# kjedrzejewski/video-cycle_gan-upscaling

Measured on AMD Instinct MI355X. Metric: upscaled frames/s (train step, G+D fwd+bwd) at 256->512, higher is better.
Workload: dtype f32; 1 GPU; C2: make_upscaler_orig((512,512,3),k=3,x2,res=9) + PatchGAN-70, batch 8/GPU, gan2 wiring, Wasserstein + pixel-MSE, faithful 3-call step incl. predict pass; global_batch=8, frame=256x256->512x512, parallelism=dp1, launch=hipGraph replay

## Files before the change

include/vcg.h:

```cpp
#ifndef VCG_H
#define VCG_H

#include <stddef.h>
#include <stdint.h>

#ifdef __cplusplus
extern "C" {
#endif

typedef void* vcg_stream_t;

enum {
    VCG_OK = 0,
    VCG_E_NULL = -1,
    VCG_E_SHAPE = -2,
    VCG_E_UNSUPPORTED = -3,
    VCG_E_WORKSPACE = -4
};

enum { VCG_ACT_NONE = 0, VCG_ACT_LRELU = 1, VCG_ACT_PRELU = 2, VCG_ACT_TANH = 3 };
enum { VCG_NORM_BATCH = 0, VCG_NORM_INSTANCE = 1 };
enum { VCG_LOSS_MSE = 0, VCG_LOSS_MAE = 1 };
enum { VCG_HEAD_NONE = 0, VCG_HEAD_SIGMOID = 1, VCG_HEAD_LOGSIGM = 2, VCG_HEAD_TANH = 3, VCG_HEAD_BILOG = 4 };

typedef struct vcg_conv_desc {
    int32_t n, cin, h, w;
    int32_t cout, oh, ow;
    int32_t kh, kw, stride;
    int32_t pad_top, pad_left;
} vcg_conv_desc;

typedef struct vcg_epilogue {
    const float* bias;
    int32_t act;
    float act_alpha;
    const float* prelu_alpha;
    const float* residual;
} vcg_epilogue;

const char* vcg_version(void);
const char* vcg_error_string(int code);

int vcg_conv2d_fwd(const vcg_conv_desc* d, const float* x, const float* w_hwio, float* y,
                   const vcg_epilogue* ep, vcg_stream_t stream);
int vcg_conv2d_stats_records(const vcg_conv_desc* d, int stats_mode);
int vcg_conv2d_fwd_stats(const vcg_conv_desc* d, const float* x, const float* w_hwio, const float* bias, float* y, float* stats,
                         vcg_stream_t stream);
int vcg_conv2d_dgrad(const vcg_conv_desc* d, const float* dy, const float* w_hwio, const float* w_hwoi,
                     float* dx, const float* residual, vcg_stream_t stream);
int vcg_conv2d_fwd_affine(const vcg_conv_desc* d, const float* x, const float* w_hwio, float* y, const vcg_epilogue* ep, const float* scale,
                          const float* shift, vcg_stream_t stream);
size_t vcg_conv2d_wgrad_workspace_bytes(const vcg_conv_desc* d);
int vcg_conv2d_wgrad(const vcg_conv_desc* d, const float* x, const float* dy, float* dw_hwio, float* dbias,
                     void* ws, size_t ws_bytes, vcg_stream_t stream);

int vcg_conv_transpose2d_fwd(const vcg_conv_desc* d, const float* x, const float* w_hwio_t, float* y,
                             const vcg_epilogue* ep, vcg_stream_t stream);
int vcg_conv_transpose2d_dgrad(const vcg_conv_desc* d, const float* dy, const float* w_hwoi, float* dx,
                               const float* residual, vcg_stream_t stream);
size_t vcg_conv_transpose2d_wgrad_workspace_bytes(const vcg_conv_desc* d);
int vcg_conv_transpose2d_wgrad(const vcg_conv_desc* d, const float* x, const float* dy, float* dw_hwoi,
                               float* dbias, void* ws, size_t ws_bytes, vcg_stream_t stream);

int vcg_kernel_transpose(const float* src, float* dst, int taps, int a, int b, vcg_stream_t stream);

size_t vcg_norm_stats_workspace_bytes(int n, int c, int hw, int mode);
int vcg_norm_stats(const float* x, int n, int c, int hw, int mode, float* mean, float* var,
                   void* ws, size_t ws_bytes, vcg_stream_t stream);
int vcg_norm_finalize(const float* mean, const float* var, const float* gamma, const float* beta, int c,
                      int rows, float eps, float* scale, float* shift, float* invstd,
                      float* moving_mean, float* moving_var, float momentum, int unbiased_count,
                      vcg_stream_t stream);
int vcg_sum_records(const float* part, int nrec, int c, float scale, float* out, vcg_stream_t stream);
int vcg_bn_fold(const float* bias, const float* moving_mean, const float* moving_var, const float* gamma, const float* beta, int c, float eps,
                float* scale, float* shift, vcg_stream_t stream);
int vcg_bn_fold_batch(const float* const* bias, const float* const* moving_mean, const float* const* moving_var, const float* const* gamma,
                      const float* const* beta, int count, int c, float eps, float* scale, float* shift, vcg_stream_t stream);
int vcg_norm_finalize_batch(const float* const* mean, const float* const* var, const float* const* gamma, const float* const* beta, int count,
                            int c, float eps, float* scale, float* shift, vcg_stream_t stream);
int vcg_norm_finalize_partials(const float* part, int nrec, int groups, int c, double count, const float* gamma, const float* beta,
                               float eps, float* mean, float* scale, float* shift, float* invstd, float* moving_mean,
                               float* moving_var, float momentum, int unbiased_count, vcg_stream_t stream);
int vcg_norm_finalize_partials_shifted(const float* part, int nrec, int groups, int c, double count, const float* kshift, const float* gamma,
                                       const float* beta, float eps, float* mean, float* scale, float* shift, float* invstd, float* moving_mean,
                                       float* moving_var, float momentum, int unbiased_count, vcg_stream_t stream);
int vcg_norm_act_fwd(const float* x, int n, int c, int hw, const float* scale, const float* shift,
                     int per_sample, int act, float act_alpha, const float* prelu_alpha,
                     const float* residual, float* y, vcg_stream_t stream);
size_t vcg_norm_act_bwd_workspace_bytes(int n, int c, int hw, int mode);
int vcg_norm_act_bwd(const float* x, const float* dy, int n, int c, int hw, int mode,
                     const float* mean, const float* invstd, const float* gamma, const float* beta,
                     int act, float act_alpha, const float* prelu_alpha, int use_batch_stats,
                     float* dx, float* dgamma, float* dbeta, float* dprelu_alpha,
                     void* ws, size_t ws_bytes, vcg_stream_t stream);

size_t vcg_act_bwd_workspace_bytes(int n, int c, int hw);
int vcg_act_bwd(const float* saved, const float* dy, int n, int c, int hw, int act, float act_alpha,
                const float* prelu_alpha, float* dx, float* dprelu_alpha, float* dsum, void* ws, size_t ws_bytes,
                vcg_stream_t stream);
size_t vcg_channel_sum_workspace_bytes(int n, int c, int hw);
int vcg_channel_sum(const float* x, int n, int c, int hw, float* out, void* ws, size_t ws_bytes,
                    vcg_stream_t stream);

int vcg_dense_fwd(const float* x, const float* w_io, const float* bias, float* y, int batch, int in,
                  int out, vcg_stream_t stream);
int vcg_dense_dgrad(const float* dy, const float* w_io, float* dx, int batch, int in, int out,
                    vcg_stream_t stream);
int vcg_dense_wgrad(const float* x, const float* dy, float* dw_io, float* dbias, int batch, int in,
                    int out, vcg_stream_t stream);

size_t vcg_mean_reduce_workspace_bytes(size_t count);
int vcg_mean_reduce(const float* x, size_t count, float* out, void* ws, size_t ws_bytes, vcg_stream_t stream);
int vcg_pixel_loss(const float* pred, const float* target, size_t count, int kind, float grad_scale,
                   float* out, float* dpred, void* ws, size_t ws_bytes, vcg_stream_t stream);
int vcg_head_act_fwd(const float* z, float* y, size_t count, int kind, vcg_stream_t stream);
int vcg_head_act_bwd(const float* z, const float* dy, float* dz, size_t count, int kind, vcg_stream_t stream);
int vcg_gan_loss(const float* mean_a, const float* mean_b, float mean_scale, int kind, float* loss_out, float* da, size_t na,
                 float ga, float* db, size_t nb, float gb, vcg_stream_t stream);
int vcg_sigmoid_gate_fwd(const float* a, const float* m, float* y, size_t count, vcg_stream_t stream);
int vcg_sigmoid_gate_bwd(const float* a, const float* m, const float* dy, float* da, float* dm, size_t count, vcg_stream_t stream);
int vcg_atanh_scale(const float* x, float* y, size_t count, float scale, vcg_stream_t stream);
int vcg_dilate2d(const float* src, float* dst, size_t planes, int h, int w, int stride, vcg_stream_t stream);
int vcg_resize2d(const float* src, float* dst, size_t planes, int h, int w, int factor, int bilinear, vcg_stream_t stream);
int vcg_crop2d(const float* src, float* dst, size_t planes, int h, int w, int top, int left, int oh, int ow, vcg_stream_t stream);
int vcg_pad2d(const float* src, float* dst, size_t planes, int h, int w, int top, int left, int oh, int ow, vcg_stream_t stream);
int vcg_copy_channels(const float* src, float* dst, int n, int c_src, int c_src_off, int c_dst, int c_dst_off, int c_count, size_t hw,
                      vcg_stream_t stream);
int vcg_dropout_fwd(const float* x, float* y, unsigned char* mask, size_t count, float rate, unsigned long long seed,
                    const unsigned long long* step, vcg_stream_t stream);
int vcg_dropout_bwd(const float* dy, const unsigned char* mask, float* dx, size_t count, float rate, vcg_stream_t stream);
int vcg_counter_inc(unsigned long long* counter, vcg_stream_t stream);
int vcg_fill(float* y, size_t count, float value, vcg_stream_t stream);
int vcg_axpby(const float* x, float* y, size_t count, float a, float b, vcg_stream_t stream);

int vcg_maxpool2x2_fwd(const float* x, float* y, int n, int c, int h, int w, vcg_stream_t stream);
int vcg_maxpool2x2_bwd(const float* x, const float* dy, float* dx, int n, int c, int h, int w, vcg_stream_t stream);

int vcg_adam_keras_multi(float* p, const float* g, float* m, float* v, size_t count, float lr_t,
                         float beta_1, float beta_2, float eps, float grad_scale, vcg_stream_t stream);

int vcg_adam_keras_multi_dev(float* p, const float* g, float* m, float* v, size_t count, float lr,
                             float beta_1, float beta_2, float eps, float grad_scale, int* t_dev, vcg_stream_t stream);

int vcg_frames_u8_to_nchw(const uint8_t* src, float* dst, int n, int h, int w, int c, vcg_stream_t stream);
int vcg_nchw_to_frames_u8(const float* src, uint8_t* dst, int n, int h, int w, int c, vcg_stream_t stream);
int vcg_nhwc_to_nchw(const float* src, float* dst, int n, int h, int w, int c, vcg_stream_t stream);
int vcg_nchw_to_nhwc(const float* src, float* dst, int n, int h, int w, int c, vcg_stream_t stream);


typedef struct vcg_epilogue_bf16 {
    const void* scale;
    const void* shift;
    int32_t act;
    float act_alpha;
    const void* prelu_alpha;
    const void* residual;
    void* stats;
    int32_t stats_mode;
} vcg_epilogue_bf16;
#define VCG_STATS_NONE 0
#define VCG_STATS_BATCH 1
#define VCG_STATS_INSTANCE 2

int vcg_pack_conv_kernel_bf16(const void* w, int32_t taps, int32_t a, int32_t b, int32_t transpose, int32_t flip, void* out,
                              hipStream_t stream);

int vcg_pack_conv3x3_c64_bf16_batch(const void* const* w_host_array, int32_t count, void* out, hipStream_t stream);
int vcg_f32_nchw_to_bf16_nhwc(const void* x, void* y, int32_t n, int32_t c, int32_t h, int32_t w, hipStream_t stream);
int vcg_bf16_nhwc_to_f32_nchw(const void* x, void* y, int32_t n, int32_t c, int32_t h, int32_t w, hipStream_t stream);

int vcg_conv2d_bf16_fwd(const vcg_conv_desc* d, const void* x, const void* w_packed, void* y, const vcg_epilogue_bf16* ep,
                        hipStream_t stream);
int vcg_conv2d_bf16_stats_records(const vcg_conv_desc* d, int32_t stats_mode);

int vcg_conv_transpose2d_bf16_fwd(const vcg_conv_desc* d, const void* x, const void* w_packed, void* y, const vcg_epilogue_bf16* ep,
                                  hipStream_t stream);

#define VCG_FINAL9X9_WFRAG_BYTES ((4 * 9 * 4 * 64 + 4) * 16)
int vcg_pack_final9x9_bf16(const void* w, void* out, hipStream_t stream);
int vcg_conv9x9_to3_bf16_fwd(const vcg_conv_desc* d, const void* x, const void* wfrag, const void* bias, int32_t tanh_act, void* y,
                             hipStream_t stream);
size_t vcg_conv9x9_to3_bf16_wfrag_bytes(int32_t cin);
int vcg_pack_conv9x9_to3_bf16(const void* w, int32_t cin, void* out, hipStream_t stream);
#define VCG_OUT_F32_NCHW 0
#define VCG_OUT_U8_NHWC 1
int vcg_conv9x9_to3_bf16_fwd_window(const vcg_conv_desc* d, const void* x, const void* wfrag, const void* bias, int32_t tanh_act,
                                    int32_t out_kind, void* y, int32_t row0, int32_t rows, int32_t y_row0, int32_t y_h, hipStream_t stream);
size_t vcg_conv9x9_c64to3_bf16_wfrag_bytes(void);
int vcg_pack_conv9x9_c64to3_bf16(const void* w, void* out, hipStream_t stream);
int vcg_conv9x9_c64to3_bf16_fwd(const vcg_conv_desc* d, const void* x, const void* wfrag, const void* bias, int32_t tanh_act, void* y,
                                hipStream_t stream);
int vcg_conv9x9_c64to3_bf16_fwd_window(const vcg_conv_desc* d, const void* x, const void* wfrag, const void* bias, int32_t tanh_act,
                                       int32_t out_kind, void* y, int32_t row0, int32_t rows, int32_t y_row0, int32_t y_h, hipStream_t stream);

#define VCG_FIRST9X9_WFRAG_BYTES (27 * 64 * 2 * 16)
int vcg_pack_first9x9_bf16(const void* w, void* out, hipStream_t stream);
int vcg_pack_conv9x9_3ch_bf16(const void* w, int32_t cout, int32_t dgrad, void* out, hipStream_t stream);
int vcg_conv9x9_to3_bf16_dgrad(const vcg_conv_desc* d, const void* dy, const void* wfrag, const void* y_prev, float lrelu_slope, void* dx,
                               hipStream_t stream);
int vcg_conv9x9_to3_bf16_dgrad_chsum_records(const vcg_conv_desc* d);
int vcg_conv9x9_to3_bf16_dgrad_chsum(const vcg_conv_desc* d, const void* dy, const void* wfrag, const void* y_prev, float lrelu_slope, void* dx,
                                     float* records, hipStream_t stream);
int vcg_conv9x9_from3_bf16_fwd(const vcg_conv_desc* d, const void* x, const void* wfrag, const void* bias, const void* prelu_alpha,
                               void* y, hipStream_t stream);

size_t vcg_conv3ch_bf16_wfrag_bytes(int32_t kh, int32_t kw, int32_t cout);
int vcg_pack_conv3ch_bf16(const void* w, int32_t kh, int32_t kw, int32_t cout, void* out, hipStream_t stream);
int vcg_conv3ch_bf16_fwd(const vcg_conv_desc* d, const void* x, const void* wfrag, const void* bias, float lrelu_slope, void* y, hipStream_t stream);

size_t vcg_conv_in_gate_bf16_wfrag_bytes(int32_t cin, int32_t kh, int32_t kw, int32_t cout);
int vcg_pack_conv_in_gate_bf16(const void* w_hwio, int32_t cin, int32_t kh, int32_t kw, int32_t cout, void* out, hipStream_t stream);
int vcg_conv_in_gate_bf16_fwd(const vcg_conv_desc* d, const void* u, const void* wfrag, const void* bias, const void* m, void* y,
                              hipStream_t stream);

int vcg_input_convt_add_bf16(const vcg_conv_desc* d, const void* x, const void* w_hwoi, const void* bias, void* y, hipStream_t stream);
size_t vcg_conv3ch_bf16_dgrad_workspace_bytes(const vcg_conv_desc* d);
int vcg_conv3ch_bf16_dgrad(const vcg_conv_desc* d, const void* dz, const float* w_hwio, float* dx, void* ws, size_t ws_bytes, vcg_stream_t stream);
size_t vcg_conv3ch_bf16_wgrad_workspace_bytes(const vcg_conv_desc* d);
int vcg_conv3ch_bf16_wgrad(const vcg_conv_desc* d, const float* x, const void* dz, float* dw_hwio, float* dbias, void* ws, size_t ws_bytes,
                           vcg_stream_t stream);
int vcg_conv9x9_from3_bf16_fwd_train(const vcg_conv_desc* d, const void* x, const void* wfrag, const void* bias, const void* prelu_alpha,
                                     void* y, void* z, hipStream_t stream);
int vcg_prelu_bwd_nhwc_bf16_records(int n, int hw);
int vcg_prelu_bwd_nhwc_bf16(const void* d1, const void* d2, const void* z, const float* prelu_alpha, int n, int c, int hw, float* dz_nchw,
                            float* records, hipStream_t stream);
int vcg_prelu_bwd_nhwc_bf16_to_bf16(const void* d1, const void* d2, const void* z, const float* prelu_alpha, int n, int c, int hw, void* dz_nhwc,
                                    float* records, hipStream_t stream);

size_t vcg_norm_stats_bf16_workspace_bytes(int n, int c, int hw, int mode);
int vcg_norm_stats_bf16(const void* x, int n, int c, int hw, int mode, float* mean, float* var, void* ws, size_t ws_bytes,
                        hipStream_t stream);
int vcg_norm_act_fwd_bf16(const void* x, int n, int c, int hw, const float* scale, const float* shift, int per_sample, int act,
                          float alpha, const float* prelu_alpha, const void* residual, void* y, hipStream_t stream);
size_t vcg_norm_act_bwd_bf16_workspace_bytes(int n, int c, int hw, int mode);
int vcg_norm_act_bwd_bf16(const void* x, const void* dy, int n, int c, int hw, int mode, const float* mean, const float* invstd,
                          const float* gamma, const float* beta, int act, float act_alpha, const float* prelu_alpha, int use_batch_stats,
                          void* dx, float* dgamma, float* dbeta, float* dprelu_alpha, void* ws, size_t ws_bytes, hipStream_t stream);

int vcg_conv2d_cout1_nhwc_bf16_fwd(const vcg_conv_desc* d, const void* x, const float* w_hwio, const float* bias, float* y, vcg_stream_t stream);
int vcg_conv2d_cout1_nhwc_bf16_dgrad(const vcg_conv_desc* d, const float* dy, const float* w_hwio, void* dx, vcg_stream_t stream);
size_t vcg_conv2d_cout1_nhwc_bf16_wgrad_workspace_bytes(const vcg_conv_desc* d);
int vcg_conv2d_cout1_nhwc_bf16_wgrad(const vcg_conv_desc* d, const void* x, const float* dy, float* dw_hwio, float* dbias, void* ws, size_t ws_bytes,
                                     vcg_stream_t stream);

size_t vcg_conv2d_bf16_wgrad_workspace_bytes(const vcg_conv_desc* d);
int vcg_conv2d_bf16_wgrad(const vcg_conv_desc* d, const void* x, const void* dy, float* dw_hwio, float* dbias, void* ws, size_t ws_bytes,
                          hipStream_t stream);

size_t vcg_conv9x9_to3_bf16_wgrad_workspace_bytes(const vcg_conv_desc* d);
int vcg_conv9x9_to3_bf16_wgrad(const vcg_conv_desc* d, const void* x, const float* dz, float* dw_hwio, void* ws, size_t ws_bytes, hipStream_t stream);

size_t vcg_conv_frag_bf16_bytes(int taps, int mdim, int kdim);
// ... 28 lines not shown
```

video-cycle_gan-upscaling_amd/csrc/api.hip:

```cpp
#include "vcg_common.hpp"

int vcg_internal_conv(const float* x, const float* w, float* y, int n, int cin, int h, int wd, int cout, int oh,
                      int ow, int kh, int kw, int stride, int pad_top, int pad_left, int flip, const vcg_epilogue* ep,
                      int smallm, int ws_t, int ws_m, int ws_k, hipStream_t st, float* stats = nullptr, const float* scale = nullptr,
                      const float* shift = nullptr);
int vcg_internal_convt(const float* x, const float* w, float* y, int n, int cin, int h, int wd, int cout, int oh,
                       int ow, int k, int cby, int cbx, const vcg_epilogue* ep, hipStream_t st);
size_t vcg_internal_wgrad_ws(int n, int mtot, int ah, int aw, int jctot, int kh, int kw, int S);
int vcg_internal_wgrad(const float* A, const float* B, float* dw, float* db, int n, int mtot, int ah, int aw,
                       int jctot, int bh, int bw, int kh, int kw, int S, int pt, int pl_, int flip, int ts, int sm,
                       int sj, void* ws, size_t ws_bytes, hipStream_t st);

namespace {

int check_desc(const vcg_conv_desc* d) {
    if (d == nullptr) return VCG_E_NULL;
    if (d->n <= 0 || d->cin <= 0 || d->h <= 0 || d->w <= 0 || d->cout <= 0 || d->oh <= 0 || d->ow <= 0)
        return VCG_E_SHAPE;
    if (d->kh <= 0 || d->kw <= 0 || d->stride < 1 || d->stride > 3) return VCG_E_UNSUPPORTED;
    if (d->pad_top < 0 || d->pad_left < 0 || d->pad_top >= d->kh || d->pad_left >= d->kw) return VCG_E_SHAPE;
    return VCG_OK;
}

inline bool use_smallm(int mch, int kh, int kw, int stride) { return stride == 1 && kh == kw && kh >= 3 && mch * kw <= 32; }

}

extern "C" {

const char* vcg_version(void) { return "vcg-hip 0.1 (gfx950, fp32 MFMA 32x32x2)"; }

const char* vcg_error_string(int code) {
    switch (code) {
        case VCG_OK: return "ok";
        case VCG_E_NULL: return "required pointer is NULL";
        case VCG_E_SHAPE: return "inconsistent or unsupported dimensions";
        case VCG_E_UNSUPPORTED: return "kernel size / stride / padding combination not instantiated";
        case VCG_E_WORKSPACE: return "workspace missing or too small";
        default: return code > 0 ? hipGetErrorString((hipError_t)code) : "unknown error";
    }
}

int vcg_conv2d_fwd(const vcg_conv_desc* d, const float* x, const float* w_hwio, float* y, const vcg_epilogue* ep,
                   vcg_stream_t stream) {
    int rc = check_desc(d);
    if (rc) return rc;
    VCG_CHECK_PTR(x); VCG_CHECK_PTR(w_hwio); VCG_CHECK_PTR(y);
    if ((d->oh - 1) * d->stride - d->pad_top >= d->h || (d->ow - 1) * d->stride - d->pad_left >= d->w) return VCG_E_SHAPE;
    const bool sm = use_smallm(d->cout, d->kh, d->kw, d->stride);
    return vcg_internal_conv(x, w_hwio, y, d->n, d->cin, d->h, d->w, d->cout, d->oh, d->ow, d->kh, d->kw, d->stride,
                             d->pad_top, d->pad_left, 0, ep, sm ? 1 : 0, d->cin * d->cout, 1, d->cout,
                             (hipStream_t)stream);
}

static bool conv_stats_tiles(const vcg_conv_desc* d, int* tiles_per_image) {
    const bool k3 = d->kh == 3 && d->kw == 3, k4 = d->kh == 4 && d->kw == 4;
    if (!(k3 || k4) || d->stride > 2 || d->cin <= 3) return false;
    const bool sm = use_smallm(d->cout, d->kh, d->kw, d->stride);
    if (sm) return false;
    const int xt = (k3 && d->stride == 1 && d->ow > 32) ? 2 : 1;
    *tiles_per_image = ceil_div(d->ow, 32 * xt) * ceil_div(d->oh, 8);
    return true;
}

int vcg_conv2d_stats_records(const vcg_conv_desc* d, int stats_mode) {
    int rc = check_desc(d);
    if (rc) return rc;
    int tpi = 0;
    if (!conv_stats_tiles(d, &tpi) || (stats_mode != VCG_STATS_BATCH && stats_mode != VCG_STATS_INSTANCE)) return VCG_E_UNSUPPORTED;
    const long all = (long)tpi * d->n;
    if (all > 0x3fffffffL) return VCG_E_UNSUPPORTED;
    return (int)(stats_mode == VCG_STATS_INSTANCE ? tpi : all);
}

int vcg_conv2d_fwd_stats(const vcg_conv_desc* d, const float* x, const float* w_hwio, const float* bias, float* y, float* stats,
                         vcg_stream_t stream) {
    int rc = check_desc(d);
    if (rc) return rc;
    VCG_CHECK_PTR(x); VCG_CHECK_PTR(w_hwio); VCG_CHECK_PTR(y); VCG_CHECK_PTR(stats);
    if ((d->oh - 1) * d->stride - d->pad_top >= d->h || (d->ow - 1) * d->stride - d->pad_left >= d->w) return VCG_E_SHAPE;
    int tpi = 0;
    if (!conv_stats_tiles(d, &tpi)) return VCG_E_UNSUPPORTED;
    vcg_epilogue ep{};
    ep.bias = bias;
    ep.act = VCG_ACT_NONE;
    return vcg_internal_conv(x, w_hwio, y, d->n, d->cin, d->h, d->w, d->cout, d->oh, d->ow, d->kh, d->kw, d->stride, d->pad_top, d->pad_left, 0,
                             &ep, 0, d->cin * d->cout, 1, d->cout, (hipStream_t)stream, stats);
}

int vcg_conv2d_fwd_affine(const vcg_conv_desc* d, const float* x, const float* w_hwio, float* y, const vcg_epilogue* ep, const float* scale,
                          const float* shift, vcg_stream_t stream) {
    int rc = check_desc(d);
    if (rc) return rc;
    VCG_CHECK_PTR(x); VCG_CHECK_PTR(w_hwio); VCG_CHECK_PTR(y); VCG_CHECK_PTR(scale); VCG_CHECK_PTR(shift);
    if ((d->oh - 1) * d->stride - d->pad_top >= d->h || (d->ow - 1) * d->stride - d->pad_left >= d->w) return VCG_E_SHAPE;
    if (use_smallm(d->cout, d->kh, d->kw, d->stride)) return VCG_E_UNSUPPORTED;
    return vcg_internal_conv(x, w_hwio, y, d->n, d->cin, d->h, d->w, d->cout, d->oh, d->ow, d->kh, d->kw, d->stride, d->pad_top, d->pad_left, 0,
                             ep, 0, d->cin * d->cout, 1, d->cout, (hipStream_t)stream, nullptr, scale, shift);
}

int vcg_conv2d_dgrad(const vcg_conv_desc* d, const float* dy, const float* w_hwio, const float* w_hwoi, float* dx,
                     const float* residual, vcg_stream_t stream) {
    int rc = check_desc(d);
    if (rc) return rc;
    VCG_CHECK_PTR(dy); VCG_CHECK_PTR(dx);
    vcg_epilogue ep{};
    ep.residual = residual;
    hipStream_t st = (hipStream_t)stream;
    if (d->stride == 1) {
        const int pt = d->kh - 1 - d->pad_top, pl = d->kw - 1 - d->pad_left;
        if (use_smallm(d->cin, d->kh, d->kw, 1)) {
            VCG_CHECK_PTR(w_hwio);
            return vcg_internal_conv(dy, w_hwio, dx, d->n, d->cout, d->oh, d->ow, d->cin, d->h, d->w, d->kh, d->kw, 1,
                                     pt, pl, 1, &ep, 1, d->cin * d->cout, d->cout, 1, st);
        }
        VCG_CHECK_PTR(w_hwoi);
        return vcg_internal_conv(dy, w_hwoi, dx, d->n, d->cout, d->oh, d->ow, d->cin, d->h, d->w, d->kh, d->kw, 1, pt,
                                 pl, 1, &ep, 0, 0, 0, 0, st);
    }
    if (d->kh != d->kw || d->stride != 2) return VCG_E_UNSUPPORTED;
    VCG_CHECK_PTR(w_hwoi);
    return vcg_internal_convt(dy, w_hwoi, dx, d->n, d->cout, d->oh, d->ow, d->cin, d->h, d->w, d->kh, d->pad_top,
                              d->pad_left, &ep, st);
}

size_t vcg_conv2d_wgrad_workspace_bytes(const vcg_conv_desc* d) {
    if (check_desc(d)) return 0;
    size_t a;
    if (d->stride == 1 && d->cout <= 3)
        a = vcg_internal_wgrad_ws(d->n, d->cin, d->h, d->w, d->cout, d->kh, d->kw, 1);
    else
        a = vcg_internal_wgrad_ws(d->n, d->cout, d->oh, d->ow, d->cin, d->kh, d->kw, d->stride);
    const size_t b = vcg_channel_sum_workspace_bytes(d->n, d->cout, d->oh * d->ow);
    return a > b ? a : b;
}

int vcg_conv2d_wgrad(const vcg_conv_desc* d, const float* x, const float* dy, float* dw_hwio, float* dbias, void* ws,
                     size_t ws_bytes, vcg_stream_t stream) {
    int rc = check_desc(d);
    if (rc) return rc;
    VCG_CHECK_PTR(x); VCG_CHECK_PTR(dy); VCG_CHECK_PTR(dw_hwio);
    hipStream_t st = (hipStream_t)stream;
    const int cc = d->cin * d->cout;
    if (d->stride == 1 && d->cout <= 3) {
        rc = vcg_internal_wgrad(x, dy, dw_hwio, nullptr, d->n, d->cin, d->h, d->w, d->cout, d->oh, d->ow, d->kh, d->kw,
                                1, d->kh - 1 - d->pad_top, d->kw - 1 - d->pad_left, 1, cc, d->cout, 1, ws, ws_bytes, st);
    } else {
        rc = vcg_internal_wgrad(dy, x, dw_hwio, dbias, d->n, d->cout, d->oh, d->ow, d->cin, d->h, d->w, d->kh, d->kw,
                                d->stride, d->pad_top, d->pad_left, 0, cc, 1, d->cout, ws, ws_bytes, st);
        dbias = nullptr;
    }
    if (rc) return rc;
    if (dbias) {
        if (ws_bytes < vcg_channel_sum_workspace_bytes(d->n, d->cout, d->oh * d->ow)) return VCG_E_WORKSPACE;
        rc = vcg_channel_sum(dy, d->n, d->cout, d->oh * d->ow, dbias, ws, ws_bytes, stream);
    }
    return rc;
}

int vcg_conv_transpose2d_fwd(const vcg_conv_desc* d, const float* x, const float* w_hwio_t, float* y,
                             const vcg_epilogue* ep, vcg_stream_t stream) {
    int rc = check_desc(d);
    if (rc) return rc;
    VCG_CHECK_PTR(x); VCG_CHECK_PTR(w_hwio_t); VCG_CHECK_PTR(y);
    if (d->stride != 2 || d->kh != d->kw) return VCG_E_UNSUPPORTED;
    if (d->oh > 2 * d->h || d->ow > 2 * d->w) return VCG_E_SHAPE;
    return vcg_internal_convt(x, w_hwio_t, y, d->n, d->cin, d->h, d->w, d->cout, d->oh, d->ow, d->kh, d->pad_top,
                              d->pad_left, ep, (hipStream_t)stream);
}

int vcg_conv_transpose2d_dgrad(const vcg_conv_desc* d, const float* dy, const float* w_hwoi, float* dx,
                               const float* residual, vcg_stream_t stream) {
    int rc = check_desc(d);
    if (rc) return rc;
    VCG_CHECK_PTR(dy); VCG_CHECK_PTR(w_hwoi); VCG_CHECK_PTR(dx);
    if (d->stride != 2) return VCG_E_UNSUPPORTED;
    vcg_epilogue ep{};
    ep.residual = residual;
    return vcg_internal_conv(dy, w_hwoi, dx, d->n, d->cout, d->oh, d->ow, d->cin, d->h, d->w, d->kh, d->kw, 2,
                             d->pad_top, d->pad_left, 0, &ep, 0, 0, 0, 0, (hipStream_t)stream);
}

size_t vcg_conv_transpose2d_wgrad_workspace_bytes(const vcg_conv_desc* d) {
    if (check_desc(d)) return 0;
    size_t a = vcg_internal_wgrad_ws(d->n, d->cin, d->h, d->w, d->cout, d->kh, d->kw, 2);
    size_t b = vcg_channel_sum_workspace_bytes(d->n, d->cout, d->oh * d->ow);
    return a > b ? a : b;
}

int vcg_conv_transpose2d_wgrad(const vcg_conv_desc* d, const float* x, const float* dy, float* dw_hwoi, float* dbias,
                               void* ws, size_t ws_bytes, vcg_stream_t stream) {
    int rc = check_desc(d);
    if (rc) return rc;
    VCG_CHECK_PTR(x); VCG_CHECK_PTR(dy); VCG_CHECK_PTR(dw_hwoi);
    if (d->stride != 2) return VCG_E_UNSUPPORTED;
    rc = vcg_internal_wgrad(x, dy, dw_hwoi, nullptr, d->n, d->cin, d->h, d->w, d->cout, d->oh, d->ow, d->kh, d->kw, 2,
                            d->pad_top, d->pad_left, 0, d->cin * d->cout, 1, d->cin, ws, ws_bytes, (hipStream_t)stream);
    if (rc) return rc;
    if (dbias) {
        if (ws_bytes < vcg_channel_sum_workspace_bytes(d->n, d->cout, d->oh * d->ow)) return VCG_E_WORKSPACE;
        rc = vcg_channel_sum(dy, d->n, d->cout, d->oh * d->ow, dbias, ws, ws_bytes, stream);
    }
    return rc;
}

}
```

video-cycle_gan-upscaling_amd/csrc/conv_fwd.hip:

```cpp
#include "vcg_common.hpp"
#include <type_traits>

namespace {

struct ConvParams {
    const float* x;
    const float* w;
    float* y;
    const float* bias;
    const float* prelu;
    const float* residual;
    int n, cin, h, w_, cout, oh, ow, pad_top, pad_left;
    int tiles_x, tiles_y, co_blocks;
    int act;
    float alpha;
    int flip;
    int ws_t, ws_m, ws_k;
    float* stats;
    const float* scale;
    const float* shift;
};

template <int KH, int KW, int S, int CK, int XT>
struct ConvCfg {
    static constexpr int ROWS = 8;
    static constexpr int IH = (ROWS - 1) * S + KH;
    static constexpr int IW = (32 * XT - 1) * S + KW;
    static constexpr int PLANE = IH * IW;
    static constexpr int T = KH * KW;
    static constexpr int IN_ELEMS = CK * PLANE;
    static constexpr int W_ELEMS = CK * T * 64;
    static constexpr int IN_PT = (IN_ELEMS + 255) / 256;
    static constexpr int W_PT = (W_ELEMS + 255) / 256;
    static constexpr size_t LDS_BYTES = (size_t)(IN_ELEMS + W_ELEMS) * sizeof(float);
};

template <int XT, bool AFFINE = false>
__device__ __forceinline__ void conv_epilogue(const ConvParams& p, f32x16 (&acc)[2][2][XT], int n, int co0, int oy0, int ox0,
                                              int wv, int lane) {
    const int half = lane >> 5, l31 = lane & 31;
    const unsigned plane = (unsigned)(p.oh * p.ow), plane4 = 4u * plane, ow4 = 4u * (unsigned)p.ow;
    const int nch = p.cout - co0 < 64 ? p.cout - co0 : 64;
    const size_t blk = ((size_t)n * p.cout + co0) * plane;
    const size_t blk_bytes = (size_t)nch * plane * sizeof(float);
    const vcg_rsrc ry = make_rsrc(p.y + blk, blk_bytes);
    const vcg_rsrc rr = make_rsrc(p.residual ? p.residual + blk : nullptr, p.residual ? blk_bytes : 0);
    const bool is_prelu = p.act == VCG_ACT_PRELU;
    const vcg_rsrc rbias = make_rsrc(p.bias, p.bias ? (size_t)p.cout * sizeof(float) : 0);
    const vcg_rsrc rslope = make_rsrc(is_prelu ? p.prelu : nullptr, is_prelu ? (size_t)p.cout * sizeof(float) : 0);
    const float slope_u = (p.act == VCG_ACT_LRELU) ? p.alpha : 1.f;
    const unsigned chan4 = 4u * (unsigned)(co0 + 4 * half);
    const vcg_rsrc rscale = make_rsrc(AFFINE ? p.scale : nullptr, AFFINE ? (size_t)p.cout * sizeof(float) : 0);
    const vcg_rsrc rshift = make_rsrc(AFFINE ? p.shift : nullptr, AFFINE ? (size_t)p.cout * sizeof(float) : 0);

    const int oy = oy0 + wv * 2, ox = ox0 + l31;
    const unsigned base = (unsigned)(4 * half) * plane4 + (unsigned)oy * ow4 + 4u * (unsigned)ox;
    unsigned vo[2][XT];
#pragma unroll
    for (int rt = 0; rt < 2; ++rt)
#pragma unroll
        for (int xt = 0; xt < XT; ++xt)
            vo[rt][xt] = (oy + rt < p.oh && ox + xt * 32 < p.ow) ? base + (unsigned)rt * ow4 + 128u * xt : VCG_OOB;

    constexpr int RG = 8 / XT, NG = 32 / RG;
    auto emit = [&](auto res_tag, auto prelu_tag) {
        constexpr bool RES = decltype(res_tag)::value;
        constexpr bool PRELU_FMA = decltype(prelu_tag)::value;
        float rs[2][RG][2][XT];
        auto row_of = [](int g, int j) { const int q = g * RG + j, r = q & 15; return (q >> 4) * 32 + (r & 3) + 8 * (r >> 2); };
        auto load_res = [&](int g) {
#pragma unroll
            for (int j = 0; j < RG; ++j) {
                const unsigned srow = (unsigned)row_of(g, j) * plane4;
#pragma unroll
                for (int rt = 0; rt < 2; ++rt)
#pragma unroll
                    for (int xt = 0; xt < XT; ++xt) rs[g & 1][j][rt][xt] = buf_load(rr, __builtin_elementwise_add_sat(vo[rt][xt], srow));
            }
        };
        if (RES) load_res(0);
#pragma unroll
        for (int g = 0; g < NG; ++g) {
            float bv[RG], al[RG], sc[RG], sh[RG];
#pragma unroll
            for (int j = 0; j < RG; ++j) {
                bv[j] = buf_load(rbias, chan4 + 4u * (unsigned)row_of(g, j));
                const float pa = buf_load(rslope, chan4 + 4u * (unsigned)row_of(g, j));
                al[j] = is_prelu ? pa : slope_u;
                if (AFFINE) {
                    sc[j] = buf_load(rscale, chan4 + 4u * (unsigned)row_of(g, j));
                    sh[j] = buf_load(rshift, chan4 + 4u * (unsigned)row_of(g, j));
                }
            }
            if (RES && g + 1 < NG) load_res(g + 1);
#pragma unroll
            for (int j = 0; j < RG; ++j) {
                const int q = g * RG + j;
                const unsigned srow = (unsigned)row_of(g, j) * plane4;
#pragma unroll
                for (int rt = 0; rt < 2; ++rt) {
#pragma unroll
                    for (int xt = 0; xt < XT; ++xt) {
                        float v = acc[q >> 4][rt][xt][q & 15] + bv[j];
                        if (AFFINE) v = __builtin_fmaf(sc[j], v, sh[j]);
                        if (PRELU_FMA) v = __builtin_fmaf(al[j], fminf(v, 0.f), fmaxf(v, 0.f));
                        else v = v >= 0.f ? v : v * al[j];
                        if (RES) v += rs[g & 1][j][rt][xt];
                        buf_store(ry, __builtin_elementwise_add_sat(vo[rt][xt], srow), v);
                    }
                }
            }
        }
    };
    if constexpr (AFFINE) {
        if (is_prelu) {
            if (p.residual) emit(std::true_type{}, std::true_type{}); else emit(std::false_type{}, std::true_type{});
        } else {
            if (p.residual) emit(std::true_type{}, std::false_type{}); else emit(std::false_type{}, std::false_type{});
        }
    } else {
        if (p.residual) emit(std::true_type{}, std::false_type{}); else emit(std::false_type{}, std::false_type{});
    }
}

template <int XT>
__device__ __forceinline__ void conv_stats_epilogue(const ConvParams& p, f32x16 (&acc)[2][2][XT], float* smem, int rec, int co0, int oy0, int ox0,
                                                    int wv, int lane, int tid) {
    const int half = lane >> 5, l31 = lane & 31;
    float sv[32], sq[32];
#pragma unroll
    for (int mt = 0; mt < 2; ++mt)
#pragma unroll
        for (int r = 0; r < 16; ++r) {
            float a = 0.f, b = 0.f;
#pragma unroll
            for (int rt = 0; rt < 2; ++rt)
#pragma unroll
                for (int xt = 0; xt < XT; ++xt) {
                    const bool ok = oy0 + wv * 2 + rt < p.oh && ox0 + l31 + xt * 32 < p.ow;
                    const float v = ok ? acc[mt][rt][xt][r] : 0.f;
                    a += v;
                    b = fmaf(v, v, b);
                }
            sv[mt * 16 + r] = a;
            sq[mt * 16 + r] = b;
        }
    const float ts = half_wave_reduce_scatter32(sv, l31), tq = half_wave_reduce_scatter32(sq, l31);
    const int ch = (l31 >> 4) * 32 + (l31 & 3) + 8 * ((l31 & 15) >> 2) + 4 * half;
    __syncthreads();
    smem[(0 * 4 + wv) * 64 + ch] = ts;
    smem[(1 * 4 + wv) * 64 + ch] = tq;
    __syncthreads();
    if (tid < 128) {
        const int st = tid >> 6, c = tid & 63;
        const float t = (smem[(st * 4 + 0) * 64 + c] + smem[(st * 4 + 1) * 64 + c]) + (smem[(st * 4 + 2) * 64 + c] + smem[(st * 4 + 3) * 64 + c]);
        if (co0 + c < p.cout) p.stats[((size_t)rec * 2 + st) * p.cout + co0 + c] = t;
    }
}

template <int KH, int KW, int S, int CK, int XT, bool STATS = false, bool AFFINE = false>
__global__ __launch_bounds__(256, (KH >= 9 ? 1 : 2)) void conv_fwd_kernel(const ConvParams p) {
    using C = ConvCfg<KH, KW, S, CK, XT>;
    extern __shared__ __attribute__((aligned(16))) float smem[];
    float* s_in = smem;
    float* s_w = smem + C::IN_ELEMS;

    const int tid = threadIdx.x, lane = tid & 63, wv = tid >> 6;
    const int half = lane >> 5, l31 = lane & 31;
    int b = blockIdx.x;
    const int cb = b % p.co_blocks; b /= p.co_blocks;
    const int tx = b % p.tiles_x;   b /= p.tiles_x;
    const int ty = b % p.tiles_y;   b /= p.tiles_y;
    const int n = b;
    const int ox0 = tx * 32 * XT, oy0 = ty * C::ROWS, co0 = cb * 64;
    const int gy0 = oy0 * S - p.pad_top, gx0 = ox0 * S - p.pad_left;
    const float* xn = p.x + (size_t)n * p.cin * p.h * p.w_;

    float rin[C::IN_PT], rw[C::W_PT];

    const int hw = p.h * p.w_;
    const int wvu = __builtin_amdgcn_readfirstlane(wv);
    const unsigned wcol = 4u * (unsigned)(co0 + lane < p.cout ? co0 + lane : p.cout - 1);
    const size_t wbytes = (size_t)C::T * p.cin * p.cout * sizeof(float);

    auto in_rsrc = [&](int ci0) { return make_rsrc(xn + (size_t)ci0 * hw, (size_t)(p.cin - ci0) * hw * sizeof(float)); };
    auto load_w = [&](int ci0) {
        const vcg_rsrc rwt = make_rsrc(p.w + (size_t)ci0 * p.cout, wbytes - (size_t)ci0 * p.cout * sizeof(float));
#pragma unroll
        for (int i = 0; i < C::W_PT; ++i) {
            const int q = wvu + 4 * i;
            const int t = q % C::T, ci = q / C::T;
            const int tap = p.flip ? (C::T - 1 - t) : t;
            rw[i] = buf_load(rwt, 4u * (unsigned)((tap * p.cin + ci) * p.cout) + wcol);
        }
    };
    load_w(0);
    __builtin_amdgcn_sched_barrier(0);

    unsigned in_off[C::IN_PT];
    {
        constexpr int Q1 = 256 / C::PLANE, R1 = 256 % C::PLANE, QR = R1 / C::IW, RC = R1 % C::IW;
        const vcg_rsrc rx = in_rsrc(0);
        const unsigned w4 = 4u * (unsigned)p.w_, hw4 = 4u * (unsigned)hw;
        const unsigned step = (unsigned)Q1 * hw4 + (unsigned)QR * w4 + 4u * RC;
        const unsigned col_wrap = w4 - 4u * C::IW, row_wrap = hw4 - (unsigned)C::IH * w4;
        int ci = tid / C::PLANE, r = (tid % C::PLANE) / C::IW, c = (tid % C::PLANE) % C::IW;
        unsigned off = (unsigned)ci * hw4 + (unsigned)(gy0 + r) * w4 + 4u * (unsigned)(gx0 + c);
#pragma unroll
        for (int i = 0; i < C::IN_PT; ++i) {
            const bool in_tile = (i + 1) * 256 <= C::IN_ELEMS || ci < CK;
            const bool ok = in_tile && (unsigned)(gy0 + r) < (unsigned)p.h && (unsigned)(gx0 + c) < (unsigned)p.w_;
            in_off[i] = ok ? off : VCG_OOB;
            rin[i] = buf_load(rx, in_off[i]);
            __builtin_amdgcn_sched_barrier(0);
            c += RC;
            const bool cw = c >= C::IW;
            c -= cw ? C::IW : 0;
            r += QR + (cw ? 1 : 0);
            const bool rwr = r >= C::IH;
            r -= rwr ? C::IH : 0;
            ci += Q1 + (rwr ? 1 : 0);
            off += step + (cw ? col_wrap : 0u) + (rwr ? row_wrap : 0u);
        }
    }
    auto load_chunk = [&](int ci0) {
        const vcg_rsrc rx = in_rsrc(ci0);
#pragma unroll
        for (int i = 0; i < C::IN_PT; ++i) rin[i] = buf_load(rx, in_off[i]);
        load_w(ci0);
    };
    auto store_chunk = [&]() {
#pragma unroll
        for (int i = 0; i < C::IN_PT; ++i) {
            const int e = tid + i * 256;
            if (e < C::IN_ELEMS) s_in[e] = rin[i];
        }
#pragma unroll
        for (int i = 0; i < C::W_PT; ++i) {
            const int e = tid + i * 256;
            if (e < C::W_ELEMS) s_w[e] = rw[i];
        }
    };

    f32x16 acc[2][2][XT];
#pragma unroll
    for (int i = 0; i < 2; ++i)
#pragma unroll
        for (int j = 0; j < 2; ++j)
#pragma unroll
            for (int x = 0; x < XT; ++x)
#pragma unroll
                for (int r = 0; r < 16; ++r) acc[i][j][x][r] = 0.f;

    const float* bbase = s_in + half * C::PLANE + (wv * 2 * S) * C::IW + l31 * S;
    const float* abase = s_w + half * C::T * 64 + l31;

    const int nchunks = (p.cin + CK - 1) / CK;
    for (int c = 0; c < nchunks; ++c) {
        __syncthreads();
        store_chunk();
        __syncthreads();
        if (c + 1 < nchunks) load_chunk((c + 1) * CK);
        constexpr int NTAP = (CK / 2) * C::T;
        auto rd = [&](int q, float (&a)[2], float (&b)[2][XT]) {
            const int cp = q / C::T, t = q % C::T, ky = t / KW, kx = t % KW;
            a[0] = abase[(cp * 2 * C::T + t) * 64];
            a[1] = abase[(cp * 2 * C::T + t) * 64 + 32];
#pragma unroll
            for (int xt = 0; xt < XT; ++xt) {
                b[0][xt] = bbase[cp * 2 * C::PLANE + ky * C::IW + kx + xt * 32 * S];
                b[1][xt] = bbase[cp * 2 * C::PLANE + (S + ky) * C::IW + kx + xt * 32 * S];
            }
        };
        float a_[2][2], b_[2][2][XT];
        rd(0, a_[0], b_[0]);
#pragma unroll
        for (int q = 0; q < NTAP; ++q) {
            const int cur = q & 1, nxt = cur ^ 1;
            if (q + 1 < NTAP) rd(q + 1, a_[nxt], b_[nxt]);
#pragma unroll
            for (int xt = 0; xt < XT; ++xt) {
                acc[0][0][xt] = mfma32(a_[cur][0], b_[cur][0][xt], acc[0][0][xt]);
                acc[0][1][xt] = mfma32(a_[cur][0], b_[cur][1][xt], acc[0][1][xt]);
                acc[1][0][xt] = mfma32(a_[cur][1], b_[cur][0][xt], acc[1][0][xt]);
                acc[1][1][xt] = mfma32(a_[cur][1], b_[cur][1][xt], acc[1][1][xt]);
            }
            if (q + 1 < NTAP) __builtin_amdgcn_sched_group_barrier(0x100, 1 + 2 * XT, 0);
            __builtin_amdgcn_sched_group_barrier(0x008, 4 * XT, 0);
        }
    }

    conv_epilogue<XT, AFFINE>(p, acc, n, co0, oy0, ox0, wv, lane);
    if (STATS) conv_stats_epilogue<XT>(p, acc, smem, (n * p.tiles_y + ty) * p.tiles_x + tx, co0, oy0, ox0, wv, lane, tid);
}

template <int KH, int KW, int S>
struct C3Cfg {
    static constexpr int ROWS = 8;
    static constexpr int IH = (ROWS - 1) * S + KH;
    static constexpr int IW = 31 * S + KW;
    static constexpr int PLANE = IH * IW;
    static constexpr int T = KH * KW;
    static constexpr int KT = 3 * T;
    static constexpr int NP = (KT + 1) / 2;
    static constexpr int IN_ELEMS = 3 * PLANE;
    static constexpr int W_ROWS = 2 * NP;
    static constexpr int W_ELEMS = W_ROWS * 64;
    static constexpr int IN_PT = (IN_ELEMS + 255) / 256;
    static constexpr int W_PT = W_ELEMS / 256;
    static constexpr int IN_BUF = IN_ELEMS + 4;
    static constexpr size_t LDS_BYTES = (size_t)(2 * IN_BUF + W_ELEMS) * sizeof(float);
    static_assert(IW < 256 && W_ELEMS % 256 == 0, "packed (row, column) of a halo element; whole weight rows per wave");
    static constexpr int off(int k) { return (k / T) * PLANE + ((k % T) / KW) * IW + (k % T) % KW; }
    static constexpr int D_ROW = IW - (KW - 1);
    static constexpr int D_CH = PLANE - (KH - 1) * IW - (KW - 1);
};

template <int KH, int KW, int S>
__global__ __launch_bounds__(256, 2) void conv_c3_kernel(const ConvParams p) {
    using C = C3Cfg<KH, KW, S>;
    extern __shared__ __attribute__((aligned(16))) float smem[];
    float* s_in = smem;
    float* s_w = smem + 2 * C::IN_BUF;

    const int tid = threadIdx.x, lane = tid & 63, wv = tid >> 6;
    const int half = lane >> 5, l31 = lane & 31;
    const int nblk = p.co_blocks, step = (int)gridDim.x / nblk;
    const int cb = (int)blockIdx.x % nblk, co0 = cb * 64;
    int t = (int)blockIdx.x / nblk;
    const int tiles = p.n * p.tiles_y * p.tiles_x;
    if (t >= tiles) return;
    int tx = t % p.tiles_x, ty = (t / p.tiles_x) % p.tiles_y, n = t / (p.tiles_x * p.tiles_y);
    const int dtx = step % p.tiles_x, dty = (step / p.tiles_x) % p.tiles_y, dn = step / (p.tiles_x * p.tiles_y);

    constexpr bool KEEP = C::IN_PT <= 8;
    const int hw = p.h * p.w_;
    const unsigned w4 = 4u * (unsigned)p.w_, hw4 = 4u * (unsigned)hw;
    const size_t img_bytes = (size_t)p.cin * hw * sizeof(float);
    auto decode = [&](int tid_, int i, unsigned& rel_, unsigned& rc_) {
        const int e = tid_ + i * 256;
        const int ci = e / C::PLANE, rem = e % C::PLANE;
        const int r = rem / C::IW, c = rem % C::IW;
        rel_ = (unsigned)ci * hw4 + (unsigned)r * w4 + 4u * (unsigned)c;
        rc_ = (unsigned)(r << 8 | c);
    };
    unsigned rel[KEEP ? C::IN_PT : 1], rc[KEEP ? C::IN_PT : 1];
    if constexpr (KEEP) {
#pragma unroll
        for (int i = 0; i < C::IN_PT; ++i) {
            decode(tid, i, rel[i], rc[i]);
            asm volatile("" : "+v"(rc[i]));
        }
    }
    const bool last_live = tid + (C::IN_PT - 1) * 256 < C::IN_ELEMS;
    float rin[C::IN_PT];
    auto load_tile = [&](int n_, int ty_, int tx_) {
        const int gy0 = ty_ * C::ROWS * S - p.pad_top, gx0 = tx_ * 32 * S - p.pad_left;
        const vcg_rsrc rx = make_rsrc(p.x + (size_t)n_ * p.cin * hw, img_bytes);
        const unsigned tb = (unsigned)gy0 * w4 + 4u * (unsigned)gx0;
        int tid_t = tid;
        if constexpr (!KEEP) asm volatile("" : "+v"(tid_t));
#pragma unroll
        for (int i = 0; i < C::IN_PT; ++i) {
            unsigned rl, q;
            if constexpr (KEEP) { rl = rel[i]; q = rc[i]; } else decode(tid_t, i, rl, q);
            bool ok = (unsigned)(gy0 + (int)(q >> 8)) < (unsigned)p.h && (unsigned)(gx0 + (int)(q & 255u)) < (unsigned)p.w_;
            if (i == C::IN_PT - 1) ok = ok && last_live;
            rin[i] = buf_load(rx, ok ? tb + rl : VCG_OOB);
        }
    };
    auto store_tile = [&](float* buf) {
#pragma unroll
        for (int i = 0; i < C::IN_PT; ++i) {
            const int e = tid + i * 256;
            if (e < C::IN_ELEMS) buf[e] = rin[i];
        }
    };
    load_tile(n, ty, tx);

    {
        const vcg_rsrc rwt = make_rsrc(p.w, (size_t)C::T * p.cin * p.cout * sizeof(float));
        const int wvu = __builtin_amdgcn_readfirstlane(wv);
        const unsigned col = co0 + lane < p.cout ? 4u * (unsigned)(co0 + lane) : VCG_OOB;
        float rw[C::W_PT];
#pragma unroll
        for (int i = 0; i < C::W_PT; ++i) {
            const int k = wvu + 4 * i;
            const int ci = k / C::T, tt = k % C::T;
            const int tap = p.flip ? (C::T - 1 - tt) : tt;
            const unsigned row = (k < C::KT && ci < p.cin) ? 4u * (unsigned)((tap * p.cin + ci) * p.cout) : VCG_OOB;
            rw[i] = buf_load(rwt, __builtin_elementwise_add_sat(col, row));
        }
        if (tid < 8) s_in[(tid >> 2) * C::IN_BUF + C::IN_ELEMS + (tid & 3)] = 0.f;
#pragma unroll
        for (int i = 0; i < C::W_PT; ++i) s_w[tid + i * 256] = rw[i];
    }
    store_tile(s_in);
    lds_barrier();

    const float* abase = s_w + half * 64 + l31;
    const float* b0p = s_in + (wv * 2 * S) * C::IW + l31 * S;
    int cur = 0;
    for (;;) {
        const bool more = step < tiles - t;
        const int n0 = n, oy0 = ty * C::ROWS, ox0 = tx * 32;
        if (more) {
            t += step;
            tx += dtx;
            const int cx = tx >= p.tiles_x ? 1 : 0;
            tx -= cx ? p.tiles_x : 0;
            ty += dty + cx;
            const int cy = ty >= p.tiles_y ? 1 : 0;
            ty -= cy ? p.tiles_y : 0;
            n += dn + cy;
            load_tile(n, ty, tx);
        }

        f32x16 acc[2][2][1];
#pragma unroll
        for (int i = 0; i < 2; ++i)
#pragma unroll
            for (int j = 0; j < 2; ++j)
#pragma unroll
                for (int r = 0; r < 16; ++r) acc[i][j][0][r] = 0.f;

        const float* b0 = b0p + cur * C::IN_BUF;
        const float* bb1 = b0 + half * 1;
        const float* bb2 = b0 + half * C::D_ROW;
        const float* bb3 = b0 + half * C::D_CH;
        auto rd = [&](int pr, float (&f)[4]) {
            const int k0 = 2 * pr, k1 = 2 * pr + 1;
            const int o0 = C::off(k0);
            const int d = (k1 < C::KT) ? (C::off(k1) - o0) : 1;
            const float* bb = (d == 1) ? bb1 : (d == C::D_ROW ? bb2 : bb3);
            f[0] = abase[k0 * 64];
            f[1] = abase[k0 * 64 + 32];
            f[2] = bb[o0];
            f[3] = bb[o0 + S * C::IW];
        };
        float f_[2][4];
        rd(0, f_[0]);
#pragma unroll
        for (int pr = 0; pr < C::NP; ++pr) {
            const float(&f)[4] = f_[pr & 1];
            if (pr + 1 < C::NP) rd(pr + 1, f_[(pr & 1) ^ 1]);
            acc[0][0][0] = mfma32(f[0], f[2], acc[0][0][0]);
            acc[0][1][0] = mfma32(f[0], f[3], acc[0][1][0]);
            acc[1][0][0] = mfma32(f[1], f[2], acc[1][0][0]);
            acc[1][1][0] = mfma32(f[1], f[3], acc[1][1][0]);
            if (pr + 1 < C::NP) __builtin_amdgcn_sched_group_barrier(0x100, 4, 0);
            __builtin_amdgcn_sched_group_barrier(0x008, 4, 0);
        }
        if (more) {
            store_tile(s_in + (cur ^ 1) * C::IN_BUF);
            lds_barrier();
        }
        conv_epilogue<1>(p, acc, n0, co0, oy0, ox0, wv, lane);
        if (!more) break;
        cur ^= 1;
    }
}

template <int KH, int KW, int CK>
struct SmallCfg {
    static constexpr int ROWS = 8;
    static constexpr int XW = 64;
    static constexpr int OUTW = XW - (KW - 1);
    static constexpr int IH = ROWS + KH - 1;
    static constexpr int PLANE = IH * XW;
    static constexpr int IN_ELEMS = CK * PLANE;
    static constexpr int W_ELEMS = CK * KH * 32;
    static constexpr int IN_PT = (IN_ELEMS + 255) / 256;
    static constexpr int W_PT = (W_ELEMS + 255) / 256;
    static constexpr int PST = XW + 1;
    static constexpr int SCRATCH = 4 * 32 * PST;
    static constexpr int LDS_ELEMS = (IN_ELEMS + W_ELEMS) > SCRATCH ? (IN_ELEMS + W_ELEMS) : SCRATCH;
    static constexpr size_t LDS_BYTES = (size_t)LDS_ELEMS * sizeof(float);
};

template <int KH, int KW, int CK>
__global__ __launch_bounds__(256) void conv_smallm_kernel(const ConvParams p) {
    using C = SmallCfg<KH, KW, CK>;
    extern __shared__ __attribute__((aligned(16))) float smem[];
    float* s_in = smem;
    float* s_w = smem + C::IN_ELEMS;

    const int tid = threadIdx.x, lane = tid & 63, wv = tid >> 6;
    const int half = lane >> 5, l31 = lane & 31;
    int b = blockIdx.x;
    const int tx = b % p.tiles_x; b /= p.tiles_x;
    const int ty = b % p.tiles_y; b /= p.tiles_y;
    const int n = b;
    const int ox0 = tx * C::OUTW, oy0 = ty * C::ROWS;
    const int gy0 = oy0 - p.pad_top, gx0 = ox0 - p.pad_left;
    const float* xn = p.x + (size_t)n * p.cin * p.h * p.w_;
    const int mrows = p.cout * KW;

    float rin[C::IN_PT], rw[C::W_PT];
    const int wvu = __builtin_amdgcn_readfirstlane(tid >> 6);
    const int gx = gx0 + lane;
    const bool col_ok = gx >= 0 && gx < p.w_;
    const int gxc = min(max(gx, 0), p.w_ - 1);
    const int hw = p.h * p.w_;
    const vcg_rsrc rx = make_rsrc(xn, (size_t)p.cin * hw * sizeof(float));
    const vcg_rsrc rwt = make_rsrc(p.w, (size_t)KH * KW * p.cin * p.cout * sizeof(float));
    auto load_chunk = [&](int ci0) {
#pragma unroll
        for (int i = 0; i < C::IN_PT; ++i) {
            const int q = wvu + 4 * i;
            const int r = q % C::IH, ci = q / C::IH;
            const int gy = gy0 + r, ch = ci0 + ci;
            const bool ok = col_ok && ch < p.cin && gy >= 0 && gy < p.h;
            rin[i] = buf_load(rx, ok ? 4u * (unsigned)(ch * hw + gy * p.w_ + gxc) : VCG_OOB);
        }
#pragma unroll
        for (int i = 0; i < C::W_PT; ++i) {
            const int e = tid + i * 256;
            const int mi = e & 31, q = e >> 5;
            const int ky = q % KH, ci = q / KH;
            const int ch = ci0 + ci;
            const bool ok = e < C::W_ELEMS && ch < p.cin && mi < mrows;
            const int mch = mi / KW, kx = mi % KW;
            int tap = ky * KW + kx;
            if (p.flip) tap = KH * KW - 1 - tap;
            rw[i] = buf_load(rwt, ok ? 4u * (unsigned)(tap * p.ws_t + mch * p.ws_m + ch * p.ws_k) : VCG_OOB);
        }
    };
    auto store_chunk = [&]() {
#pragma unroll
        for (int i = 0; i < C::IN_PT; ++i) {
            const int e = tid + i * 256;
            if (e < C::IN_ELEMS) s_in[e] = rin[i];
        }
#pragma unroll
        for (int i = 0; i < C::W_PT; ++i) {
            const int e = tid + i * 256;
            if (e < C::W_ELEMS) s_w[e] = rw[i];
        }
    };

    f32x16 acc[2][2];
#pragma unroll
    for (int i = 0; i < 2; ++i)
#pragma unroll
        for (int j = 0; j < 2; ++j)
#pragma unroll
            for (int r = 0; r < 16; ++r) acc[i][j][r] = 0.f;

    const float* bbase = s_in + half * C::PLANE + (wv * 2) * C::XW + l31;
    const float* abase = s_w + half * KH * 32 + l31;

    const int nchunks = (p.cin + CK - 1) / CK;
    load_chunk(0);
    for (int c = 0; c < nchunks; ++c) {
        __syncthreads();
        store_chunk();
        __syncthreads();
        if (c + 1 < nchunks) load_chunk((c + 1) * CK);
#pragma unroll
        for (int cp = 0; cp < CK / 2; ++cp) {
#pragma unroll
            for (int ky = 0; ky < KH; ++ky) {
                const float a = abase[(cp * 2 * KH + ky) * 32];
                const float b00 = bbase[cp * 2 * C::PLANE + ky * C::XW];
                const float b01 = bbase[cp * 2 * C::PLANE + ky * C::XW + 32];
                const float b10 = bbase[cp * 2 * C::PLANE + (ky + 1) * C::XW];
                const float b11 = bbase[cp * 2 * C::PLANE + (ky + 1) * C::XW + 32];
                acc[0][0] = mfma32(a, b00, acc[0][0]);
                acc[0][1] = mfma32(a, b01, acc[0][1]);
                acc[1][0] = mfma32(a, b10, acc[1][0]);
                acc[1][1] = mfma32(a, b11, acc[1][1]);
            }
        }
    }

    float* s_p = smem + wv * 32 * C::PST;
#pragma unroll
    for (int rt = 0; rt < 2; ++rt) {
        __syncthreads();
#pragma unroll
        for (int xt = 0; xt < 2; ++xt)
#pragma unroll
            for (int r = 0; r < 16; ++r) s_p[mfma_row(r, lane) * C::PST + xt * 32 + l31] = acc[rt][xt][r];
        __syncthreads();
        const int oy = oy0 + wv * 2 + rt;
        const int ox = ox0 + lane;
        if (lane < C::OUTW && oy < p.oh && ox < p.ow) {
            for (int mch = 0; mch < p.cout; ++mch) {
                float v = 0.f;
#pragma unroll
                for (int kx = 0; kx < KW; ++kx) v += s_p[(mch * KW + kx) * C::PST + lane + kx];
                const float bv = p.bias ? p.bias[mch] : 0.f;
                const float al = (p.act == VCG_ACT_PRELU) ? p.prelu[mch] : p.alpha;
                const size_t idx = (((size_t)n * p.cout + mch) * p.oh + oy) * p.ow + ox;
                v = apply_act(v + bv, p.act, al);
                if (p.residual) v += p.residual[idx];
                p.y[idx] = v;
            }
        }
    }
}

template <int K>
__global__ __launch_bounds__(256) void conv_cout1_kernel(const ConvParams p) {
    __shared__ float red[4][64];
    const int tid = threadIdx.x, xl = tid & 63;
    const int cg = __builtin_amdgcn_readfirstlane(tid >> 6);
    int b = blockIdx.x;
    const int seg = b % p.tiles_x; b /= p.tiles_x;
    const int oy = b % p.oh;
    const int n = b / p.oh;
    const int ox = seg * 64 + xl, gx0 = ox - p.pad_left, gy0 = oy - p.pad_top;
    const int hw = p.h * p.w_;
    const vcg_rsrc rx = make_rsrc(p.x + (size_t)n * p.cin * hw, (size_t)p.cin * hw * sizeof(float));
    unsigned coff[K];
#pragma unroll
    for (int kx = 0; kx < K; ++kx) coff[kx] = (unsigned)(gx0 + kx) < (unsigned)p.w_ ? 4u * (unsigned)(gx0 + kx) : VCG_OOB;
    float acc = 0.f;
#pragma unroll 1
    for (int c = cg; c < p.cin; c += 4) {
        float wr[K * K];
#pragma unroll
        for (int t = 0; t < K * K; ++t) wr[t] = p.w[(p.flip ? K * K - 1 - t : t) * p.ws_t + c * p.ws_k];
#pragma unroll
        for (int ky = 0; ky < K; ++ky) {
            const int gy = gy0 + ky;
            const bool rok = (unsigned)gy < (unsigned)p.h;
            const unsigned rbase = 4u * (unsigned)(c * hw + gy * p.w_);
#pragma unroll
            for (int kx = 0; kx < K; ++kx) acc += buf_load(rx, rok && coff[kx] != VCG_OOB ? rbase + coff[kx] : VCG_OOB) * wr[ky * K + kx];
        }
    }
    red[cg][xl] = acc;
    __syncthreads();
    if (cg == 0 && ox < p.ow) {
        float v = ((red[0][xl] + red[1][xl]) + (red[2][xl] + red[3][xl])) + (p.bias ? p.bias[0] : 0.f);
        if (p.act == VCG_ACT_LRELU) v = v >= 0.f ? v : v * p.alpha;
        else if (p.act == VCG_ACT_TANH) v = tanhf(v);
        const size_t o = ((size_t)n * p.oh + oy) * p.ow + ox;
        if (p.residual) v += p.residual[o];
        p.y[o] = v;
    }
}

template <int K>
int launch_cout1(ConvParams p, hipStream_t st) {
    p.tiles_x = ceil_div(p.ow, 64);
    const long grid = (long)p.tiles_x * p.oh * p.n;
    if (grid <= 0 || grid > 0x7fffffffL) return VCG_E_SHAPE;
    hipLaunchKernelGGL(conv_cout1_kernel<K>, dim3((unsigned)grid), dim3(256), 0, st, p);
    VCG_LAUNCH_CHECK();
    return VCG_OK;
}

template <typename Kern>
int launch_with_lds(Kern kern, int grid, size_t lds, const ConvParams& p, hipStream_t st) {
    if (int e = vcg_allow_dyn_lds(reinterpret_cast<const void*>(kern), lds)) return e;
    hipLaunchKernelGGL(kern, dim3(grid), dim3(256), lds, st, p);
    VCG_LAUNCH_CHECK();
    return VCG_OK;
}

bool conv_block_fits(int oh, int ow, int ck, int h, int w) {
    const unsigned long long lim = 0xFFFFFFE0ull;
    return 64ull * oh * ow * sizeof(float) < lim && (unsigned long long)ck * h * w * sizeof(float) < lim;
}

template <int KH, int KW, int S, int CK, int XT>
int launch_conv(ConvParams p, hipStream_t st) {
    using C = ConvCfg<KH, KW, S, CK, XT>;
    if (!conv_block_fits(p.oh, p.ow, CK, p.h, p.w_)) return VCG_E_UNSUPPORTED;
    p.tiles_x = ceil_div(p.ow, 32 * XT);
    p.tiles_y = ceil_div(p.oh, C::ROWS);
    p.co_blocks = ceil_div(p.cout, 64);
    const long grid = (long)p.tiles_x * p.tiles_y * p.co_blocks * p.n;
    if (grid <= 0 || grid > 0x7fffffffL) return VCG_E_SHAPE;
    if (p.stats && p.scale) return VCG_E_UNSUPPORTED;
    if (p.stats) {
        if constexpr ((KH == 3 && KW == 3 && S <= 2) || (KH == 4 && KW == 4 && S <= 2))
            return launch_with_lds(conv_fwd_kernel<KH, KW, S, CK, XT, true>, (int)grid, C::LDS_BYTES, p, st);
        else
            return VCG_E_UNSUPPORTED;
    }
    if (p.scale) {
        if constexpr (S == 1 && ((KH == 3 && KW == 3) || (KH == 5 && KW == 5)))
            return launch_with_lds(conv_fwd_kernel<KH, KW, S, CK, XT, false, true>, (int)grid, C::LDS_BYTES, p, st);
        else
            return VCG_E_UNSUPPORTED;
    }
    return launch_with_lds(conv_fwd_kernel<KH, KW, S, CK, XT>, (int)grid, C::LDS_BYTES, p, st);
}

int device_cu_count() {
    static const int cus = [] {
        int dev = 0, v = 0;
        if (hipGetDevice(&dev) != hipSuccess || hipDeviceGetAttribute(&v, hipDeviceAttributeMultiprocessorCount, dev) != hipSuccess) return 0;
        return v;
    }();
    return cus;
}

template <int KH, int KW, int S>
int launch_c3(ConvParams p, hipStream_t st) {
    using C = C3Cfg<KH, KW, S>;
    if (!conv_block_fits(p.oh, p.ow, 3, p.h, p.w_)) return VCG_E_UNSUPPORTED;
    p.tiles_x = ceil_div(p.ow, 32);
    p.tiles_y = ceil_div(p.oh, C::ROWS);
    p.co_blocks = ceil_div(p.cout, 64);
    const long tiles = (long)p.tiles_x * p.tiles_y * p.co_blocks * p.n;
    if (tiles <= 0 || tiles > 0x7fffffffL) return VCG_E_SHAPE;
    const int cus = device_cu_count();
    if (cus <= 0) return VCG_E_UNSUPPORTED;
    long grid = tiles < 2L * cus ? tiles : 2L * cus;
    grid -= grid % p.co_blocks;
    if (grid < p.co_blocks) grid = p.co_blocks;
    return launch_with_lds(conv_c3_kernel<KH, KW, S>, (int)grid, C::LDS_BYTES, p, st);
}

template <int KH, int KW, int CK>
int launch_smallm(ConvParams p, hipStream_t st) {
    using C = SmallCfg<KH, KW, CK>;
    p.tiles_x = ceil_div(p.ow, C::OUTW);
    p.tiles_y = ceil_div(p.oh, C::ROWS);
    p.co_blocks = 1;
    const long grid = (long)p.tiles_x * p.tiles_y * p.n;
    if (grid <= 0 || grid > 0x7fffffffL) return VCG_E_SHAPE;
    return launch_with_lds(conv_smallm_kernel<KH, KW, CK>, (int)grid, C::LDS_BYTES, p, st);
}

}

int vcg_internal_conv9_rowchain(const float* x, const float* w, float* y, int n, int cin, int h, int wd, int cout, const float* bias, int act,
                                int ws_t, int ws_m, int ws_k, hipStream_t st);

int vcg_internal_conv(const float* x, const float* w, float* y, int n, int cin, int h, int wd, int cout,
                      int oh, int ow, int kh, int kw, int stride, int pad_top, int pad_left, int flip,
                      const vcg_epilogue* ep, int smallm, int ws_t, int ws_m, int ws_k, hipStream_t st, float* stats, const float* scale, const float* shift) {
    ConvParams p{};
    p.x = x; p.w = w; p.y = y; p.stats = stats;
    if (stats && (smallm || cin <= 3)) return VCG_E_UNSUPPORTED;
    if (scale && (smallm || stats || cin <= 3)) return VCG_E_UNSUPPORTED;
    if (scale && shift == nullptr) return VCG_E_NULL;
    p.scale = scale; p.shift = scale ? shift : nullptr;
    p.bias = ep ? ep->bias : nullptr;
    p.prelu = ep ? ep->prelu_alpha : nullptr;
    p.residual = ep ? ep->residual : nullptr;
    p.act = ep ? ep->act : VCG_ACT_NONE;
    p.alpha = ep ? ep->act_alpha : 0.f;
    if (p.act == VCG_ACT_PRELU && p.prelu == nullptr) return VCG_E_NULL;
    p.n = n; p.cin = cin; p.h = h; p.w_ = wd; p.cout = cout; p.oh = oh; p.ow = ow;
    p.pad_top = pad_top; p.pad_left = pad_left; p.flip = flip;
    p.ws_t = ws_t; p.ws_m = ws_m; p.ws_k = ws_k;
    if (n <= 0 || cin <= 0 || cout <= 0 || oh <= 0 || ow <= 0) return VCG_E_SHAPE;
    if (smallm) {
        if (stride != 1 || cout * kw > 32) return VCG_E_UNSUPPORTED;
        if (kh == 9 && kw == 9 && !flip && pad_top == 4 && pad_left == 4 && oh == h && ow == wd && !p.prelu && !p.residual) {
            const int rc = vcg_internal_conv9_rowchain(x, w, y, n, cin, h, wd, cout, p.bias, p.act, ws_t, ws_m, ws_k, st);
            if (rc != VCG_E_UNSUPPORTED) return rc;
        }
        if (cout == 1 && cin >= 64 && kh == kw && ws_m == 1 && !p.prelu && (size_t)cin * h * wd * 4 <= 0xFFFFFFE0u) {
            if (kh == 3) return launch_cout1<3>(p, st);
            if (kh == 4) return launch_cout1<4>(p, st);
            if (kh == 5) return launch_cout1<5>(p, st);
        }
        if (kh == 9 && kw == 9) return launch_smallm<9, 9, 8>(p, st);
        if (kh == 4 && kw == 4) return launch_smallm<4, 4, 8>(p, st);
        if (kh == 3 && kw == 3) return launch_smallm<3, 3, 8>(p, st);
        if (kh == 5 && kw == 5) return launch_smallm<5, 5, 8>(p, st);
        return VCG_E_UNSUPPORTED;
    }
    if (p.act == VCG_ACT_TANH) return VCG_E_UNSUPPORTED;
    if (cin <= 3) {
        if (kh == 9 && kw == 9 && stride == 1) return launch_c3<9, 9, 1>(p, st);
        if (kh == 3 && kw == 3 && stride == 1) return launch_c3<3, 3, 1>(p, st);
        if (kh == 4 && kw == 4 && stride == 2) return launch_c3<4, 4, 2>(p, st);
        if (kh == 5 && kw == 5 && stride == 1) return launch_c3<5, 5, 1>(p, st);
    }
    const bool wide = ow > 32;
    if (kh == 3 && kw == 3 && stride == 1) return wide ? launch_conv<3, 3, 1, 8, 2>(p, st) : launch_conv<3, 3, 1, 8, 1>(p, st);
    if (kh == 5 && kw == 5 && stride == 1) return launch_conv<5, 5, 1, 8, 1>(p, st);
    if (scale) return VCG_E_UNSUPPORTED;
    if (kh == 3 && kw == 3 && stride == 2) return launch_conv<3, 3, 2, 8, 1>(p, st);
    if (kh == 4 && kw == 4 && stride == 1) return launch_conv<4, 4, 1, 8, 1>(p, st);
    if (kh == 4 && kw == 4 && stride == 2) return launch_conv<4, 4, 2, 4, 1>(p, st);
    if (kh == 5 && kw == 5 && stride == 2) return launch_conv<5, 5, 2, 4, 1>(p, st);
    if (kh == 5 && kw == 5 && stride == 3) return launch_conv<5, 5, 3, 4, 1>(p, st);
    if (kh == 9 && kw == 9 && stride == 1) return launch_conv<9, 9, 1, 4, 1>(p, st);
    if (stride == 1) {
        if (kh == 1 && kw == 1) return launch_conv<1, 1, 1, 8, 1>(p, st);
        if (kh == 1 && kw == 3) return launch_conv<1, 3, 1, 8, 1>(p, st);
        if (kh == 3 && kw == 1) return launch_conv<3, 1, 1, 8, 1>(p, st);
        if (kh == 1 && kw == 5) return launch_conv<1, 5, 1, 8, 1>(p, st);
        if (kh == 5 && kw == 1) return launch_conv<5, 1, 1, 8, 1>(p, st);
        if (kh == 1 && kw == 7) return launch_conv<1, 7, 1, 8, 1>(p, st);
        if (kh == 7 && kw == 1) return launch_conv<7, 1, 1, 8, 1>(p, st);
    }
    return VCG_E_UNSUPPORTED;
}
```

video-cycle_gan-upscaling_amd/csrc/conv_transpose.hip:

```cpp
#include "vcg_common.hpp"
#include <type_traits>

namespace {

struct ConvTParams {
    const float* x;
    const float* w;
    float* y;
    const float* bias;
    const float* prelu;
    const float* residual;
    int n, cin, h, w_, cout, oh, ow;
    int tiles_x, tiles_y, co_blocks;
    int act;
    float alpha;
};

constexpr int phase_of(int k, int cb) { return (((k - cb) % 2) + 2) % 2; }
constexpr int d_of(int k, int cb) { return (k - cb - phase_of(k, cb)) / 2; }
constexpr int dmin_of(int K, int cb) { int m = 1000; for (int k = 0; k < K; ++k) m = d_of(k, cb) < m ? d_of(k, cb) : m; return m; }
constexpr int dmax_of(int K, int cb) { int m = -1000; for (int k = 0; k < K; ++k) m = d_of(k, cb) > m ? d_of(k, cb) : m; return m; }

template <int K, int CBY, int CBX, int CK, int MT>
struct ConvTCfg {
    static constexpr int QROWS = 4;
    static constexpr int DMINY = dmin_of(K, CBY), DMAXY = dmax_of(K, CBY);
    static constexpr int DMINX = dmin_of(K, CBX), DMAXX = dmax_of(K, CBX);
    static constexpr int NDY = DMAXY - DMINY + 1, NDX = DMAXX - DMINX + 1;
    static constexpr int NR = QROWS + DMAXY - DMINY;
    static constexpr int NC = 32 + DMAXX - DMINX;
    static constexpr int PLANE = NR * NC;
    static constexpr int T = K * K;
    static constexpr int IN_ELEMS = CK * PLANE;
    static constexpr int MB = 32 * MT;
    static constexpr int W_ELEMS = CK * T * MB;
    static constexpr int IN_PT = (IN_ELEMS + 255) / 256;
    static constexpr int W_PT = (W_ELEMS + 255) / 256;
    static constexpr size_t LDS_BYTES = (size_t)(IN_ELEMS + W_ELEMS) * sizeof(float);
};

template <int K, int CBY, int CBX, int CK, int MT>
__global__ __launch_bounds__(256, (MT == 1 ? 2 : 1)) void convt_kernel(const ConvTParams p) {
    using C = ConvTCfg<K, CBY, CBX, CK, MT>;
    extern __shared__ __attribute__((aligned(16))) float smem[];
    float* s_in = smem;
    float* s_w = smem + C::IN_ELEMS;

    const int tid = threadIdx.x, lane = tid & 63, wv = tid >> 6;
    const int half = lane >> 5, l31 = lane & 31;
    int b = blockIdx.x;
    const int cb = b % p.co_blocks; b /= p.co_blocks;
    const int tx = b % p.tiles_x;   b /= p.tiles_x;
    const int ty = b % p.tiles_y;   b /= p.tiles_y;
    const int n = b;
    const int qx0 = tx * 32, qy0 = ty * C::QROWS, co0 = cb * C::MB;
    const int gy0 = qy0 - C::DMAXY, gx0 = qx0 - C::DMAXX;
    const float* xn = p.x + (size_t)n * p.cin * p.h * p.w_;

    float rin[C::IN_PT], rw[C::W_PT];
    unsigned in_off[C::IN_PT];
#pragma unroll
    for (int i = 0; i < C::IN_PT; ++i) {
        const int e = tid + i * 256;
        unsigned off = VCG_OOB;
        if (e < C::IN_ELEMS) {
            const int ci = e / C::PLANE, rem = e % C::PLANE;
            const int r = rem / C::NC, c = rem % C::NC;
            const int gy = gy0 + r, gx = gx0 + c;
            if (gy >= 0 && gy < p.h && gx >= 0 && gx < p.w_) off = 4u * (unsigned)((ci * p.h + gy) * p.w_ + gx);
        }
        in_off[i] = off;
    }
    const int hw = p.h * p.w_;
    unsigned w_off[C::W_PT];
#pragma unroll
    for (int i = 0; i < C::W_PT; ++i) {
        const int e = tid + i * 256;
        const int m = e % C::MB, q = e / C::MB;
        const int t = q % C::T, ci = q / C::T;
        const int col = co0 + m < p.cout ? co0 + m : p.cout - 1;
        w_off[i] = e < C::W_ELEMS ? 4u * (unsigned)((t * p.cin + ci) * p.cout + col) : VCG_OOB;
    }
    const size_t wbytes = (size_t)C::T * p.cin * p.cout * sizeof(float);
    auto load_chunk = [&](int ci0) {
        const vcg_rsrc rx = make_rsrc(xn + (size_t)ci0 * hw, (size_t)(p.cin - ci0) * hw * sizeof(float));
#pragma unroll
        for (int i = 0; i < C::IN_PT; ++i) rin[i] = buf_load(rx, in_off[i]);
        const vcg_rsrc rwt = make_rsrc(p.w + (size_t)ci0 * p.cout, wbytes - (size_t)ci0 * p.cout * sizeof(float));
#pragma unroll
        for (int i = 0; i < C::W_PT; ++i) rw[i] = buf_load(rwt, w_off[i]);
    };
    auto store_chunk = [&]() {
#pragma unroll
        for (int i = 0; i < C::IN_PT; ++i) {
            const int e = tid + i * 256;
            if (e < C::IN_ELEMS) s_in[e] = rin[i];
        }
#pragma unroll
        for (int i = 0; i < C::W_PT; ++i) {
            const int e = tid + i * 256;
            if (e < C::W_ELEMS) s_w[e] = rw[i];
        }
    };

    f32x16 acc[2][2][MT];
#pragma unroll
    for (int a = 0; a < 2; ++a)
#pragma unroll
        for (int c = 0; c < 2; ++c)
#pragma unroll
            for (int m = 0; m < MT; ++m)
#pragma unroll
                for (int r = 0; r < 16; ++r) acc[a][c][m][r] = 0.f;

    const float* bbase = s_in + half * C::PLANE + wv * C::NC + l31;
    const float* abase = s_w + half * C::T * C::MB + l31;

    const int nchunks = (p.cin + CK - 1) / CK;
    load_chunk(0);
    for (int c = 0; c < nchunks; ++c) {
        __syncthreads();
        store_chunk();
        __syncthreads();
        if (c + 1 < nchunks) load_chunk((c + 1) * CK);
#pragma unroll
        for (int cp = 0; cp < CK / 2; ++cp) {
            float bv[C::NDY][C::NDX];
#pragma unroll
            for (int iy = 0; iy < C::NDY; ++iy)
#pragma unroll
                for (int ix = 0; ix < C::NDX; ++ix)
                    bv[iy][ix] = bbase[cp * 2 * C::PLANE + (C::DMAXY - (C::DMINY + iy)) * C::NC +
                                       (C::DMAXX - (C::DMINX + ix))];
            float av[C::T][MT];
#pragma unroll
            for (int t = 0; t < C::T; ++t)
#pragma unroll
                for (int mt = 0; mt < MT; ++mt) av[t][mt] = abase[(cp * 2 * C::T + t) * C::MB + mt * 32];
#pragma unroll
            for (int ky = 0; ky < K; ++ky) {
#pragma unroll
                for (int kx = 0; kx < K; ++kx) {
                    const int t = ky * K + kx;
                    const int py = phase_of(ky, CBY), px = phase_of(kx, CBX);
                    const int iy = d_of(ky, CBY) - C::DMINY, ix = d_of(kx, CBX) - C::DMINX;
#pragma unroll
                    for (int mt = 0; mt < MT; ++mt) acc[py][px][mt] = mfma32(av[t][mt], bv[iy][ix], acc[py][px][mt]);
                }
            }
        }
    }

    const int qy = qy0 + wv, qx = qx0 + l31;
    const bool vec_ok = (p.ow % 2) == 0;
    const bool full = vec_ok && (co0 + C::MB <= p.cout) && (2 * (qy0 + C::QROWS) <= p.oh) && (2 * (qx0 + 32) <= p.ow);
    const int plane = p.oh * p.ow;
    const size_t img = (size_t)n * p.cout * plane;
    float* yimg = p.y + img;
    const float* rimg = p.residual ? p.residual + img : nullptr;
    const int ob = (co0 + 4 * half) * plane + (2 * qy) * p.ow + 2 * qx;
    const float* bp = p.bias ? p.bias : vcg_zero_word;
    const int bmask = p.bias ? ~0 : 0;
    const bool is_prelu = p.act == VCG_ACT_PRELU;
    const float* ap = is_prelu ? p.prelu : vcg_zero_word;
    const int amask = is_prelu ? ~0 : 0;
    const float slope_u = (p.act == VCG_ACT_LRELU) ? p.alpha : 1.f;
    auto emit = [&](auto guard_tag, auto res_tag) {
        constexpr bool GUARD = decltype(guard_tag)::value, RES = decltype(res_tag)::value;
#pragma unroll
        for (int mt = 0; mt < MT; ++mt) {
#pragma unroll
            for (int r = 0; r < 16; ++r) {
                const int row = mt * 32 + mfma_row(r, lane);
                const int co = co0 + row;
                const bool co_ok = !GUARD || co < p.cout;
                const int cs = co_ok ? co : co0;
                const float bvv = bp[cs & bmask];
                const float pa = ap[cs & amask];
                const float al = is_prelu ? pa : slope_u;
#pragma unroll
                for (int py = 0; py < 2; ++py) {
                    const int o = ob + (row - 4 * half) * plane + py * p.ow;
                    float v0 = acc[py][0][mt][r] + bvv, v1 = acc[py][1][mt][r] + bvv;
                    v0 = v0 >= 0.f ? v0 : v0 * al;
                    v1 = v1 >= 0.f ? v1 : v1 * al;
                    if (!GUARD) {
                        if (RES) { const float2 rr = *reinterpret_cast<const float2*>(rimg + o); v0 += rr.x; v1 += rr.y; }
                        *reinterpret_cast<float2*>(yimg + o) = make_float2(v0, v1);
                    } else {
                        const int oy = 2 * qy + py, ox = 2 * qx;
                        if (co_ok && oy < p.oh && ox < p.ow) {
                            if (vec_ok) {
                                if (RES) { const float2 rr = *reinterpret_cast<const float2*>(rimg + o); v0 += rr.x; v1 += rr.y; }
                                *reinterpret_cast<float2*>(yimg + o) = make_float2(v0, v1);
                            } else {
                                if (RES) v0 += rimg[o];
                                yimg[o] = v0;
                                if (ox + 1 < p.ow) {
                                    if (RES) v1 += rimg[o + 1];
                                    yimg[o + 1] = v1;
                                }
                            }
                        }
                    }
                }
            }
        }
    };
    using T_ = std::true_type;
    using F_ = std::false_type;
    if (full) {
        if (p.residual) emit(F_{}, T_{}); else emit(F_{}, F_{});
    } else {
        if (p.residual) emit(T_{}, T_{}); else emit(T_{}, F_{});
    }
}

template <int K, int CBY, int CBX, int CK, int MT>
int launch_convt(ConvTParams p, hipStream_t st) {
    using C = ConvTCfg<K, CBY, CBX, CK, MT>;
    p.tiles_x = ceil_div(ceil_div(p.ow, 2), 32);
    p.tiles_y = ceil_div(ceil_div(p.oh, 2), C::QROWS);
    p.co_blocks = ceil_div(p.cout, C::MB);
    const long grid = (long)p.tiles_x * p.tiles_y * p.co_blocks * p.n;
    if (grid <= 0 || grid > 0x7fffffffL) return VCG_E_SHAPE;
    auto kern = convt_kernel<K, CBY, CBX, CK, MT>;
    if (int e = vcg_allow_dyn_lds(reinterpret_cast<const void*>(kern), C::LDS_BYTES)) return e;
    hipLaunchKernelGGL(kern, dim3((int)grid), dim3(256), C::LDS_BYTES, st, p);
    VCG_LAUNCH_CHECK();
    return VCG_OK;
}

}

int vcg_internal_convt(const float* x, const float* w, float* y, int n, int cin, int h, int wd, int cout,
                       int oh, int ow, int k, int cby, int cbx, const vcg_epilogue* ep, hipStream_t st) {
    ConvTParams p{};
    p.x = x; p.w = w; p.y = y;
    p.bias = ep ? ep->bias : nullptr;
    p.prelu = ep ? ep->prelu_alpha : nullptr;
    p.residual = ep ? ep->residual : nullptr;
    p.act = ep ? ep->act : VCG_ACT_NONE;
    p.alpha = ep ? ep->act_alpha : 0.f;
    if (p.act == VCG_ACT_PRELU && p.prelu == nullptr) return VCG_E_NULL;
    if (p.act == VCG_ACT_TANH) return VCG_E_UNSUPPORTED;
    p.n = n; p.cin = cin; p.h = h; p.w_ = wd; p.cout = cout; p.oh = oh; p.ow = ow;
    if (n <= 0 || cin <= 0 || cout <= 0 || oh <= 0 || ow <= 0) return VCG_E_SHAPE;
#define VCG_CT(K_, A_, B_, CK_, MT_) if (k == K_ && cby == A_ && cbx == B_) return launch_convt<K_, A_, B_, CK_, MT_>(p, st)
    VCG_CT(3, 0, 0, 16, 1); VCG_CT(3, 0, 1, 16, 1); VCG_CT(3, 1, 0, 16, 1); VCG_CT(3, 1, 1, 16, 1);
    VCG_CT(4, 1, 1, 16, 1);
    VCG_CT(5, 1, 1, 8, 2); VCG_CT(5, 1, 2, 8, 2); VCG_CT(5, 2, 1, 8, 2); VCG_CT(5, 2, 2, 8, 2);
#undef VCG_CT
    return VCG_E_UNSUPPORTED;
}
```

video-cycle_gan-upscaling_amd/csrc/elementwise.hip:

```cpp
#include "vcg_common.hpp"

namespace {

constexpr int kSumSplitMax = 64;

inline int pick_split_cs(int c, size_t per_channel) {
    int s = 1;
    while (s < kSumSplitMax && (size_t)c * s < 1024 && per_channel / (s * 2) >= 2048) s *= 2;
    return s;
}

__device__ __forceinline__ float act_bwd_one(float s, float d, int act, float al, float& dal) {
    float g;
    if (act == VCG_ACT_TANH) g = 1.f - s * s;
    else if (act == VCG_ACT_LRELU) g = s > 0.f ? 1.f : al;
    else if (act == VCG_ACT_PRELU) { g = s > 0.f ? 1.f : al; dal += d * fminf(s, 0.f); }
    else g = 1.f;
    return d * g;
}

template <bool VEC>
__global__ __launch_bounds__(256) void act_bwd_kernel(const float* saved, const float* dy, int n, int c, int hw,
                                                      int act, float act_alpha, const float* prelu, float* dx,
                                                      float* part_alpha, float* part_sum ) {
    __shared__ float red[8];
    for (int plane = blockIdx.y; plane < n * c; plane += gridDim.y) {
    const int ch = plane % c;
    const float al = (act == VCG_ACT_PRELU) ? prelu[ch] : act_alpha;
    const size_t base = (size_t)plane * hw;
    float v[2] = {0.f, 0.f};
    if (VEC) {
        for (int i = (blockIdx.x * 256 + threadIdx.x) * 4; i < hw; i += gridDim.x * 1024) {
            const float4 s = *reinterpret_cast<const float4*>(saved + base + i);
            const float4 d = *reinterpret_cast<const float4*>(dy + base + i);
            float4 o;
            o.x = act_bwd_one(s.x, d.x, act, al, v[0]);
            o.y = act_bwd_one(s.y, d.y, act, al, v[0]);
            o.z = act_bwd_one(s.z, d.z, act, al, v[0]);
            o.w = act_bwd_one(s.w, d.w, act, al, v[0]);
            v[1] += (o.x + o.y) + (o.z + o.w);
            *reinterpret_cast<float4*>(dx + base + i) = o;
        }
    } else {
        for (int i = blockIdx.x * 256 + threadIdx.x; i < hw; i += gridDim.x * 256) {
            const float o = act_bwd_one(saved[base + i], dy[base + i], act, al, v[0]);
            v[1] += o;
            dx[base + i] = o;
        }
    }
    if (part_alpha || part_sum) {
        block_sum<2>(v, red);
        if (threadIdx.x == 0) {
            if (part_alpha) part_alpha[(size_t)plane * gridDim.x + blockIdx.x] = v[0];
            if (part_sum) part_sum[(size_t)plane * gridDim.x + blockIdx.x] = v[1];
        }
    }
    }
}

template <int AHEAD>
__device__ __forceinline__ void plane_chain(const float* part, int c, int ch, int per, int total, int& j, int& nn, int& k, float& s) {
    for (; j + AHEAD <= total; j += AHEAD) {
        float v[AHEAD];
#pragma unroll
        for (int u = 0; u < AHEAD; ++u) {
            v[u] = part[((size_t)nn * c + ch) * per + k];
            if (++k == per) { k = 0; ++nn; }
        }
#pragma unroll
        for (int u = 0; u < AHEAD; ++u) s += v[u];
    }
}

__global__ void plane_partial_final_kernel(const float* part, int n, int c, int per, float* out) {
    const int ch = blockIdx.x * blockDim.x + threadIdx.x;
    if (ch >= c) return;
    const int total = n * per;
    float s = 0.f;
    int nn = 0, k = 0, j = 0;
    plane_chain<32>(part, c, ch, per, total, j, nn, k, s);
    plane_chain<8>(part, c, ch, per, total, j, nn, k, s);
    plane_chain<1>(part, c, ch, per, total, j, nn, k, s);
    out[ch] = s;
}

__global__ __launch_bounds__(256) void channel_sum_partial_kernel(const float* x, int n, int c, int hw, int split,
                                                                  float* part ) {
    __shared__ float red[4];
    const int ch = blockIdx.x / split, s = blockIdx.x % split;
    const size_t M = (size_t)n * hw;
    const size_t per = (M + split - 1) / split;
    const size_t beg = (size_t)s * per, end = beg + per < M ? beg + per : M;
    float v[1] = {0.f};
    if (beg < end) {
        const size_t hws = (size_t)hw;
        const size_t n0 = beg / hws, n1 = (end - 1) / hws;
        for (size_t nn = n0; nn <= n1; ++nn) {
            const size_t lo = (beg > nn * hws ? beg : nn * hws) - nn * hws;
            const size_t hi = (end < (nn + 1) * hws ? end : (nn + 1) * hws) - nn * hws;
            const float* xp = x + (nn * c + ch) * hws;
            for (size_t r = lo + threadIdx.x; r < hi; r += 256) v[0] += xp[r];
        }
    }
    block_sum<1>(v, red);
    if (threadIdx.x == 0) part[(size_t)ch * split + s] = v[0];
}

__global__ void channel_sum_final_kernel(const float* part, int c, int split, float* out) {
    const int ch = blockIdx.x * blockDim.x + threadIdx.x;
    if (ch >= c) return;
    float s = 0.f;
    for (int k = 0; k < split; ++k) s += part[(size_t)ch * split + k];
    out[ch] = s;
}

constexpr int kRedBlocks = 1024;

__global__ __launch_bounds__(256) void sum_partial_kernel(const float* x, size_t count, float* part) {
    __shared__ float red[4];
    float v[1] = {0.f};
    for (size_t i = (size_t)blockIdx.x * 256 + threadIdx.x; i < count; i += (size_t)gridDim.x * 256) v[0] += x[i];
    block_sum<1>(v, red);
    if (threadIdx.x == 0) part[blockIdx.x] = v[0];
}

__global__ __launch_bounds__(256) void sum_final_kernel(const float* part, int nparts, float scale, float* out) {
    __shared__ float red[4];
    float v[1] = {0.f};
    for (int i = threadIdx.x; i < nparts; i += 256) v[0] += part[i];
    block_sum<1>(v, red);
    if (threadIdx.x == 0) out[0] = v[0] * scale;
}

__global__ __launch_bounds__(256) void pixel_loss_kernel(const float* pred, const float* target, size_t count, int kind,
                                                         float gscale, float* part, float* dpred) {
    __shared__ float red[4];
    float v[1] = {0.f};
    for (size_t i = (size_t)blockIdx.x * 256 + threadIdx.x; i < count; i += (size_t)gridDim.x * 256) {
        const float d = pred[i] - target[i];
        if (kind == VCG_LOSS_MSE) {
            v[0] += d * d;
            if (dpred) dpred[i] = 2.f * d * gscale;
        } else {
            v[0] += fabsf(d);
            if (dpred) dpred[i] = (d > 0.f ? 1.f : (d < 0.f ? -1.f : 0.f)) * gscale;
        }
    }
    block_sum<1>(v, red);
    if (threadIdx.x == 0) part[blockIdx.x] = v[0];
}

__global__ void fill_kernel(float* y, size_t count, float value) {
    const size_t i = (size_t)blockIdx.x * 256 + threadIdx.x;
    if (i < count) y[i] = value;
}

__global__ void axpby_kernel(const float* x, float* y, size_t count, float a, float b) {
    const size_t i = (size_t)blockIdx.x * 256 + threadIdx.x;
    if (i < count) y[i] = a * x[i] + (b == 0.f ? 0.f : b * y[i]);
}

__global__ __launch_bounds__(256) void adam_kernel(float* p, const float* g, float* m, float* v, size_t count,
                                                   float lr_t, float b1, float b2, float eps, float gscale) {
    const size_t i = (size_t)blockIdx.x * 256 + threadIdx.x;
    if (i >= count) return;
    const float gi = g[i] * gscale;
    const float mi = b1 * m[i] + (1.f - b1) * gi;
    const float vi = b2 * v[i] + (1.f - b2) * gi * gi;
    m[i] = mi;
    v[i] = vi;
    p[i] = p[i] - lr_t * mi / (sqrtf(vi) + eps);
}

__global__ void adam_lr_kernel(int* t_dev, float lr, float b1, float b2) {
    if (threadIdx.x != 0 || blockIdx.x != 0) return;
    const double t = (double)(t_dev[0] + 1);
    const double lr_t = (double)lr * sqrt(1.0 - pow((double)b2, t)) / (1.0 - pow((double)b1, t));
    ((float*)t_dev)[1] = (float)lr_t;
    t_dev[0] += 1;
}

__global__ __launch_bounds__(256) void adam_dev_kernel(float* p, const float* g, float* m, float* v, size_t count, float b1,
                                                       float b2, float eps, float gscale, const int* t_dev) {
    const size_t i = (size_t)blockIdx.x * 256 + threadIdx.x;
    if (i >= count) return;
// ... 201 lines not shown
                                  int oh, int ow) {
    const size_t total = planes * oh * ow;
    const size_t i = (size_t)blockIdx.x * 256 + threadIdx.x;
    if (i >= total) return;
    const int x = (int)(i % ow), y = (int)((i / ow) % oh);
    const size_t pl = i / ((size_t)ow * oh);
    if (PAD) {
        const int sy = y - top, sx = x - left;
        dst[i] = ((unsigned)sy < (unsigned)h && (unsigned)sx < (unsigned)w) ? src[(pl * h + sy) * w + sx] : 0.f;
    } else {
        dst[i] = src[(pl * h + y + top) * w + x + left];
    }
}

__global__ void copy_channels_kernel(const float* __restrict__ src, float* __restrict__ dst, int c_src, int c_src_off, int c_dst, int c_dst_off,
                                     int c_count, size_t hw, size_t total) {
    const size_t i = (size_t)blockIdx.x * 256 + threadIdx.x;
    if (i >= total) return;
    const size_t p = i % hw, c = (i / hw) % c_count, n = i / (hw * c_count);
    dst[(n * c_dst + c_dst_off + c) * hw + p] = src[(n * c_src + c_src_off + c) * hw + p];
}

__device__ __forceinline__ float hash_uniform(unsigned long long seed, unsigned long long step, unsigned long long idx) {
    unsigned long long z = seed + 0x9E3779B97F4A7C15ull * (step + 1) + 0xD1B54A32D192ED03ull * idx;
    z = (z ^ (z >> 30)) * 0xBF58476D1CE4E5B9ull;
    z = (z ^ (z >> 27)) * 0x94D049BB133111EBull;
    z ^= z >> 31;
    return (float)(unsigned)(z >> 40) * (1.0f / 16777216.0f);
}

__global__ void dropout_fwd_kernel(const float* __restrict__ x, float* __restrict__ y, unsigned char* __restrict__ mask, size_t count, float rate,
                                   unsigned long long seed, const unsigned long long* __restrict__ step) {
    const size_t i = (size_t)blockIdx.x * 256 + threadIdx.x;
    if (i >= count) return;
    const bool keep = hash_uniform(seed, step ? *step : 0ull, i) >= rate;
    mask[i] = keep ? 1 : 0;
    y[i] = keep ? x[i] / (1.0f - rate) : 0.f;
}

__global__ void dropout_bwd_kernel(const float* __restrict__ dy, const unsigned char* __restrict__ mask, float* __restrict__ dx, size_t count, float rate) {
    const size_t i = (size_t)blockIdx.x * 256 + threadIdx.x;
    if (i >= count) return;
    dx[i] = mask[i] ? dy[i] / (1.0f - rate) : 0.f;
}

__global__ void counter_inc_kernel(unsigned long long* c) { *c += 1; }

inline unsigned blocks_for(size_t count) { return (unsigned)((count + 255) / 256); }

}

extern "C" {

size_t vcg_act_bwd_workspace_bytes(int n, int c, int hw) { return (size_t)2 * n * c * 64 * sizeof(float); }

int vcg_act_bwd(const float* saved, const float* dy, int n, int c, int hw, int act, float act_alpha,
                const float* prelu_alpha, float* dx, float* dprelu_alpha, float* dsum, void* ws, size_t ws_bytes,
                vcg_stream_t stream) {
    VCG_CHECK_PTR(saved); VCG_CHECK_PTR(dy); VCG_CHECK_PTR(dx);
    if (n <= 0 || c <= 0 || hw <= 0 || (long)n * c > 0x7fffffffL) return VCG_E_SHAPE;
    if (act == VCG_ACT_PRELU && prelu_alpha == nullptr) return VCG_E_NULL;
    hipStream_t st = (hipStream_t)stream;
    const unsigned gy = (unsigned)((long)n * c > 65535 ? 65535 : n * c);
    int gx = ceil_div(hw, 256 * 4);
    if (gx > 64) gx = 64;
    if (gx < 1) gx = 1;
    float* part_alpha = nullptr;
    float* part_sum = nullptr;
    if (dprelu_alpha || dsum) {
        if (ws == nullptr || ws_bytes < vcg_act_bwd_workspace_bytes(n, c, hw)) return VCG_E_WORKSPACE;
        if (dprelu_alpha) part_alpha = (float*)ws;
        if (dsum) part_sum = (float*)ws + (size_t)n * c * 64;
    }
    if (hw % 4 == 0) {
        hipLaunchKernelGGL(act_bwd_kernel<true>, dim3(gx, gy), dim3(256), 0, st, saved, dy, n, c, hw, act,
                           act_alpha, prelu_alpha, dx, part_alpha, part_sum);
    } else {
        hipLaunchKernelGGL(act_bwd_kernel<false>, dim3(gx, gy), dim3(256), 0, st, saved, dy, n, c, hw, act,
                           act_alpha, prelu_alpha, dx, part_alpha, part_sum);
    }
    VCG_LAUNCH_CHECK();
    if (dprelu_alpha) {
        hipLaunchKernelGGL(plane_partial_final_kernel, dim3(ceil_div(c, 256)), dim3(256), 0, st, (const float*)part_alpha,
                           n, c, gx, dprelu_alpha);
        VCG_LAUNCH_CHECK();
    }
    if (dsum) {
        hipLaunchKernelGGL(plane_partial_final_kernel, dim3(ceil_div(c, 256)), dim3(256), 0, st, (const float*)part_sum, n,
                           c, gx, dsum);
        VCG_LAUNCH_CHECK();
    }
    return VCG_OK;
}

size_t vcg_channel_sum_workspace_bytes(int n, int c, int hw) { return (size_t)c * kSumSplitMax * sizeof(float); }

int vcg_channel_sum(const float* x, int n, int c, int hw, float* out, void* ws, size_t ws_bytes,
                    vcg_stream_t stream) {
    VCG_CHECK_PTR(x); VCG_CHECK_PTR(out); VCG_CHECK_PTR(ws);
    if (n <= 0 || c <= 0 || hw <= 0) return VCG_E_SHAPE;
    if (ws_bytes < vcg_channel_sum_workspace_bytes(n, c, hw)) return VCG_E_WORKSPACE;
    hipStream_t st = (hipStream_t)stream;
    const int split = pick_split_cs(c, (size_t)n * hw);
    hipLaunchKernelGGL(channel_sum_partial_kernel, dim3(c * split), dim3(256), 0, st, x, n, c, hw, split, (float*)ws);
    VCG_LAUNCH_CHECK();
    hipLaunchKernelGGL(channel_sum_final_kernel, dim3(ceil_div(c, 256)), dim3(256), 0, st, (const float*)ws, c, split,
                       out);
    VCG_LAUNCH_CHECK();
    return VCG_OK;
}

size_t vcg_mean_reduce_workspace_bytes(size_t count) { return kRedBlocks * sizeof(float); }

int vcg_mean_reduce(const float* x, size_t count, float* out, void* ws, size_t ws_bytes, vcg_stream_t stream) {
    VCG_CHECK_PTR(x); VCG_CHECK_PTR(out); VCG_CHECK_PTR(ws);
    if (count == 0) return VCG_E_SHAPE;
    if (ws_bytes < kRedBlocks * sizeof(float)) return VCG_E_WORKSPACE;
    hipStream_t st = (hipStream_t)stream;
    unsigned nb = blocks_for(count);
    if (nb > kRedBlocks) nb = kRedBlocks;
    hipLaunchKernelGGL(sum_partial_kernel, dim3(nb), dim3(256), 0, st, x, count, (float*)ws);
    VCG_LAUNCH_CHECK();
    hipLaunchKernelGGL(sum_final_kernel, dim3(1), dim3(256), 0, st, (const float*)ws, (int)nb, 1.f / (float)count, out);
    VCG_LAUNCH_CHECK();
    return VCG_OK;
}

int vcg_pixel_loss(const float* pred, const float* target, size_t count, int kind, float grad_scale, float* out,
                   float* dpred, void* ws, size_t ws_bytes, vcg_stream_t stream) {
    VCG_CHECK_PTR(pred); VCG_CHECK_PTR(target); VCG_CHECK_PTR(out); VCG_CHECK_PTR(ws);
    if (count == 0) return VCG_E_SHAPE;
    if (kind != VCG_LOSS_MSE && kind != VCG_LOSS_MAE) return VCG_E_UNSUPPORTED;
    if (ws_bytes < kRedBlocks * sizeof(float)) return VCG_E_WORKSPACE;
    hipStream_t st = (hipStream_t)stream;
    unsigned nb = blocks_for(count);
    if (nb > kRedBlocks) nb = kRedBlocks;
    hipLaunchKernelGGL(pixel_loss_kernel, dim3(nb), dim3(256), 0, st, pred, target, count, kind,
                       grad_scale / (float)count, (float*)ws, dpred);
    VCG_LAUNCH_CHECK();
    hipLaunchKernelGGL(sum_final_kernel, dim3(1), dim3(256), 0, st, (const float*)ws, (int)nb, 1.f / (float)count, out);
    VCG_LAUNCH_CHECK();
    return VCG_OK;
}

int vcg_head_act_fwd(const float* z, float* y, size_t count, int kind, vcg_stream_t stream) {
    VCG_CHECK_PTR(z); VCG_CHECK_PTR(y);
    if (kind < VCG_HEAD_NONE || kind > VCG_HEAD_BILOG) return VCG_E_UNSUPPORTED;
    if (count == 0) return VCG_OK;
    hipLaunchKernelGGL(head_act_fwd_kernel, dim3(blocks_for(count)), dim3(256), 0, (hipStream_t)stream, z, y, count, kind);
    VCG_LAUNCH_CHECK();
    return VCG_OK;
}

int vcg_head_act_bwd(const float* z, const float* dy, float* dz, size_t count, int kind, vcg_stream_t stream) {
    VCG_CHECK_PTR(z); VCG_CHECK_PTR(dy); VCG_CHECK_PTR(dz);
    if (kind < VCG_HEAD_NONE || kind > VCG_HEAD_BILOG) return VCG_E_UNSUPPORTED;
    if (count == 0) return VCG_OK;
    hipLaunchKernelGGL(head_act_bwd_kernel, dim3(blocks_for(count)), dim3(256), 0, (hipStream_t)stream, z, dy, dz, count, kind);
    VCG_LAUNCH_CHECK();
    return VCG_OK;
}

int vcg_gan_loss(const float* mean_a, const float* mean_b, float mean_scale, int kind, float* loss_out, float* da, size_t na,
                 float ga, float* db, size_t nb, float gb, vcg_stream_t stream) {
    VCG_CHECK_PTR(mean_a);
    if (kind < VCG_HEAD_NONE || kind > VCG_HEAD_BILOG) return VCG_E_UNSUPPORTED;
    if ((na && da == nullptr) || (nb && db == nullptr)) return VCG_E_NULL;
    const size_t most = na > nb ? na : nb;
    unsigned nbk = blocks_for(most ? most : 1);
    if (nbk > 1024) nbk = 1024;
    hipLaunchKernelGGL(gan_loss_kernel, dim3(nbk), dim3(256), 0, (hipStream_t)stream, mean_a, mean_b, mean_scale, kind, loss_out,
                       da, na, ga, db, nb, gb);
    VCG_LAUNCH_CHECK();
    return VCG_OK;
}

int vcg_sigmoid_gate_fwd(const float* a, const float* m, float* y, size_t count, vcg_stream_t stream) {
    VCG_CHECK_PTR(a); VCG_CHECK_PTR(m); VCG_CHECK_PTR(y);
    if (count == 0) return VCG_OK;
    hipLaunchKernelGGL(sigmoid_gate_fwd_kernel, dim3(blocks_for(count)), dim3(256), 0, (hipStream_t)stream, a, m, y, count);
    VCG_LAUNCH_CHECK();
    return VCG_OK;
}

int vcg_sigmoid_gate_bwd(const float* a, const float* m, const float* dy, float* da, float* dm, size_t count, vcg_stream_t stream) {
    VCG_CHECK_PTR(a); VCG_CHECK_PTR(m); VCG_CHECK_PTR(dy); VCG_CHECK_PTR(da); VCG_CHECK_PTR(dm);
    if (count == 0) return VCG_OK;
    hipLaunchKernelGGL(sigmoid_gate_bwd_kernel, dim3(blocks_for(count)), dim3(256), 0, (hipStream_t)stream, a, m, dy, da, dm, count);
    VCG_LAUNCH_CHECK();
    return VCG_OK;
}

int vcg_atanh_scale(const float* x, float* y, size_t count, float scale, vcg_stream_t stream) {
    VCG_CHECK_PTR(x); VCG_CHECK_PTR(y);
    if (count == 0) return VCG_OK;
    hipLaunchKernelGGL(atanh_scale_kernel, dim3(blocks_for(count)), dim3(256), 0, (hipStream_t)stream, x, y, count, scale);
    VCG_LAUNCH_CHECK();
    return VCG_OK;
}

int vcg_dilate2d(const float* src, float* dst, size_t planes, int h, int w, int stride, vcg_stream_t stream) {
    VCG_CHECK_PTR(src); VCG_CHECK_PTR(dst);
    if (planes == 0 || h <= 0 || w <= 0 || stride < 1) return VCG_E_SHAPE;
    const size_t total = planes * ((size_t)(h - 1) * stride + 1) * ((size_t)(w - 1) * stride + 1);
    hipLaunchKernelGGL(dilate2d_kernel, dim3(blocks_for(total)), dim3(256), 0, (hipStream_t)stream, src, dst, planes, h, w, stride);
    VCG_LAUNCH_CHECK();
    return VCG_OK;
}

int vcg_resize2d(const float* src, float* dst, size_t planes, int h, int w, int factor, int bilinear, vcg_stream_t stream) {
    VCG_CHECK_PTR(src); VCG_CHECK_PTR(dst);
    if (planes == 0 || h <= 0 || w <= 0 || factor < 1) return VCG_E_SHAPE;
    const size_t total = planes * (size_t)h * factor * w * factor;
    hipLaunchKernelGGL(resize2d_kernel, dim3(blocks_for(total)), dim3(256), 0, (hipStream_t)stream, src, dst, planes, h, w, factor, bilinear);
    VCG_LAUNCH_CHECK();
    return VCG_OK;
}

int vcg_crop2d(const float* src, float* dst, size_t planes, int h, int w, int top, int left, int oh, int ow, vcg_stream_t stream) {
    VCG_CHECK_PTR(src); VCG_CHECK_PTR(dst);
    if (planes == 0 || h <= 0 || w <= 0 || oh <= 0 || ow <= 0 || top < 0 || left < 0 || top + oh > h || left + ow > w) return VCG_E_SHAPE;
    hipLaunchKernelGGL(crop_pad2d_kernel<false>, dim3(blocks_for(planes * oh * ow)), dim3(256), 0, (hipStream_t)stream, src, dst, planes, h, w, top,
                       left, oh, ow);
    VCG_LAUNCH_CHECK();
    return VCG_OK;
}

int vcg_pad2d(const float* src, float* dst, size_t planes, int h, int w, int top, int left, int oh, int ow, vcg_stream_t stream) {
    VCG_CHECK_PTR(src); VCG_CHECK_PTR(dst);
    if (planes == 0 || h <= 0 || w <= 0 || oh <= 0 || ow <= 0 || top < 0 || left < 0 || top + h > oh || left + w > ow) return VCG_E_SHAPE;
    hipLaunchKernelGGL(crop_pad2d_kernel<true>, dim3(blocks_for(planes * oh * ow)), dim3(256), 0, (hipStream_t)stream, src, dst, planes, h, w, top,
                       left, oh, ow);
    VCG_LAUNCH_CHECK();
    return VCG_OK;
}

int vcg_copy_channels(const float* src, float* dst, int n, int c_src, int c_src_off, int c_dst, int c_dst_off, int c_count, size_t hw,
                      vcg_stream_t stream) {
    VCG_CHECK_PTR(src); VCG_CHECK_PTR(dst);
    if (n <= 0 || c_count <= 0 || hw == 0 || c_src_off < 0 || c_dst_off < 0 || c_src_off + c_count > c_src || c_dst_off + c_count > c_dst)
        return VCG_E_SHAPE;
    const size_t total = (size_t)n * c_count * hw;
    hipLaunchKernelGGL(copy_channels_kernel, dim3(blocks_for(total)), dim3(256), 0, (hipStream_t)stream, src, dst, c_src, c_src_off, c_dst, c_dst_off,
                       c_count, hw, total);
    VCG_LAUNCH_CHECK();
    return VCG_OK;
}

int vcg_dropout_fwd(const float* x, float* y, unsigned char* mask, size_t count, float rate, unsigned long long seed,
                    const unsigned long long* step, vcg_stream_t stream) {
    VCG_CHECK_PTR(x); VCG_CHECK_PTR(y); VCG_CHECK_PTR(mask);
    if (!(rate >= 0.f && rate < 1.f)) return VCG_E_SHAPE;
    if (count == 0) return VCG_OK;
    hipLaunchKernelGGL(dropout_fwd_kernel, dim3(blocks_for(count)), dim3(256), 0, (hipStream_t)stream, x, y, mask, count, rate, seed, step);
    VCG_LAUNCH_CHECK();
    return VCG_OK;
}

int vcg_dropout_bwd(const float* dy, const unsigned char* mask, float* dx, size_t count, float rate, vcg_stream_t stream) {
    VCG_CHECK_PTR(dy); VCG_CHECK_PTR(mask); VCG_CHECK_PTR(dx);
    if (!(rate >= 0.f && rate < 1.f)) return VCG_E_SHAPE;
    if (count == 0) return VCG_OK;
    hipLaunchKernelGGL(dropout_bwd_kernel, dim3(blocks_for(count)), dim3(256), 0, (hipStream_t)stream, dy, mask, dx, count, rate);
    VCG_LAUNCH_CHECK();
    return VCG_OK;
}

int vcg_counter_inc(unsigned long long* counter, vcg_stream_t stream) {
    VCG_CHECK_PTR(counter);
    hipLaunchKernelGGL(counter_inc_kernel, dim3(1), dim3(1), 0, (hipStream_t)stream, counter);
    VCG_LAUNCH_CHECK();
    return VCG_OK;
}

int vcg_fill(float* y, size_t count, float value, vcg_stream_t stream) {
    VCG_CHECK_PTR(y);
    if (count == 0) return VCG_OK;
    hipLaunchKernelGGL(fill_kernel, dim3(blocks_for(count)), dim3(256), 0, (hipStream_t)stream, y, count, value);
    VCG_LAUNCH_CHECK();
    return VCG_OK;
}

int vcg_axpby(const float* x, float* y, size_t count, float a, float b, vcg_stream_t stream) {
    VCG_CHECK_PTR(x); VCG_CHECK_PTR(y);
    if (count == 0) return VCG_OK;
    hipLaunchKernelGGL(axpby_kernel, dim3(blocks_for(count)), dim3(256), 0, (hipStream_t)stream, x, y, count, a, b);
    VCG_LAUNCH_CHECK();
    return VCG_OK;
}

int vcg_adam_keras_multi(float* p, const float* g, float* m, float* v, size_t count, float lr_t, float beta_1,
                         float beta_2, float eps, float grad_scale, vcg_stream_t stream) {
    VCG_CHECK_PTR(p); VCG_CHECK_PTR(g); VCG_CHECK_PTR(m); VCG_CHECK_PTR(v);
    if (count == 0) return VCG_OK;
    hipLaunchKernelGGL(adam_kernel, dim3(blocks_for(count)), dim3(256), 0, (hipStream_t)stream, p, g, m, v, count, lr_t,
                       beta_1, beta_2, eps, grad_scale);
    VCG_LAUNCH_CHECK();
    return VCG_OK;
}

int vcg_adam_keras_multi_dev(float* p, const float* g, float* m, float* v, size_t count, float lr, float beta_1,
                             float beta_2, float eps, float grad_scale, int* t_dev, vcg_stream_t stream) {
    VCG_CHECK_PTR(p); VCG_CHECK_PTR(g); VCG_CHECK_PTR(m); VCG_CHECK_PTR(v); VCG_CHECK_PTR(t_dev);
    hipStream_t st = (hipStream_t)stream;
    hipLaunchKernelGGL(adam_lr_kernel, dim3(1), dim3(64), 0, st, (int*)t_dev, lr, beta_1, beta_2);
    VCG_LAUNCH_CHECK();
// ... 73 lines not shown
```

video-cycle_gan-upscaling_amd/upscaler/_engine.py:

```python
import ctypes
import math
from collections import OrderedDict

import numpy as np
import torch

from . import _lib as L

BN_EPS = 1e-3
BN_MOMENTUM = 0.99
IN_EPS = 1e-5


def same_pads(size, k, s):
    out = -(-size // s)
    total = max((out - 1) * s + k - size, 0)
    return out, total // 2, total - total // 2


class Runtime:

    _inst = None

    def __init__(self):
# ... 120 lines not shown
def glorot_uniform(rng, shape, fan_in, fan_out):
    limit = math.sqrt(6.0 / (fan_in + fan_out))
    return rng.uniform(-limit, limit, size=shape).astype(np.float32)


class Layer:
    def __init__(self, name):
        self.name = name
        self.rt = None
        self.ps = None
        self.caches = []

    def bind(self, rt, ps):
        self.rt, self.ps = rt, ps

    def init_weights(self, rng):
        return {}

    def refresh(self):
        for c in self.caches:
            c.stale = True


class PackedOperand:

    def __init__(self, build, *layers):
        self.build, self.bufs, self.stale = build, None, True
        for l in layers:
            l.caches.append(self)

    def get(self):
        if self.stale:
            bufs = self.build(self.bufs)
            self.bufs = bufs if self.bufs is None else self.bufs
            self.stale = False
        return self.bufs


def act_bwd_bias(layer, y, dy, d, param_grads, which):
    rt = layer.rt
    hw = d.oh * d.ow
    dz = rt.empty(*dy.shape)
    db = layer.ps.grad(layer.name + "/bias", which).data_ptr() if param_grads else None
    ws, wsn = rt.workspace(rt.lib.vcg_act_bwd_workspace_bytes(d.n, layer.cout, hw))
    L.check(rt.lib.vcg_act_bwd(y.data_ptr(), dy.data_ptr(), d.n, layer.cout, hw, layer.act, float(layer.alpha),
                               None, dz.data_ptr(), None, db, ws, wsn, rt.stream), "vcg_act_bwd[%s]" % layer.name)
    return dz


def kernel_transpose(rt, w, taps, a, b, out=None):
    out = rt.empty(taps, b, a) if out is None else out
    L.check(rt.lib.vcg_kernel_transpose(w.data_ptr(), out.data_ptr(), taps, a, b, rt.stream), "vcg_kernel_transpose")
    return out


class Conv2D(Layer):

    def __init__(self, name, cin, cout, k, stride=1, padding="same", act=L.ACT_NONE, alpha=0.0):
        super().__init__(name)
        self.kh, self.kw = (int(k[0]), int(k[1])) if isinstance(k, (tuple, list)) else (int(k), int(k))
        self.cin, self.cout, self.k, self.stride, self.padding = cin, cout, self.kh, stride, padding
        self.act, self.alpha = act, alpha
        self._wt = PackedOperand(lambda out: kernel_transpose(self.rt, self.ps[self.name + "/kernel"], self.kh * self.kw, self.cin, self.cout, out), self)

    def declare(self, ps):
        ps.declare(self.name + "/kernel", (self.kh, self.kw, self.cin, self.cout))
        ps.declare(self.name + "/bias", (self.cout,))

    def init_weights(self, rng):
        t = self.kh * self.kw
        return {self.name + "/kernel": glorot_uniform(rng, (self.kh, self.kw, self.cin, self.cout), t * self.cin, t * self.cout),
                self.name + "/bias": np.zeros((self.cout,), np.float32)}

    def out_hw(self, h, w):
        kh, kw, s = self.kh, self.kw, self.stride
        if self.padding == "same":
            oh, pt, _ = same_pads(h, kh, s)
            ow, pl, _ = same_pads(w, kw, s)
        elif self.padding == "valid":
            oh, ow, pt, pl = (h - kh) // s + 1, (w - kw) // s + 1, 0, 0
        else:
            p = int(self.padding)
            oh, ow, pt, pl = (h + 2 * p - kh) // s + 1, (w + 2 * p - kw) // s + 1, p, p
        return oh, ow, pt, pl

    def desc(self, n, h, w):
        oh, ow, pt, pl = self.out_hw(h, w)
        return L.ConvDesc(n, self.cin, h, w, self.cout, oh, ow, self.kh, self.kw, self.stride, pt, pl)

    def forward(self, x, residual=None, tag=None):
        rt = self.rt
        n, _, h, w = x.shape
        d = self.desc(n, h, w)
        y = rt.empty(n, self.cout, d.oh, d.ow)
        ep = L.Epilogue(_ptr(self.ps[self.name + "/bias"]), self.act, float(self.alpha), None, _ptr(residual))
        with Timed(rt, tag):
            L.check(rt.lib.vcg_conv2d_fwd(ctypes.byref(d), x.data_ptr(), self.ps[self.name + "/kernel"].data_ptr(),
                                          y.data_ptr(), ctypes.byref(ep), rt.stream), "vcg_conv2d_fwd[%s]" % self.name)
        return y, (x, y if self.act != L.ACT_NONE else None, d)

    def forward_prelu(self, x, alpha, training=False, tag=None):
        if training or self.act != L.ACT_NONE:
            raise NotImplementedError("Conv2D.forward_prelu: the predict pass of a layer without an activation of its own")
        rt = self.rt
        n, _, h, w = x.shape
        d = self.desc(n, h, w)
        y = rt.empty(n, self.cout, d.oh, d.ow)
        ep = L.Epilogue(_ptr(self.ps[self.name + "/bias"]), L.ACT_PRELU, 0.0, alpha.data_ptr(), None)
        with Timed(rt, tag):
            L.check(rt.lib.vcg_conv2d_fwd(ctypes.byref(d), x.data_ptr(), self.ps[self.name + "/kernel"].data_ptr(),
                                          y.data_ptr(), ctypes.byref(ep), rt.stream), "vcg_conv2d_fwd[%s]" % self.name)
        return y

    def forward_folded(self, x, norm, residual=None, folded=None, tag=None):
        rt, ps = self.rt, self.ps
        if self.act != L.ACT_NONE or norm.norm != "batch":
            raise NotImplementedError("Conv2D.forward_folded: a convolution without activation in front of a BatchNormalization")
        n, _, h, w = x.shape
        d = self.desc(n, h, w)
        if folded is not None:
            scale, shift = folded
        else:
            scale, shift = finalize_batch(rt, [norm])[id(norm)]
        y = rt.empty(n, self.cout, d.oh, d.ow)
        ep = L.Epilogue(_ptr(ps[self.name + "/bias"]), norm.act, float(norm.alpha), norm._alpha_ptr(), _ptr(residual))
        with Timed(rt, tag):
            rc = rt.lib.vcg_conv2d_fwd_affine(ctypes.byref(d), x.data_ptr(), ps[self.name + "/kernel"].data_ptr(), y.data_ptr(), ctypes.byref(ep),
                                              scale.data_ptr(), shift.data_ptr(), rt.stream)
        if rc != L.E_UNSUPPORTED:
            L.check(rc, "vcg_conv2d_fwd_affine[%s]" % self.name)
            return y
        z, _ = self.forward(x, tag=tag)
        L.check(rt.lib.vcg_norm_act_fwd(z.data_ptr(), n, self.cout, d.oh * d.ow, scale.data_ptr(), shift.data_ptr(), 0, norm.act, float(norm.alpha),
                                        norm._alpha_ptr(), _ptr(residual), y.data_ptr(), rt.stream), "vcg_norm_act_fwd[%s]" % norm.name)
        return y

    def forward_stats(self, x, instance, tag=None):
        rt = self.rt
        n, _, h, w = x.shape
        d = self.desc(n, h, w)
        nrec = rt.lib.vcg_conv2d_stats_records(ctypes.byref(d), L.STATS_INSTANCE if instance else L.STATS_BATCH)
        if nrec <= 0 or self.act != L.ACT_NONE:
            y, ctx = self.forward(x, tag=tag)
            return y, ctx, None
        y = rt.empty(n, self.cout, d.oh, d.ow)
        total = nrec * (n if instance else 1)
        rec = rt.empty(total * 2 * self.cout)
        bias = self.ps[self.name + "/bias"]
        with Timed(rt, tag):
            L.check(rt.lib.vcg_conv2d_fwd_stats(ctypes.byref(d), x.data_ptr(), self.ps[self.name + "/kernel"].data_ptr(), bias.data_ptr(),
                                                y.data_ptr(), rec.data_ptr(), rt.stream), "vcg_conv2d_fwd_stats[%s]" % self.name)
        return y, (x, None, d), (rec, nrec, bias)

    def backward(self, ctx, dy, need_dx=True, param_grads=True, which=0, dx_residual=None, tag=None):
        rt = self.rt
        x, y, d = ctx
        n = d.n
        db_done = self.act != L.ACT_NONE
        if db_done:
            dy = act_bwd_bias(self, y, dy, d, param_grads, which)
        if param_grads:
            self._wgrad_fp32(d, x, dy, which, not db_done, tag)
        dx = None
        if need_dx:
            dx = rt.empty(n, self.cin, d.h, d.w)
            dd, dyd = d, dy
            if self.stride > 2:
                s = self.stride
                dyd = rt.empty(n, self.cout, (d.oh - 1) * s + 1, (d.ow - 1) * s + 1)
                L.check(rt.lib.vcg_dilate2d(dy.data_ptr(), dyd.data_ptr(), n * self.cout, d.oh, d.ow, s, rt.stream), "vcg_dilate2d")
                dd = L.ConvDesc(n, self.cin, d.h, d.w, self.cout, dyd.shape[2], dyd.shape[3], self.kh, self.kw, 1, d.pad_top, d.pad_left)
            with Timed(rt, tag and tag + "_dgrad"):
                L.check(rt.lib.vcg_conv2d_dgrad(ctypes.byref(dd), dyd.data_ptr(), self.ps[self.name + "/kernel"].data_ptr(),
                                                self._wt.get().data_ptr(), dx.data_ptr(), _ptr(dx_residual), rt.stream),
                        "vcg_conv2d_dgrad[%s]" % self.name)
        return dx

    def _wgrad_fp32(self, d, x, dy, which, with_bias, tag):
        rt = self.rt
        ws, wsn = rt.workspace(rt.lib.vcg_conv2d_wgrad_workspace_bytes(ctypes.byref(d)))
        with Timed(rt, tag and tag + "_wgrad"):
            L.check(rt.lib.vcg_conv2d_wgrad(ctypes.byref(d), x.data_ptr(), dy.data_ptr(), self.ps.grad(self.name + "/kernel", which).data_ptr(),
                                            self.ps.grad(self.name + "/bias", which).data_ptr() if with_bias else None, ws, wsn, rt.stream),
                    "vcg_conv2d_wgrad[%s]" % self.name)


class ConvT2D(Layer):

    def __init__(self, name, cin, cout, k, act=L.ACT_NONE, alpha=0.0):
        super().__init__(name)
        self.cin, self.cout, self.k, self.act, self.alpha = cin, cout, k, act, alpha
        self._wt = PackedOperand(lambda out: kernel_transpose(self.rt, self.ps[self.name + "/kernel"], k * k, cout, cin, out), self)

    def declare(self, ps):
        ps.declare(self.name + "/kernel", (self.k, self.k, self.cout, self.cin))
        ps.declare(self.name + "/bias", (self.cout,))

    def init_weights(self, rng):
        k = self.k
        return {self.name + "/kernel": glorot_uniform(rng, (k, k, self.cout, self.cin), k * k * self.cout, k * k * self.cin),
                self.name + "/bias": np.zeros((self.cout,), np.float32)}

    def desc(self, n, h, w):
        crop = max(self.k - 2, 0) // 2
        return L.ConvDesc(n, self.cin, h, w, self.cout, 2 * h, 2 * w, self.k, self.k, 2, crop, crop)

    def forward(self, x, tag=None):
        rt = self.rt
        n, _, h, w = x.shape
        d = self.desc(n, h, w)
        y = rt.empty(n, self.cout, d.oh, d.ow)
        ep = L.Epilogue(_ptr(self.ps[self.name + "/bias"]), self.act, float(self.alpha), None, None)
        with Timed(rt, tag):
            L.check(rt.lib.vcg_conv_transpose2d_fwd(ctypes.byref(d), x.data_ptr(), self._wt.get().data_ptr(), y.data_ptr(),
                                                    ctypes.byref(ep), rt.stream), "vcg_conv_transpose2d_fwd[%s]" % self.name)
        return y, (x, y if self.act != L.ACT_NONE else None, d)

    def backward(self, ctx, dy, need_dx=True, param_grads=True, which=0, tag=None):
        rt = self.rt
        x, y, d = ctx
        db_done = self.act != L.ACT_NONE
        if db_done:
            dy = act_bwd_bias(self, y, dy, d, param_grads, which)
        if param_grads:
            need = rt.lib.vcg_conv_transpose2d_wgrad_workspace_bytes(ctypes.byref(d))
            ws, wsn = rt.workspace(need)
            with Timed(rt, tag and tag + "_wgrad"):
                L.check(rt.lib.vcg_conv_transpose2d_wgrad(ctypes.byref(d), x.data_ptr(), dy.data_ptr(),
                                                          self.ps.grad(self.name + "/kernel", which).data_ptr(),
                                                          None if db_done else self.ps.grad(self.name + "/bias", which).data_ptr(),
                                                          ws, wsn, rt.stream), "vcg_conv_transpose2d_wgrad[%s]" % self.name)
        dx = None
        if need_dx:
            dx = rt.empty(d.n, self.cin, d.h, d.w)
            with Timed(rt, tag and tag + "_dgrad"):
                L.check(rt.lib.vcg_conv_transpose2d_dgrad(ctypes.byref(d), dy.data_ptr(),
                                                          self.ps[self.name + "/kernel"].data_ptr(), dx.data_ptr(), None,
                                                          rt.stream), "vcg_conv_transpose2d_dgrad[%s]" % self.name)
        return dx


class ConvTDilated(ConvT2D):

    def __init__(self, name, cin, cout, k, stride):
        super().__init__(name, cin, cout, k, L.ACT_NONE, 0.0)
        if k < stride:
            raise NotImplementedError("Conv2DTranspose with kernel_size < strides")
        self.stride = stride
        self._ones = None

    def _descs(self, n, h, w):
        s, k = self.stride, self.k
        hd, wd = (h - 1) * s + 1, (w - 1) * s + 1
        crop = (k - s) // 2
        return hd, wd, L.ConvDesc(n, self.cout, h * s, w * s, self.cin, hd, wd, k, k, 1, crop, crop)

    def forward(self, x, tag=None):
        rt = self.rt
        n, _, h, w = x.shape
        hd, wd, d = self._descs(n, h, w)
        xd = rt.empty(n, self.cin, hd, wd)
        L.check(rt.lib.vcg_dilate2d(x.data_ptr(), xd.data_ptr(), n * self.cin, h, w, self.stride, rt.stream), "vcg_dilate2d")
        z = rt.empty(n, self.cout, d.h, d.w)
        L.check(rt.lib.vcg_conv2d_dgrad(ctypes.byref(d), xd.data_ptr(), self.ps[self.name + "/kernel"].data_ptr(), self._wt.get().data_ptr(), z.data_ptr(),
                                        None, rt.stream), "vcg_conv2d_dgrad[%s]" % self.name)
        if self._ones is None:
            self._ones = filled_like(rt, self.ps[self.name + "/bias"], 1.0)
        y = rt.empty(*z.shape)
        L.check(rt.lib.vcg_norm_act_fwd(z.data_ptr(), n, self.cout, d.h * d.w, self._ones.data_ptr(), self.ps[self.name + "/bias"].data_ptr(), 0,
                                        L.ACT_NONE, 0.0, None, None, y.data_ptr(), rt.stream), "vcg_norm_act_fwd[%s]" % self.name)
        return y, (xd, d)

    def backward(self, ctx, dy, need_dx=True, param_grads=True, which=0, tag=None):
        rt = self.rt
        xd, d = ctx
        if need_dx:
            raise NotImplementedError("Conv2DTranspose(strides=%d): the input gradient is not built (the reference applies it to the network input)"
                                      % self.stride)
        if param_grads:
            ws, wsn = rt.workspace(max(rt.lib.vcg_conv2d_wgrad_workspace_bytes(ctypes.byref(d)),
                                       rt.lib.vcg_channel_sum_workspace_bytes(d.n, self.cout, d.h * d.w)))
            L.check(rt.lib.vcg_conv2d_wgrad(ctypes.byref(d), dy.data_ptr(), xd.data_ptr(), self.ps.grad(self.name + "/kernel", which).data_ptr(), None,
                                            ws, wsn, rt.stream), "vcg_conv2d_wgrad[%s]" % self.name)
            L.check(rt.lib.vcg_channel_sum(dy.data_ptr(), d.n, self.cout, d.h * d.w, self.ps.grad(self.name + "/bias", which).data_ptr(), ws, wsn,
                                           rt.stream), "vcg_channel_sum[%s]" % self.name)
        return None


def finalize_batch(rt, norms):
    out = {}
    by_c = {}
    for nm in norms:
        by_c.setdefault(nm.c, []).append(nm)
    for c, group in by_c.items():
        for at in range(0, len(group), 48):
            part = group[at:at + 48]
            n = len(part)
            buf = rt.empty(2, n, c)
            col = lambda key: (ctypes.c_void_p * n)(*[nm.ps[nm.name + key].data_ptr() for nm in part])
            L.check(rt.lib.vcg_norm_finalize_batch(col("/moving_mean"), col("/moving_variance"), col("/gamma"), col("/beta"), n, c, BN_EPS,
                                                   buf[0].data_ptr(), buf[1].data_ptr(), rt.stream), "vcg_norm_finalize_batch")
            for i, nm in enumerate(part):
                out[id(nm)] = (buf[0, i], buf[1, i])
    return out


class NormAct(Layer):

    def __init__(self, name, c, norm="batch", act=L.ACT_NONE, alpha=0.0, prelu_name=None):
        super().__init__(name)
        self.c, self.norm, self.act, self.alpha, self.prelu_name = c, norm, act, alpha, prelu_name

    def declare(self, ps):
        if self.norm == "batch":
            ps.declare(self.name + "/gamma", (self.c,))
            ps.declare(self.name + "/beta", (self.c,))
            ps.declare(self.name + "/moving_mean", (self.c,), trainable=False)
            ps.declare(self.name + "/moving_variance", (self.c,), trainable=False)
        if self.act == L.ACT_PRELU:
            ps.declare(self.prelu_name + "/alpha", (self.c,))

    def init_weights(self, rng):
        w = {}
        if self.norm == "batch":
            w[self.name + "/gamma"] = np.ones((self.c,), np.float32)
            w[self.name + "/beta"] = np.zeros((self.c,), np.float32)
            w[self.name + "/moving_mean"] = np.zeros((self.c,), np.float32)
            w[self.name + "/moving_variance"] = np.ones((self.c,), np.float32)
        if self.act == L.ACT_PRELU:
            w[self.prelu_name + "/alpha"] = np.zeros((self.c,), np.float32)
        return w

    def _alpha_ptr(self):
        return self.ps[self.prelu_name + "/alpha"].data_ptr() if self.act == L.ACT_PRELU else None

    def needs_stats(self, training):
        return self.norm is not None and bool(training or self.norm == "instance")

    STATS, ACT_FWD, ACT_BWD = "vcg_norm_stats", "vcg_norm_act_fwd", "vcg_norm_act_bwd"

    def _dims(self, x):
        if x.dim() == 4:
            n, c, h, w = x.shape
            return n, c, h * w
        n, c = x.shape
        return n, c, 1

    def _like(self, x):
        return self.rt.empty(*x.shape)

    def _finalize_partials(self, stats, rows, c, count, gamma, beta, eps, mean, scale, shift, invstd, mm, mv, unbiased_n):
        buf, nrec, kshift = stats
        L.check(self.rt.lib.vcg_norm_finalize_partials_shifted(buf.data_ptr(), nrec, rows, c, count, kshift.data_ptr(), gamma, beta, eps,
                                                               mean.data_ptr(), scale.data_ptr(), shift.data_ptr(), invstd.data_ptr(), mm, mv,
                                                               BN_MOMENTUM, unbiased_n, self.rt.stream),
                "vcg_norm_finalize_partials_shifted[%s]" % self.name)

    def forward(self, x, training, residual=None, update_moving=True, stats=None):
        rt, ps = self.rt, self.ps
        lib = rt.lib
        n, c, hw = self._dims(x)
        y = self._like(x)
        saved = None
        act_fwd = getattr(lib, self.ACT_FWD)
        if self.norm is None:
            L.check(act_fwd(x.data_ptr(), n, c, hw, None, None, 0, self.act, float(self.alpha),
                            self._alpha_ptr(), _ptr(residual), y.data_ptr(), rt.stream), self.ACT_FWD)
            return y, (x, None, None, (n, c, hw))
        inst = self.norm == "instance"
        rows = n if inst else 1
        mode = L.NORM_INSTANCE if inst else L.NORM_BATCH
        scale, shift, invstd = rt.empty(rows * c), rt.empty(rows * c), rt.empty(rows * c)
        gamma = None if inst else ps[self.name + "/gamma"].data_ptr()
        beta = None if inst else ps[self.name + "/beta"].data_ptr()
        eps = IN_EPS if inst else BN_EPS
# ... 829 lines not shown
```

video-cycle_gan-upscaling_amd/upscaler/_lib.py:

```python
import ctypes
import os
from ctypes import POINTER, c_char_p, c_float, c_int, c_int32, c_size_t, c_void_p

_PKG_DIR = os.path.dirname(os.path.dirname(os.path.abspath(__file__)))
LIB_PATH = os.path.join(_PKG_DIR, "libvcg_hip.so")

ACT_NONE, ACT_LRELU, ACT_PRELU, ACT_TANH = 0, 1, 2, 3
NORM_BATCH, NORM_INSTANCE = 0, 1
LOSS_MSE, LOSS_MAE = 0, 1
HEAD_NONE, HEAD_SIGMOID, HEAD_LOGSIGM, HEAD_TANH, HEAD_BILOG = 0, 1, 2, 3, 4
HEAD_KINDS = {None: 0, "none": 0, "sigmoid": 1, "log-sigm": 2, "tanh": 3, "bi-log": 4}


class ConvDesc(ctypes.Structure):
    _fields_ = [(k, c_int32) for k in ("n", "cin", "h", "w", "cout", "oh", "ow", "kh", "kw", "stride",
                                       "pad_top", "pad_left")]


class Epilogue(ctypes.Structure):
    _fields_ = [("bias", c_void_p), ("act", c_int32), ("act_alpha", c_float), ("prelu_alpha", c_void_p),
                ("residual", c_void_p)]


FINAL9X9_WFRAG_BYTES = (4 * 9 * 4 * 64 + 4) * 16
FIRST9X9_WFRAG_BYTES = 27 * 64 * 2 * 16


class EpilogueBf16(ctypes.Structure):
    _fields_ = [("scale", c_void_p), ("shift", c_void_p), ("act", c_int32), ("act_alpha", c_float),
                ("prelu_alpha", c_void_p), ("residual", c_void_p), ("stats", c_void_p), ("stats_mode", c_int32)]


STATS_NONE, STATS_BATCH, STATS_INSTANCE = 0, 1, 2
E_UNSUPPORTED = -3
OUT_F32_NCHW, OUT_U8_NHWC = 0, 1

_P = c_void_p
_D = POINTER(ConvDesc)
_E = POINTER(Epilogue)
_EB = POINTER(EpilogueBf16)
SIGNATURES = {
    "vcg_version": (c_char_p, []),
    "vcg_error_string": (c_char_p, [c_int]),
    "vcg_conv2d_fwd": (c_int, [_D, _P, _P, _P, _E, _P]),
    "vcg_conv2d_dgrad": (c_int, [_D, _P, _P, _P, _P, _P, _P]),
    "vcg_conv2d_fwd_affine": (c_int, [_D, _P, _P, _P, _E, _P, _P, _P]),
    "vcg_norm_finalize_batch": (c_int, [_P, _P, _P, _P, c_int, c_int, c_float, _P, _P, _P]),
    "vcg_conv2d_wgrad_workspace_bytes": (c_size_t, [_D]),
    "vcg_conv2d_wgrad": (c_int, [_D, _P, _P, _P, _P, _P, c_size_t, _P]),
    "vcg_conv_transpose2d_fwd": (c_int, [_D, _P, _P, _P, _E, _P]),
    "vcg_conv_transpose2d_dgrad": (c_int, [_D, _P, _P, _P, _P, _P]),
    "vcg_conv_transpose2d_wgrad_workspace_bytes": (c_size_t, [_D]),
    "vcg_conv_transpose2d_wgrad": (c_int, [_D, _P, _P, _P, _P, _P, c_size_t, _P]),
    "vcg_kernel_transpose": (c_int, [_P, _P, c_int, c_int, c_int, _P]),
    "vcg_norm_stats_workspace_bytes": (c_size_t, [c_int, c_int, c_int, c_int]),
    "vcg_norm_stats": (c_int, [_P, c_int, c_int, c_int, c_int, _P, _P, _P, c_size_t, _P]),
    "vcg_norm_finalize": (c_int, [_P, _P, _P, _P, c_int, c_int, c_float, _P, _P, _P, _P, _P, c_float, c_int, _P]),
    "vcg_sum_records": (c_int, [_P, c_int, c_int, c_float, _P, _P]),
    "vcg_bn_fold": (c_int, [_P, _P, _P, _P, _P, c_int, c_float, _P, _P, _P]),
    "vcg_norm_finalize_partials": (c_int, [_P, c_int, c_int, c_int, ctypes.c_double, _P, _P, c_float, _P, _P, _P, _P, _P, _P, c_float, c_int, _P]),
    "vcg_norm_finalize_partials_shifted": (c_int, [_P, c_int, c_int, c_int, ctypes.c_double, _P, _P, _P, c_float, _P, _P, _P, _P, _P, _P, c_float, c_int, _P]),
    "vcg_conv2d_stats_records": (c_int, [_D, c_int]),
    "vcg_conv2d_fwd_stats": (c_int, [_D, _P, _P, _P, _P, _P, _P]),
    "vcg_norm_act_fwd": (c_int, [_P, c_int, c_int, c_int, _P, _P, c_int, c_int, c_float, _P, _P, _P, _P]),
    "vcg_norm_act_bwd_workspace_bytes": (c_size_t, [c_int, c_int, c_int, c_int]),
    "vcg_norm_act_bwd": (c_int, [_P, _P, c_int, c_int, c_int, c_int, _P, _P, _P, _P, c_int, c_float, _P, c_int,
                                 _P, _P, _P, _P, _P, c_size_t, _P]),
    "vcg_act_bwd_workspace_bytes": (c_size_t, [c_int, c_int, c_int]),
    "vcg_act_bwd": (c_int, [_P, _P, c_int, c_int, c_int, c_int, c_float, _P, _P, _P, _P, _P, c_size_t, _P]),
    "vcg_channel_sum_workspace_bytes": (c_size_t, [c_int, c_int, c_int]),
    "vcg_channel_sum": (c_int, [_P, c_int, c_int, c_int, _P, _P, c_size_t, _P]),
    "vcg_dense_fwd": (c_int, [_P, _P, _P, _P, c_int, c_int, c_int, _P]),
    "vcg_dense_dgrad": (c_int, [_P, _P, _P, c_int, c_int, c_int, _P]),
    "vcg_dense_wgrad": (c_int, [_P, _P, _P, _P, c_int, c_int, c_int, _P]),
    "vcg_mean_reduce_workspace_bytes": (c_size_t, [c_size_t]),
    "vcg_mean_reduce": (c_int, [_P, c_size_t, _P, _P, c_size_t, _P]),
    "vcg_pixel_loss": (c_int, [_P, _P, c_size_t, c_int, c_float, _P, _P, _P, c_size_t, _P]),
    "vcg_dilate2d": (c_int, [_P, _P, c_size_t, c_int, c_int, c_int, _P]),
    "vcg_resize2d": (c_int, [_P, _P, c_size_t, c_int, c_int, c_int, c_int, _P]),
    "vcg_crop2d": (c_int, [_P, _P, c_size_t, c_int, c_int, c_int, c_int, c_int, c_int, _P]),
    "vcg_pad2d": (c_int, [_P, _P, c_size_t, c_int, c_int, c_int, c_int, c_int, c_int, _P]),
    "vcg_copy_channels": (c_int, [_P, _P, c_int, c_int, c_int, c_int, c_int, c_int, c_size_t, _P]),
    "vcg_dropout_fwd": (c_int, [_P, _P, _P, c_size_t, c_float, ctypes.c_uint64, _P, _P]),
    "vcg_dropout_bwd": (c_int, [_P, _P, _P, c_size_t, c_float, _P]),
    "vcg_counter_inc": (c_int, [_P, _P]),
    "vcg_fill": (c_int, [_P, c_size_t, c_float, _P]),
    "vcg_axpby": (c_int, [_P, _P, c_size_t, c_float, c_float, _P]),
    "vcg_adam_keras_multi": (c_int, [_P, _P, _P, _P, c_size_t, c_float, c_float, c_float, c_float, c_float, _P]),
    "vcg_adam_keras_multi_dev": (c_int, [_P, _P, _P, _P, c_size_t, c_float, c_float, c_float, c_float, c_float, _P, _P]),
    "vcg_sigmoid_gate_fwd": (c_int, [_P, _P, _P, c_size_t, _P]),
    "vcg_sigmoid_gate_bwd": (c_int, [_P, _P, _P, _P, _P, c_size_t, _P]),
    "vcg_atanh_scale": (c_int, [_P, _P, c_size_t, c_float, _P]),
    "vcg_head_act_fwd": (c_int, [_P, _P, c_size_t, c_int, _P]),
    "vcg_head_act_bwd": (c_int, [_P, _P, _P, c_size_t, c_int, _P]),
    "vcg_gan_loss": (c_int, [_P, _P, c_float, c_int, _P, _P, c_size_t, c_float, _P, c_size_t, c_float, _P]),
    "vcg_frames_u8_to_nchw": (c_int, [_P, _P, c_int, c_int, c_int, c_int, _P]),
    "vcg_nchw_to_frames_u8": (c_int, [_P, _P, c_int, c_int, c_int, c_int, _P]),
    "vcg_nhwc_to_nchw": (c_int, [_P, _P, c_int, c_int, c_int, c_int, _P]),
    "vcg_nchw_to_nhwc": (c_int, [_P, _P, c_int, c_int, c_int, c_int, _P]),
    "vcg_maxpool2x2_fwd": (c_int, [_P, _P, c_int, c_int, c_int, c_int, _P]),
    "vcg_maxpool2x2_bwd": (c_int, [_P, _P, _P, c_int, c_int, c_int, c_int, _P]),
    "vcg_pack_conv_kernel_bf16": (c_int, [_P, c_int, c_int, c_int, c_int, c_int, _P, _P]),
    "vcg_f32_nchw_to_bf16_nhwc": (c_int, [_P, _P, c_int, c_int, c_int, c_int, _P]),
    "vcg_bf16_nhwc_to_f32_nchw": (c_int, [_P, _P, c_int, c_int, c_int, c_int, _P]),
    "vcg_conv2d_bf16_fwd": (c_int, [_D, _P, _P, _P, _EB, _P]),
    "vcg_conv2d_bf16_stats_records": (c_int, [_D, c_int32]),
    "vcg_conv_transpose2d_bf16_fwd": (c_int, [_D, _P, _P, _P, _EB, _P]),
    "vcg_norm_stats_bf16_workspace_bytes": (c_size_t, [c_int, c_int, c_int, c_int]),
    "vcg_norm_stats_bf16": (c_int, [_P, c_int, c_int, c_int, c_int, _P, _P, _P, c_size_t, _P]),
    "vcg_norm_act_fwd_bf16": (c_int, [_P, c_int, c_int, c_int, _P, _P, c_int, c_int, c_float, _P, _P, _P, _P]),
    "vcg_norm_act_bwd_bf16_workspace_bytes": (c_size_t, [c_int, c_int, c_int, c_int]),
    "vcg_norm_act_bwd_bf16": (c_int, [_P, _P, c_int, c_int, c_int, c_int, _P, _P, _P, _P, c_int, c_float, _P, c_int, _P, _P, _P, _P, _P,
                                      c_size_t, _P]),
    "vcg_pack_conv3x3_c64_bf16_batch": (c_int, [_P, c_int, _P, _P]),
    "vcg_bn_fold_batch": (c_int, [_P, _P, _P, _P, _P, c_int, c_int, c_float, _P, _P, _P]),
    "vcg_conv3ch_bf16_wfrag_bytes": (c_size_t, [c_int, c_int, c_int]),
    "vcg_pack_conv3ch_bf16": (c_int, [_P, c_int, c_int, c_int, _P, _P]),
    "vcg_conv3ch_bf16_fwd": (c_int, [_D, _P, _P, _P, c_float, _P, _P]),
    "vcg_conv3ch_bf16_dgrad_workspace_bytes": (c_size_t, [_D]),
    "vcg_conv3ch_bf16_dgrad": (c_int, [_D, _P, _P, _P, _P, c_size_t, _P]),
    "vcg_conv3ch_bf16_wgrad_workspace_bytes": (c_size_t, [_D]),
    "vcg_conv3ch_bf16_wgrad": (c_int, [_D, _P, _P, _P, _P, _P, c_size_t, _P]),
    "vcg_conv9x9_from3_bf16_fwd_train": (c_int, [_D, _P, _P, _P, _P, _P, _P, _P]),
    "vcg_prelu_bwd_nhwc_bf16_records": (c_int, [c_int, c_int]),
    "vcg_prelu_bwd_nhwc_bf16": (c_int, [_P, _P, _P, _P, c_int, c_int, c_int, _P, _P, _P]),
    "vcg_prelu_bwd_nhwc_bf16_to_bf16": (c_int, [_P, _P, _P, _P, c_int, c_int, c_int, _P, _P, _P]),
    "vcg_conv2d_cout1_nhwc_bf16_fwd": (c_int, [_D, _P, _P, _P, _P, _P]),
    "vcg_conv2d_cout1_nhwc_bf16_dgrad": (c_int, [_D, _P, _P, _P, _P]),
    "vcg_conv2d_cout1_nhwc_bf16_wgrad_workspace_bytes": (c_size_t, [_D]),
    "vcg_conv2d_cout1_nhwc_bf16_wgrad": (c_int, [_D, _P, _P, _P, _P, _P, c_size_t, _P]),
    "vcg_conv2d_bf16_wgrad_workspace_bytes": (c_size_t, [_D]),
    "vcg_conv2d_bf16_wgrad": (c_int, [_D, _P, _P, _P, _P, _P, c_size_t, _P]),
    "vcg_conv9x9_to3_bf16_wgrad_workspace_bytes": (c_size_t, [_D]),
    "vcg_conv9x9_to3_bf16_wgrad": (c_int, [_D, _P, _P, _P, _P, c_size_t, _P]),
    "vcg_pack_first9x9_bf16": (c_int, [_P, _P, _P]),
    "vcg_pack_conv9x9_3ch_bf16": (c_int, [_P, c_int, c_int, _P, _P]),
    "vcg_conv9x9_to3_bf16_dgrad": (c_int, [_D, _P, _P, _P, c_float, _P, _P]),
    "vcg_conv9x9_to3_bf16_dgrad_chsum_records": (c_int, [_D]),
    "vcg_conv9x9_to3_bf16_dgrad_chsum": (c_int, [_D, _P, _P, _P, c_float, _P, _P, _P]),
    "vcg_conv9x9_from3_bf16_fwd": (c_int, [_D, _P, _P, _P, _P, _P, _P]),
    "vcg_pack_final9x9_bf16": (c_int, [_P, _P, _P]),
    "vcg_conv9x9_to3_bf16_fwd": (c_int, [_D, _P, _P, _P, c_int, _P, _P]),
    "vcg_conv9x9_to3_bf16_fwd_window": (c_int, [_D, _P, _P, _P, c_int, c_int, _P, c_int, c_int, c_int, c_int, _P]),
    "vcg_conv9x9_to3_bf16_wfrag_bytes": (c_size_t, [c_int]),
    "vcg_pack_conv9x9_to3_bf16": (c_int, [_P, c_int, _P, _P]),
    "vcg_conv9x9_c64to3_bf16_wfrag_bytes": (c_size_t, []),
    "vcg_pack_conv9x9_c64to3_bf16": (c_int, [_P, _P, _P]),
    "vcg_conv9x9_c64to3_bf16_fwd": (c_int, [_D, _P, _P, _P, c_int, _P, _P]),
    "vcg_conv9x9_c64to3_bf16_fwd_window": (c_int, [_D, _P, _P, _P, c_int, c_int, _P, c_int, c_int, c_int, c_int, _P]),
    "vcg_conv_in_gate_bf16_wfrag_bytes": (c_size_t, [c_int, c_int, c_int, c_int]),
    "vcg_pack_conv_in_gate_bf16": (c_int, [_P, c_int, c_int, c_int, c_int, _P, _P]),
    "vcg_conv_in_gate_bf16_fwd": (c_int, [_D, _P, _P, _P, _P, _P, _P]),
    "vcg_input_convt_add_bf16": (c_int, [_D, _P, _P, _P, _P, _P]),
    "vcg_conv_frag_bf16_bytes": (c_size_t, [c_int, c_int, c_int]),
    "vcg_pack_conv_frag_bf16": (c_int, [_P, c_int, c_int, c_int, c_int, _P, _P]),
    "vcg_pack_conv_frag_bf16_pair": (c_int, [_P, c_int, c_int, c_int, _P, _P, _P]),
    "vcg_conv2d_nhwc_bf16_fwd": (c_int, [_D, _P, _P, _P, c_int, c_float, _P, _P]),
    "vcg_conv2d_nhwc_bf16_stats_records": (c_int, [_D, c_int]),
    "vcg_conv2d_nhwc_bf16_fwd_stats": (c_int, [_D, _P, _P, _P, _P, _P, _P]),
    "vcg_conv_transpose2d_nhwc_bf16_fwd": (c_int, [_D, _P, _P, _P, c_int, c_float, _P, _P]),
    "vcg_conv2d_nhwc_bf16_dgrad": (c_int, [_D, _P, _P, _P, c_float, _P, _P]),
    "vcg_conv2d_nhwc_bf16_dgrad_add": (c_int, [_D, _P, _P, _P, _P, _P]),
    "vcg_conv2d_nhwc_bf16_wgrad_workspace_bytes": (c_size_t, [_D]),
    "vcg_conv2d_nhwc_bf16_wgrad": (c_int, [_D, _P, _P, _P, _P, _P, c_size_t, _P]),
    "vcg_conv_transpose2d_nhwc_bf16_wgrad_workspace_bytes": (c_size_t, [_D]),
    "vcg_conv_transpose2d_nhwc_bf16_wgrad": (c_int, [_D, _P, _P, _P, _P, c_size_t, _P]),
    "vcg_lrelu_bwd_bf16": (c_int, [_P, _P, c_float, _P, c_size_t, _P]),
    "vcg_bf16_to_f32": (c_int, [_P, _P, c_size_t, _P]),
    "vcg_f32_to_bf16": (c_int, [_P, _P, c_size_t, _P]),
}

_lib = None


def bind(lib):
    for name, (res, args) in SIGNATURES.items():
        fn = getattr(lib, name)
        fn.restype = res
        fn.argtypes = args
    return lib


def load():
    global _lib
    if _lib is not None:
        return _lib
    if not os.path.exists(LIB_PATH):
        raise RuntimeError(
            "libvcg_hip.so not found at %s: build it with `python %s` (hipcc, gfx950). "
            "There is no CPU fallback for the hot path." % (LIB_PATH, os.path.join(_PKG_DIR, "build.py")))
    try:
        lib = ctypes.CDLL(LIB_PATH)
    except OSError as e:
        raise RuntimeError("cannot load %s: %s" % (LIB_PATH, e))
    _lib = bind(lib)
    return lib


class VcgError(RuntimeError):
    pass


def check(rc, what):
    if rc != 0:
        msg = load().vcg_error_string(int(rc)).decode()
        if rc < 0:
            raise ValueError("%s: %s (code %d)" % (what, msg, rc))
        raise VcgError("%s: HIP error %d: %s" % (what, rc, msg))


def require_gpu():
    import torch
    if not torch.cuda.is_available():
        raise RuntimeError("no HIP device visible: the hot path runs only on an MI355X (gfx950) GPU; "
                           "there is no CPU fallback")
    return torch.device("cuda", torch.cuda.current_device())
```

video-cycle_gan-upscaling_amd/upscaler/model.py:

```python
import math
from abc import ABCMeta, abstractmethod
from collections import OrderedDict

import numpy as np
import torch

from . import _engine as E
from . import _lib as L


class Adam:

    def __init__(self, lr=0.001, beta_1=0.9, beta_2=0.999, epsilon=1e-7, decay=0.0, amsgrad=False):
        if decay != 0.0 or amsgrad:
            raise NotImplementedError("Adam(decay/amsgrad) is outside the hot path")
        self.lr, self.beta_1, self.beta_2, self.epsilon = lr, beta_1, beta_2, epsilon
        self.iterations = 0

    def lr_t(self):
        t = self.iterations + 1
        lr, b1, b2 = (float(np.float32(v)) for v in (self.lr, self.beta_1, self.beta_2))
        return lr * math.sqrt(1.0 - b2 ** t) / (1.0 - b1 ** t)


# ... 211 lines not shown
    @property
    def output_shape(self):
        return (None,) + tuple(self._out_shape(self._in_shape))

    def count_params(self):
        return self.ps.count_params()

    def get_weights_dict(self):
        return self.ps.get_weights()

    def set_weights_dict(self, weights):
        missing = self.ps.set_weights(weights)
        if missing:
            raise KeyError("missing weights: %s" % missing[:5])
        self.refresh()

    from_reference_weights = set_weights_dict

    def refresh(self):
        for l in self.layers:
            l.refresh()

    def save(self, path):
        from safetensors.numpy import save_file
        save_file({k: v for k, v in self.ps.get_weights().items()}, path,
                  metadata={"format": "vcg-amd", "name": str(self.name), "input_shape": repr(self._in_shape)})

    def load_weights(self, path):
        from safetensors.numpy import load_file
        self.set_weights_dict(load_file(path))

    def predict(self, x, batch_size=32):
        rt = self.rt
        is_torch = isinstance(x, torch.Tensor)
        n = x.shape[0]
        outs = []
        for i in range(0, n, batch_size):
            xb = E.to_device_nchw(rt, x[i:i + batch_size])
            y, _ = self.forward(xb, training=False)
            outs.append(self._export(y))
        out = outs[0] if len(outs) == 1 else torch.cat(outs, 0)
        return out if is_torch else out.cpu().numpy()

    def _export(self, y):
        return E.to_nhwc(self.rt, y) if y.dim() == 4 else y

    def __call__(self, x):
        return self.predict(x)


class VGG19Features(Model):

    def __init__(self, image_shape, weights="random", seed=19):
        super().__init__("vgg19_block5_conv4", image_shape, seed)
        self.trainable = False
        self.stages = []
        cin = image_shape[2]
        for b, nconv, f in VGG19_BLOCKS:
            convs = []
            for i in range(nconv):
                convs.append(self._add(E.Conv2D("block%d_conv%d" % (b, i + 1), cin, f, 3, act=L.ACT_LRELU, alpha=0.0)))
                cin = f
            self.stages.append((convs, b < 5))
        self._finish()
        if isinstance(weights, str) and weights == "random":
            rng = np.random.RandomState(seed)
            w, cin = {}, image_shape[2]
            for b, nconv, f in VGG19_BLOCKS:
                for i in range(nconv):
                    lim = np.sqrt(6.0 / (9 * cin))
                    w["block%d_conv%d/kernel" % (b, i + 1)] = rng.uniform(-lim, lim, (3, 3, cin, f)).astype(np.float32)
                    w["block%d_conv%d/bias" % (b, i + 1)] = rng.uniform(-0.05, 0.05, (f,)).astype(np.float32)
                    cin = f
            self.set_weights_dict(w)
        elif isinstance(weights, dict):
            self.set_weights_dict({k: np.asarray(v, np.float32) for k, v in weights.items()})
        else:
            path = str(weights)
            if path.endswith(".npz"):
                self.set_weights_dict({k: v.astype(np.float32) for k, v in np.load(path).items()})
            else:
                self.load_weights(path)

    def _out_shape(self, s):
        return (s[0] // 16, s[1] // 16, 512)

    def forward(self, x, training=False):
        tape = []
        h = x
        for convs, pool in self.stages:
            for c in convs:
                h, a = c.forward(h, tag="vgg_conv")
                tape.append(a)
            if pool:
                tape.append(h)
                h = E.maxpool2x2(self.rt, h)
        return h, tape

    def backward_data(self, tape, dy):
        tape = list(tape)
        d = dy
        for convs, pool in reversed(self.stages):
            if pool:
                d = E.maxpool2x2_bwd(self.rt, tape.pop(), d)
            for c in reversed(convs):
                d = c.backward(tape.pop(), d, True, False, 0, tag="vgg_conv")
        return d


class UpscalerOrig(Model):

    def __init__(self, output_image_shape, kernel_size, filters, upscale_factor, res_block_num, norm, seed, trunk_dtype="fp32"):
        f = upscale_factor
        super().__init__("upscaler_orig", (output_image_shape[0] // f, output_image_shape[1] // f, output_image_shape[2]), seed)
        if trunk_dtype not in ("fp32", "bf16", "bf16+tail"):
            raise ValueError(trunk_dtype)
        self.tail_bf16 = trunk_dtype == "bf16+tail"
        if self.tail_bf16:
            trunk_dtype = "bf16"
            if upscale_factor < 2 or upscale_factor & (upscale_factor - 1):
                raise NotImplementedError("the bf16 tail is instantiated for power-of-two upscale_factor >= 2")
        if trunk_dtype == "bf16" and (kernel_size not in (3, 5) or filters != 64):
            raise NotImplementedError("the bf16 trunk is instantiated for kernel_size 3 or 5, filters=64")
        self.trunk_dtype = trunk_dtype
        bf = trunk_dtype == "bf16"
        trunk_conv = E.Conv3x3Bf16 if kernel_size == 3 else E.Conv5x5Bf16
        conv = (lambda n, ci, co, kk: trunk_conv(n, ci, co)) if bf else (lambda n, ci, co, kk: E.Conv2D(n, ci, co, kk))
        normact = E.NormActBf16 if bf else E.NormAct
        self.upscale_times = int(math.log(f, 2))
        self.factor = 2 ** self.upscale_times
        k = kernel_size
        nrm = {"batch": "batch", "instance": "instance"}[norm]
        self.init_bf16 = bool(self.tail_bf16 and output_image_shape[2] == 3)
        self.c_init = self._add((E.InitialConv9x9Bf16 if self.init_bf16 else E.Conv2D)("initial/conv", output_image_shape[2], filters, 9))
        self.a_init = self._add(E.NormAct("initial/prelu_op", filters, None, L.ACT_PRELU, prelu_name="initial/prelu"))
        self.blocks = []
        for i in range(res_block_num):
            n = "res_block/%d" % i
            self.blocks.append((
                self._add(conv(n + "/conv_pre", filters, filters, k)),
                self._add(normact(n + "/batch_norm_pre", filters, nrm, L.ACT_PRELU, prelu_name=n + "/prelu")),
                self._add(conv(n + "/conv_post", filters, filters, k)),
                self._add(normact(n + "/batch_norm_post", filters, nrm)),
            ))
        self.c_pre = self._add(conv("prefinal/conv2d", filters, 64, k))
        self.n_pre = self._add(normact("prefinal/batch_norm", 64, nrm))
        self.ups = []
        cin = 64
        upc = (E.ConvT3x3Bf16 if k == 3 and self.upscale_times == 1 else E.ConvTBf16) if self.tail_bf16 else E.ConvT2D
        for i in range(self.upscale_times):
            self.ups.append(self._add(upc("upscaling/%d/block/conv_transp" % i, cin, 256, k, L.ACT_LRELU, 0.2)))
            cin = 256
        self.c_fin = self._add(E.FinalConv9x9Bf16("final/conv", cin, 3, 9) if self.tail_bf16 else E.Conv2D("final/conv", cin, 3, 9, act=L.ACT_TANH))
        self._finish()
        if bf and k == 3 and len(self.blocks) * 2 + 1 <= 48:
            E.PackGroup3x3([c for b in self.blocks for c in (b[0], b[2])] + [self.c_pre])

    def _out_shape(self, s):
        return (s[0] * self.factor, s[1] * self.factor, 3)

    def to_inference_bf16(self):
        from ._infer import Bf16Generator
        return Bf16Generator(self)

    def forward(self, x, training):
        tape = []
        if self.init_bf16:
            h, c = self.c_init.forward_prelu(x, self.ps[self.a_init.prelu_name + "/alpha"], training); tape.extend((c, None))
        else:
            if training or self.trunk_dtype == "bf16":
                h, c = self.c_init.forward(x); tape.append(c)
                h, c = self.a_init.forward(h, training); tape.append(c)
            else:
                h = self.c_init.forward_prelu(x, self.ps[self.a_init.prelu_name + "/alpha"]); tape.extend((None, None))
            if self.trunk_dtype == "bf16":
                h = E.to_bf16_nhwc(self.rt, h)
        skip = h
        bf = self.trunk_dtype == "bf16"
        folds = {}
        if bf and not training and self.n_pre.norm == "batch" and len(self.blocks) * 2 + 1 <= 48:
            folds = E.fold_batch(self.rt, [p for b in self.blocks for p in ((b[0], b[1]), (b[2], b[3]))] + [(self.c_pre, self.n_pre)])
        fold32 = not bf and not training and self.n_pre.norm == "batch"
        if fold32:
            f32 = E.finalize_batch(self.rt, [nm for b in self.blocks for nm in (b[1], b[3])] + [self.n_pre])
            folds = {id(cv): f32[id(nm)] for cv, nm in [p for b in self.blocks for p in ((b[0], b[1]), (b[2], b[3]))] + [(self.c_pre, self.n_pre)]}

        def conv_norm(cv, nm, h, residual=None):
            if bf and not training and nm.norm == "batch":
                tape.extend((None, None))
                return cv.forward_folded(h, nm, residual=residual, tag="trunk_conv", folded=folds.get(id(cv)))
            if fold32:
                tape.extend((None, None))
                return cv.forward_folded(h, nm, residual=residual, folded=folds.get(id(cv)), tag="trunk_conv")
            if nm.needs_stats(training):
                h, a, st = cv.forward_stats(h, nm.norm == "instance", tag="trunk_conv"); tape.append(a)
                h, a = nm.forward(h, training, residual=residual, stats=st); tape.append(a)
            else:
                h, a = cv.forward(h, tag="trunk_conv"); tape.append(a)
                h, a = nm.forward(h, training, residual=residual); tape.append(a)
            return h

        for (c1, n1, c2, n2) in self.blocks:
            gen = h
            h = conv_norm(c1, n1, h)
            h = conv_norm(c2, n2, h, residual=gen)
        h = conv_norm(self.c_pre, self.n_pre, h, residual=skip)
        if self.trunk_dtype == "bf16" and not self.tail_bf16:
            h = E.from_bf16_nhwc(self.rt, h)
        for u in self.ups:
            h, a = u.forward(h, tag="convt"); tape.append(a)
        h, a = self.c_fin.forward(h, tag="final_conv"); tape.append(a)
        return h, tape

    def backward(self, tape, dy, which=0):
        rt = self.rt
        tape = list(tape)
        if self.tail_bf16:
            d, sums = self.c_fin.backward(tape.pop(), dy, True, True, which, tag="final_conv", input_lrelu_slope=self.ups[-1].alpha,
                                          want_channel_sums=True)
            for i in range(len(self.ups) - 1, -1, -1):
                kw = {"input_lrelu_slope": self.ups[i - 1].alpha} if i else {}
                d = self.ups[i].backward(tape.pop(), d, True, True, which, tag="convt", dz_channel_sums=sums, **kw)
                sums = None
        else:
            d = self.c_fin.backward(tape.pop(), dy, True, True, which, tag="final_conv")
            for u in reversed(self.ups):
                d = u.backward(tape.pop(), d, True, True, which, tag="convt")
        if self.init_bf16:
            dskip = d
        elif self.tail_bf16:
            dskip = E.from_bf16_nhwc(rt, d)
        else:
            dskip = d
            if self.trunk_dtype == "bf16":
                d = E.to_bf16_nhwc(rt, d)
        d = self.n_pre.backward(tape.pop(), d, True, which)
        d = self.c_pre.backward(tape.pop(), d, True, True, which, tag="trunk_conv")
        for (c1, n1, c2, n2) in reversed(self.blocks):
            dres = d
            d = n2.backward(tape.pop(), d, True, which)
            d = c2.backward(tape.pop(), d, True, True, which, tag="trunk_conv")
            d = n1.backward(tape.pop(), d, True, which)
            d = c1.backward(tape.pop(), d, True, True, which, dx_residual=dres, tag="trunk_conv")
        if self.init_bf16:
            tape.pop()
            self.c_init.backward_prelu(tape.pop(), d, dskip, self.ps[self.a_init.prelu_name + "/alpha"],
                                       self.ps.grad(self.a_init.prelu_name + "/alpha", which), which)
            return None
        if self.trunk_dtype == "bf16":
            d = E.from_bf16_nhwc(rt, d)
        E.axpby(rt, dskip, d, 1.0, 1.0)
        d = self.a_init.backward(tape.pop(), d, True, which)
        self.c_init.backward(tape.pop(), d, False, True, which)
        return None


class DiscriminatorStack(Model):

    def __init__(self, input_shape, filters, activation, seed, name, dtype="fp32", kernel=3, strides=None, padding="same", dense1=1024):
        super().__init__(name, input_shape, seed)
        if dtype not in ("fp32", "bf16"):
            raise ValueError(dtype)
        strides = strides or (1,) + (2,) * (len(filters) - 1)
        self.dtype = dtype
        self.activation = activation
        self.head = L.HEAD_KINDS.get(activation, L.HEAD_NONE)
        self.convs = []
        cin = input_shape[2]
        h, w = input_shape[0], input_shape[1]
        for i, f in enumerate(filters):
            n = "discriminator/block_%d" % (i + 1)
            s = strides[i]
            first_bf = dtype == "bf16" and i == 0 and cin == 3 and f % 64 == 0 and (kernel, s) == (3, 1)
            bf = dtype == "bf16" and (i > 0 or first_bf)
            conv = E.FirstConvBf16 if first_bf else E.Conv2DBf16 if bf else E.Conv2D
            norm = E.NormActBf16 if bf else E.NormAct
            cv = self._add(conv(n + "/Conv2d", cin, f, kernel, s, padding))
            self.convs.append((cv, self._add(norm(n + "/BatchNorm", f, "batch", L.ACT_LRELU, 0.1))))
            h, w, _, _ = cv.out_hw(h, w)
            if h < 1 or w < 1:
                raise ValueError("input %s is too small for %s" % (tuple(input_shape), name))
            cin = f
        self.first_bf16 = isinstance(self.convs[0][0], E.FirstConvBf16)
        self.flat = (h, w, cin)
        self.d1 = self._add(E.Dense("discriminator/final/Dense_1", h * w * cin, dense1))
        self.b1 = self._add(E.NormAct("discriminator/final/BatchNorm_1", dense1, "batch", L.ACT_LRELU, 0.1))
        self.d2 = self._add(E.Dense("discriminator/final/Dense_2", dense1, 32))
        self.b2 = self._add(E.NormAct("discriminator/final/BatchNorm_2", 32, "batch", L.ACT_LRELU, 0.1))
        self.d3 = self._add(E.Dense("discriminator/final/Dense_3", 32, 1))
        self._finish()

    def _out_shape(self, s):
        return (1,)

    @property
    def output_shape(self):
        return (None, 1)

    def forward(self, x, training, update_moving=True):
        if tuple(x.shape[2:]) != tuple(self._in_shape[:2]):
            raise ValueError("discriminator built for %s, got %s" % (self._in_shape[:2], tuple(x.shape[2:])))
        rt = self.rt
        bf = self.dtype == "bf16"
        tape = []
        h = x
        for i, (cv, na) in enumerate(self.convs):
            if bf and i == 1 and not self.first_bf16:
                h = E.to_bf16_nhwc(rt, h)
            if i > 0 and na.needs_stats(training) and cv.act == L.ACT_NONE:
                h, a, st = cv.forward_stats(h, False, tag="d_conv"); tape.append(a)
                h, a = na.forward(h, training, update_moving=update_moving, stats=st); tape.append(a)
                continue
            h, a = cv.forward(h, tag="d_conv"); tape.append(a)
            h, a = na.forward(h, training, update_moving=update_moving); tape.append(a)
        if bf and len(self.convs) > 1:
            tape.append(tuple(h.shape))
            hf = E.bf16_to_f32(rt, h)
        else:
            hf = E.to_nhwc(rt, h)
            tape.append(tuple(h.shape))
        h = hf.view(hf.shape[0], -1)
        for dn, bn in ((self.d1, self.b1), (self.d2, self.b2)):
            h, a = dn.forward(h); tape.append(a)
            h, a = bn.forward(h, training, update_moving=update_moving); tape.append(a)
        h, a = self.d3.forward(h); tape.append(a)
        if self.head:
            tape.append(h)
            h = E.head_act_fwd(self.rt, h, self.head)
        return h, tape

    def backward(self, tape, dy, need_dx=False, param_grads=True, which=0):
        rt = self.rt
        bf = self.dtype == "bf16" and len(self.convs) > 1
        tape = list(tape)
        if self.head:
            dy = E.head_act_bwd(rt, tape.pop(), dy, self.head)
        d = self.d3.backward(tape.pop(), dy, True, param_grads, which)
        for dn, bn in ((self.d2, self.b2), (self.d1, self.b1)):
            d = bn.backward(tape.pop(), d, param_grads, which)
            d = dn.backward(tape.pop(), d, True, param_grads, which)
        shp = tape.pop()
        if bf:
            d = E.f32_to_bf16(rt, d).view(*shp)
        else:
            n, c, h, w = shp
            dn_ = rt.empty(n, c, h, w)
            L.check(rt.lib.vcg_nhwc_to_nchw(d.data_ptr(), dn_.data_ptr(), n, h, w, c, rt.stream), "vcg_nhwc_to_nchw")
            d = dn_
        for i, (cv, na) in reversed(list(enumerate(self.convs))):
            d = na.backward(tape.pop(), d, param_grads, which)
            d = cv.backward(tape.pop(), d, need_dx or i > 0, param_grads, which, tag="d_conv")
            if bf and i == 1 and not self.first_bf16:
                d = E.from_bf16_nhwc(rt, d)
        return d


class DiscriminatorPatchGAN(Model):
    SPEC = ((64, 2, False), (128, 2, True), (256, 2, True), (512, 1, True), (1, 1, False))

    def __init__(self, input_shape, activation, norm, seed, dtype="fp32"):
        super().__init__("discriminator_patchgan_70", input_shape, seed)
        if dtype not in ("fp32", "bf16"):
            raise ValueError(dtype)
        self.dtype = dtype
        self.activation = activation
        self.head = L.HEAD_KINDS.get(activation, L.HEAD_NONE)
        self.convs = []
        cin = input_shape[2]
        for i, (f, s, has_norm) in enumerate(self.SPEC):
            n = "discriminator/block_%d" % (i + 1)
            last = i == len(self.SPEC) - 1
            if has_norm:
                bf = dtype == "bf16"
                cv = self._add((E.Conv2DBf16 if bf else E.Conv2D)(n + "/Conv2d", cin, f, 4, s, 1))
                na = self._add((E.NormActBf16 if bf else E.NormAct)(n + "/BatchNorm", f, norm, L.ACT_LRELU, 0.2))
            elif i == 0 and dtype == "bf16" and cin == 3:
                cv = self._add(E.FirstConvBf16(n + "/Conv2d", cin, f, 4, s, 1, L.ACT_LRELU, 0.2))
                na = None
            elif last and dtype == "bf16":
                cv = self._add(E.ConvCout1Bf16(n + "/Conv2d", cin, f, 4, s, 1))
# ... 545 lines not shown
```

Baseline: 137.0 frames/s.

## Fuse LeakyReLU backward into final conv dgrad via bitmask from last conv-transpose

```diff
diff --git a/include/vcg.h b/include/vcg.h
--- a/include/vcg.h
+++ b/include/vcg.h
@@ -58,6 +58,12 @@
                              const vcg_epilogue* ep, vcg_stream_t stream);
 int vcg_conv_transpose2d_dgrad(const vcg_conv_desc* d, const float* dy, const float* w_hwoi, float* dx,
                                const float* residual, vcg_stream_t stream);
+
+size_t vcg_lrelu_mask_bytes(int n, int cout, int oh, int ow);
+int vcg_conv_transpose2d_fwd_mask(const vcg_conv_desc* d, const float* x, const float* w_hwio_t, float* y, const vcg_epilogue* ep, void* mask,
+                                  vcg_stream_t stream);
+int vcg_conv2d_dgrad_lrelu_mask(const vcg_conv_desc* d, const float* dy, const float* w_hwio, const float* w_hwoi, float* dx, const void* mask,
+                                float slope, vcg_stream_t stream);
 size_t vcg_conv_transpose2d_wgrad_workspace_bytes(const vcg_conv_desc* d);
 int vcg_conv_transpose2d_wgrad(const vcg_conv_desc* d, const float* x, const float* dy, float* dw_hwoi,
                                float* dbias, void* ws, size_t ws_bytes, vcg_stream_t stream);
@@ -98,6 +104,7 @@
 int vcg_act_bwd(const float* saved, const float* dy, int n, int c, int hw, int act, float act_alpha,
                 const float* prelu_alpha, float* dx, float* dprelu_alpha, float* dsum, void* ws, size_t ws_bytes,
                 vcg_stream_t stream);
+int vcg_act_bwd_dsum(const float* dz, int n, int c, int hw, float* dsum, void* ws, size_t ws_bytes, vcg_stream_t stream);
 size_t vcg_channel_sum_workspace_bytes(int n, int c, int hw);
 int vcg_channel_sum(const float* x, int n, int c, int hw, float* out, void* ws, size_t ws_bytes,
                     vcg_stream_t stream);
diff --git a/video-cycle_gan-upscaling_amd/csrc/api.hip b/video-cycle_gan-upscaling_amd/csrc/api.hip
--- a/video-cycle_gan-upscaling_amd/csrc/api.hip
+++ b/video-cycle_gan-upscaling_amd/csrc/api.hip
@@ -3,9 +3,9 @@
 int vcg_internal_conv(const float* x, const float* w, float* y, int n, int cin, int h, int wd, int cout, int oh,
                       int ow, int kh, int kw, int stride, int pad_top, int pad_left, int flip, const vcg_epilogue* ep,
                       int smallm, int ws_t, int ws_m, int ws_k, hipStream_t st, float* stats = nullptr, const float* scale = nullptr,
-                      const float* shift = nullptr);
+                      const float* shift = nullptr, const unsigned* mask = nullptr);
 int vcg_internal_convt(const float* x, const float* w, float* y, int n, int cin, int h, int wd, int cout, int oh,
-                       int ow, int k, int cby, int cbx, const vcg_epilogue* ep, hipStream_t st);
+                       int ow, int k, int cby, int cbx, const vcg_epilogue* ep, hipStream_t st, unsigned* mask = nullptr);
 size_t vcg_internal_wgrad_ws(int n, int mtot, int ah, int aw, int jctot, int kh, int kw, int S);
 int vcg_internal_wgrad(const float* A, const float* B, float* dw, float* db, int n, int mtot, int ah, int aw,
                        int jctot, int bh, int bw, int kh, int kw, int S, int pt, int pl_, int flip, int ts, int sm,
@@ -124,6 +124,21 @@
                               d->pad_left, &ep, st);
 }
 
+int vcg_conv2d_dgrad_lrelu_mask(const vcg_conv_desc* d, const float* dy, const float* w_hwio, const float* w_hwoi, float* dx, const void* mask,
+                                float slope, vcg_stream_t stream) {
+    int rc = check_desc(d);
+    if (rc) return rc;
+    VCG_CHECK_PTR(dy); VCG_CHECK_PTR(dx); VCG_CHECK_PTR(mask); VCG_CHECK_PTR(w_hwoi);
+    (void)w_hwio;
+    if (d->stride != 1 || d->kh != 9 || d->kw != 9 || d->cout > 3 || d->pad_top != 4 || d->pad_left != 4 || d->oh != d->h || d->ow != d->w ||
+        use_smallm(d->cin, d->kh, d->kw, 1))
+        return VCG_E_UNSUPPORTED;
+    vcg_epilogue ep{};
+    ep.act_alpha = slope;
+    return vcg_internal_conv(dy, w_hwoi, dx, d->n, d->cout, d->oh, d->ow, d->cin, d->h, d->w, 9, 9, 1, 4, 4, 1, &ep, 0, 0, 0, 0, (hipStream_t)stream,
+                             nullptr, nullptr, nullptr, (const unsigned*)mask);
+}
+
 size_t vcg_conv2d_wgrad_workspace_bytes(const vcg_conv_desc* d) {
     if (check_desc(d)) return 0;
     size_t a;
@@ -169,6 +184,22 @@
                               d->pad_left, ep, (hipStream_t)stream);
 }
 
+size_t vcg_lrelu_mask_bytes(int n, int cout, int oh, int ow) {
+    if (n <= 0 || cout <= 0 || oh <= 0 || ow <= 0) return 0;
+    return (size_t)n * ceil_div(cout, 32) * ceil_div(oh, 8) * ceil_div(ow, 64) * 2048;
+}
+
+int vcg_conv_transpose2d_fwd_mask(const vcg_conv_desc* d, const float* x, const float* w_hwio_t, float* y, const vcg_epilogue* ep, void* mask,
+                                  vcg_stream_t stream) {
+    int rc = check_desc(d);
+    if (rc) return rc;
+    VCG_CHECK_PTR(x); VCG_CHECK_PTR(w_hwio_t); VCG_CHECK_PTR(y); VCG_CHECK_PTR(ep); VCG_CHECK_PTR(mask);
+    if (d->stride != 2 || d->kh != d->kw) return VCG_E_UNSUPPORTED;
+    if (d->oh > 2 * d->h || d->ow > 2 * d->w) return VCG_E_SHAPE;
+    return vcg_internal_convt(x, w_hwio_t, y, d->n, d->cin, d->h, d->w, d->cout, d->oh, d->ow, d->kh, d->pad_top, d->pad_left, ep,
+                              (hipStream_t)stream, (unsigned*)mask);
+}
+
 int vcg_conv_transpose2d_dgrad(const vcg_conv_desc* d, const float* dy, const float* w_hwoi, float* dx,
                                const float* residual, vcg_stream_t stream) {
     int rc = check_desc(d);
diff --git a/video-cycle_gan-upscaling_amd/csrc/conv_fwd.hip b/video-cycle_gan-upscaling_amd/csrc/conv_fwd.hip
--- a/video-cycle_gan-upscaling_amd/csrc/conv_fwd.hip
+++ b/video-cycle_gan-upscaling_amd/csrc/conv_fwd.hip
@@ -19,6 +19,7 @@
     float* stats;
     const float* scale;
     const float* shift;
+    const unsigned* mask;
 };
 
 template <int KH, int KW, int S, int CK, int XT>
@@ -35,11 +36,13 @@
     static constexpr size_t LDS_BYTES = (size_t)(IN_ELEMS + W_ELEMS) * sizeof(float);
 };
 
-template <int XT, bool AFFINE = false>
+template <int XT, bool AFFINE = false, bool MASK = false>
 __device__ __forceinline__ void conv_epilogue(const ConvParams& p, f32x16 (&acc)[2][2][XT], int n, int co0, int oy0, int ox0,
                                               int wv, int lane) {
     const int half = lane >> 5, l31 = lane & 31;
-    const unsigned plane = (unsigned)(p.oh * p.ow), plane4 = 4u * plane, ow4 = 4u * (unsigned)p.ow;
+    const unsigned plane = (unsigned)(p.oh * p.ow), ow4 = 4u * (unsigned)p.ow;
+    unsigned plane4 = 4u * plane;
+    if constexpr (MASK) asm volatile("" : "+s"(plane4));
     const int nch = p.cout - co0 < 64 ? p.cout - co0 : 64;
     const size_t blk = ((size_t)n * p.cout + co0) * plane;
     const size_t blk_bytes = (size_t)nch * plane * sizeof(float);
@@ -53,6 +56,25 @@
     const vcg_rsrc rscale = make_rsrc(AFFINE ? p.scale : nullptr, AFFINE ? (size_t)p.cout * sizeof(float) : 0);
     const vcg_rsrc rshift = make_rsrc(AFFINE ? p.shift : nullptr, AFFINE ? (size_t)p.cout * sizeof(float) : 0);
 
+    unsigned mw[2][2];
+    if constexpr (MASK) {
+        static_assert(XT == 1 && !AFFINE, "the mask layout is that of 32-column tiles");
+        int tsx = p.tiles_x, tsy = p.tiles_y, cch = p.cout;
+        asm volatile("" : "+s"(tsx), "+s"(tsy), "+s"(cch));
+        const int pcb = (cch + 31) >> 5, ptx = (tsx + 1) >> 1, pty = tsy;
+        int ln = lane;
+        asm volatile("" : "+v"(ln));
+        const int px = ln & 1;
+        const unsigned pl = (unsigned)((ln & 32) + 16 * ((ox0 >> 5) & 1) + ((ln & 31) >> 1));
+#pragma unroll
+        for (int j = 0; j < 2; ++j) {
+            const int cbq = (co0 >> 5) + j, cbp = cbq < pcb ? cbq : pcb - 1;
+            const size_t tile = (size_t)(((n * pcb + cbp) * pty + (oy0 >> 3)) * ptx + (ox0 >> 6));
+            const u32x2 w2 = *reinterpret_cast<const u32x2*>(p.mask + ((tile * 4 + (unsigned)wv) * 64 + pl) * 2);
+            mw[j][0] = w2.x >> px;
+            mw[j][1] = w2.y >> px;
+        }
+    }
     const int oy = oy0 + wv * 2, ox = ox0 + l31;
     const unsigned base = (unsigned)(4 * half) * plane4 + (unsigned)oy * ow4 + 4u * (unsigned)ox;
     unsigned vo[2][XT];
@@ -84,6 +106,11 @@
             float bv[RG], al[RG], sc[RG], sh[RG];
 #pragma unroll
             for (int j = 0; j < RG; ++j) {
+                if constexpr (MASK) {
+                    bv[j] = 0.f;
+                    al[j] = 1.f;
+                    continue;
+                }
                 bv[j] = buf_load(rbias, chan4 + 4u * (unsigned)row_of(g, j));
                 const float pa = buf_load(rslope, chan4 + 4u * (unsigned)row_of(g, j));
                 al[j] = is_prelu ? pa : slope_u;
@@ -103,12 +130,14 @@
                     for (int xt = 0; xt < XT; ++xt) {
                         float v = acc[q >> 4][rt][xt][q & 15] + bv[j];
                         if (AFFINE) v = __builtin_fmaf(sc[j], v, sh[j]);
-                        if (PRELU_FMA) v = __builtin_fmaf(al[j], fminf(v, 0.f), fmaxf(v, 0.f));
+                        if (MASK) v = v * (((mw[q >> 4][(q >> 3) & 1] >> ((q & 7) * 4 + rt * 2)) & 1u) ? 1.f : p.alpha);
+                        else if (PRELU_FMA) v = __builtin_fmaf(al[j], fminf(v, 0.f), fmaxf(v, 0.f));
                         else v = v >= 0.f ? v : v * al[j];
                         if (RES) v += rs[g & 1][j][rt][xt];
                         buf_store(ry, __builtin_elementwise_add_sat(vo[rt][xt], srow), v);
                     }
                 }
+                if constexpr (MASK) __builtin_amdgcn_sched_barrier(0);
             }
         }
     };
@@ -316,7 +345,7 @@
     static constexpr int D_CH = PLANE - (KH - 1) * IW - (KW - 1);
 };
 
-template <int KH, int KW, int S>
+template <int KH, int KW, int S, bool MASK = false>
 __global__ __launch_bounds__(256, 2) void conv_c3_kernel(const ConvParams p) {
     using C = C3Cfg<KH, KW, S>;
     extern __shared__ __attribute__((aligned(16))) float smem[];
@@ -455,7 +484,7 @@
             store_tile(s_in + (cur ^ 1) * C::IN_BUF);
             lds_barrier();
         }
-        conv_epilogue<1>(p, acc, n0, co0, oy0, ox0, wv, lane);
+        conv_epilogue<1, false, MASK>(p, acc, n0, co0, oy0, ox0, wv, lane);
         if (!more) break;
         cur ^= 1;
     }
@@ -700,10 +729,11 @@
     return cus;
 }
 
-template <int KH, int KW, int S>
+template <int KH, int KW, int S, bool MASK = false>
 int launch_c3(ConvParams p, hipStream_t st) {
     using C = C3Cfg<KH, KW, S>;
     if (!conv_block_fits(p.oh, p.ow, 3, p.h, p.w_)) return VCG_E_UNSUPPORTED;
+    if (MASK && vcg_lrelu_mask_bytes(p.n, p.cout, p.oh, p.ow) >= 0xFFFFFFE0ull) return VCG_E_UNSUPPORTED;
     p.tiles_x = ceil_div(p.ow, 32);
     p.tiles_y = ceil_div(p.oh, C::ROWS);
     p.co_blocks = ceil_div(p.cout, 64);
@@ -714,7 +744,7 @@
     long grid = tiles < 2L * cus ? tiles : 2L * cus;
     grid -= grid % p.co_blocks;
     if (grid < p.co_blocks) grid = p.co_blocks;
-    return launch_with_lds(conv_c3_kernel<KH, KW, S>, (int)grid, C::LDS_BYTES, p, st);
+    return launch_with_lds(conv_c3_kernel<KH, KW, S, MASK>, (int)grid, C::LDS_BYTES, p, st);
 }
 
 template <int KH, int KW, int CK>
@@ -735,9 +765,10 @@
 
 int vcg_internal_conv(const float* x, const float* w, float* y, int n, int cin, int h, int wd, int cout,
                       int oh, int ow, int kh, int kw, int stride, int pad_top, int pad_left, int flip,
-                      const vcg_epilogue* ep, int smallm, int ws_t, int ws_m, int ws_k, hipStream_t st, float* stats, const float* scale, const float* shift) {
+                      const vcg_epilogue* ep, int smallm, int ws_t, int ws_m, int ws_k, hipStream_t st, float* stats, const float* scale, const float* shift,
+                      const unsigned* mask) {
     ConvParams p{};
-    p.x = x; p.w = w; p.y = y; p.stats = stats;
+    p.x = x; p.w = w; p.y = y; p.stats = stats; p.mask = mask;
     if (stats && (smallm || cin <= 3)) return VCG_E_UNSUPPORTED;
     if (scale && (smallm || stats || cin <= 3)) return VCG_E_UNSUPPORTED;
     if (scale && shift == nullptr) return VCG_E_NULL;
@@ -752,6 +783,10 @@
     p.pad_top = pad_top; p.pad_left = pad_left; p.flip = flip;
     p.ws_t = ws_t; p.ws_m = ws_m; p.ws_k = ws_k;
     if (n <= 0 || cin <= 0 || cout <= 0 || oh <= 0 || ow <= 0) return VCG_E_SHAPE;
+    if (mask) {
+        if (smallm || stats || scale || cin > 3 || kh != 9 || kw != 9 || stride != 1 || p.act != VCG_ACT_NONE || p.bias || p.residual) return VCG_E_UNSUPPORTED;
+        return launch_c3<9, 9, 1, true>(p, st);
+    }
     if (smallm) {
         if (stride != 1 || cout * kw > 32) return VCG_E_UNSUPPORTED;
         if (kh == 9 && kw == 9 && !flip && pad_top == 4 && pad_left == 4 && oh == h && ow == wd && !p.prelu && !p.residual) {
diff --git a/video-cycle_gan-upscaling_amd/csrc/conv_transpose.hip b/video-cycle_gan-upscaling_amd/csrc/conv_transpose.hip
--- a/video-cycle_gan-upscaling_amd/csrc/conv_transpose.hip
+++ b/video-cycle_gan-upscaling_amd/csrc/conv_transpose.hip
@@ -14,6 +14,7 @@
     int tiles_x, tiles_y, co_blocks;
     int act;
     float alpha;
+    unsigned* mask;
 };
 
 constexpr int phase_of(int k, int cb) { return (((k - cb) % 2) + 2) % 2; }
@@ -39,8 +40,9 @@
     static constexpr size_t LDS_BYTES = (size_t)(IN_ELEMS + W_ELEMS) * sizeof(float);
 };
 
-template <int K, int CBY, int CBX, int CK, int MT>
+template <int K, int CBY, int CBX, int CK, int MT, bool MASK = false>
 __global__ __launch_bounds__(256, (MT == 1 ? 2 : 1)) void convt_kernel(const ConvTParams p) {
+    static_assert(!MASK || MT == 1, "the mask layout is that of the 32-channel tile");
     using C = ConvTCfg<K, CBY, CBX, CK, MT>;
     extern __shared__ __attribute__((aligned(16))) float smem[];
     float* s_in = smem;
@@ -167,6 +169,7 @@
     const float slope_u = (p.act == VCG_ACT_LRELU) ? p.alpha : 1.f;
     auto emit = [&](auto guard_tag, auto res_tag) {
         constexpr bool GUARD = decltype(guard_tag)::value, RES = decltype(res_tag)::value;
+        unsigned mbits[2] = {0u, 0u};
 #pragma unroll
         for (int mt = 0; mt < MT; ++mt) {
 #pragma unroll
@@ -184,6 +187,10 @@
                     float v0 = acc[py][0][mt][r] + bvv, v1 = acc[py][1][mt][r] + bvv;
                     v0 = v0 >= 0.f ? v0 : v0 * al;
                     v1 = v1 >= 0.f ? v1 : v1 * al;
+                    if (MASK) {
+                        mbits[r >> 3] |= (v0 > 0.f ? 1u : 0u) << ((r & 7) * 4 + py * 2);
+                        mbits[r >> 3] |= (v1 > 0.f ? 1u : 0u) << ((r & 7) * 4 + py * 2 + 1);
+                    }
                     if (!GUARD) {
                         if (RES) { const float2 rr = *reinterpret_cast<const float2*>(rimg + o); v0 += rr.x; v1 += rr.y; }
                         *reinterpret_cast<float2*>(yimg + o) = make_float2(v0, v1);
@@ -206,17 +213,25 @@
                 }
             }
         }
+        if (MASK) {
+            const size_t tile = (((size_t)n * p.co_blocks + cb) * p.tiles_y + ty) * p.tiles_x + tx;
+            *reinterpret_cast<uint2*>(p.mask + (tile * 256 + tid) * 2) = make_uint2(mbits[0], mbits[1]);
+        }
     };
     using T_ = std::true_type;
     using F_ = std::false_type;
-    if (full) {
-        if (p.residual) emit(F_{}, T_{}); else emit(F_{}, F_{});
+    if constexpr (MASK) {
+        if (full) emit(F_{}, F_{}); else emit(T_{}, F_{});
     } else {
-        if (p.residual) emit(T_{}, T_{}); else emit(T_{}, F_{});
-    }
-}
-
-template <int K, int CBY, int CBX, int CK, int MT>
+        if (full) {
+            if (p.residual) emit(F_{}, T_{}); else emit(F_{}, F_{});
+        } else {
+            if (p.residual) emit(T_{}, T_{}); else emit(T_{}, F_{});
+        }
+    }
+}
+
+template <int K, int CBY, int CBX, int CK, int MT, bool MASK = false>
 int launch_convt(ConvTParams p, hipStream_t st) {
     using C = ConvTCfg<K, CBY, CBX, CK, MT>;
     p.tiles_x = ceil_div(ceil_div(p.ow, 2), 32);
@@ -224,7 +239,7 @@
     p.co_blocks = ceil_div(p.cout, C::MB);
     const long grid = (long)p.tiles_x * p.tiles_y * p.co_blocks * p.n;
     if (grid <= 0 || grid > 0x7fffffffL) return VCG_E_SHAPE;
-    auto kern = convt_kernel<K, CBY, CBX, CK, MT>;
+    auto kern = convt_kernel<K, CBY, CBX, CK, MT, MASK>;
     if (int e = vcg_allow_dyn_lds(reinterpret_cast<const void*>(kern), C::LDS_BYTES)) return e;
     hipLaunchKernelGGL(kern, dim3((int)grid), dim3(256), C::LDS_BYTES, st, p);
     VCG_LAUNCH_CHECK();
@@ -234,9 +249,9 @@
 }
 
 int vcg_internal_convt(const float* x, const float* w, float* y, int n, int cin, int h, int wd, int cout,
-                       int oh, int ow, int k, int cby, int cbx, const vcg_epilogue* ep, hipStream_t st) {
+                       int oh, int ow, int k, int cby, int cbx, const vcg_epilogue* ep, hipStream_t st, unsigned* mask) {
     ConvTParams p{};
-    p.x = x; p.w = w; p.y = y;
+    p.x = x; p.w = w; p.y = y; p.mask = mask;
     p.bias = ep ? ep->bias : nullptr;
     p.prelu = ep ? ep->prelu_alpha : nullptr;
     p.residual = ep ? ep->residual : nullptr;
@@ -246,6 +261,12 @@
     if (p.act == VCG_ACT_TANH) return VCG_E_UNSUPPORTED;
     p.n = n; p.cin = cin; p.h = h; p.w_ = wd; p.cout = cout; p.oh = oh; p.ow = ow;
     if (n <= 0 || cin <= 0 || cout <= 0 || oh <= 0 || ow <= 0) return VCG_E_SHAPE;
+    if (mask) {
+        if (p.act != VCG_ACT_LRELU || p.residual) return VCG_E_UNSUPPORTED;
+        if (k == 3 && cby == 0 && cbx == 0) return launch_convt<3, 0, 0, 16, 1, true>(p, st);
+        if (k == 4 && cby == 1 && cbx == 1) return launch_convt<4, 1, 1, 16, 1, true>(p, st);
+        return VCG_E_UNSUPPORTED;
+    }
 #define VCG_CT(K_, A_, B_, CK_, MT_) if (k == K_ && cby == A_ && cbx == B_) return launch_convt<K_, A_, B_, CK_, MT_>(p, st)
     VCG_CT(3, 0, 0, 16, 1); VCG_CT(3, 0, 1, 16, 1); VCG_CT(3, 1, 0, 16, 1); VCG_CT(3, 1, 1, 16, 1);
     VCG_CT(4, 1, 1, 16, 1);
diff --git a/video-cycle_gan-upscaling_amd/csrc/elementwise.hip b/video-cycle_gan-upscaling_amd/csrc/elementwise.hip
--- a/video-cycle_gan-upscaling_amd/csrc/elementwise.hip
+++ b/video-cycle_gan-upscaling_amd/csrc/elementwise.hip
@@ -19,7 +19,7 @@
     return d * g;
 }
 
-template <bool VEC>
+template <bool VEC, bool SUMONLY = false>
 __global__ __launch_bounds__(256) void act_bwd_kernel(const float* saved, const float* dy, int n, int c, int hw,
                                                       int act, float act_alpha, const float* prelu, float* dx,
                                                       float* part_alpha, float* part_sum ) {
@@ -31,6 +31,11 @@
     float v[2] = {0.f, 0.f};
     if (VEC) {
         for (int i = (blockIdx.x * 256 + threadIdx.x) * 4; i < hw; i += gridDim.x * 1024) {
+            if constexpr (SUMONLY) {
+                const float4 o = *reinterpret_cast<const float4*>(dy + base + i);
+                v[1] += (o.x + o.y) + (o.z + o.w);
+                continue;
+            }
             const float4 s = *reinterpret_cast<const float4*>(saved + base + i);
             const float4 d = *reinterpret_cast<const float4*>(dy + base + i);
             float4 o;
@@ -538,6 +543,24 @@
     return VCG_OK;
 }
 
+int vcg_act_bwd_dsum(const float* dz, int n, int c, int hw, float* dsum, void* ws, size_t ws_bytes, vcg_stream_t stream) {
+    VCG_CHECK_PTR(dz); VCG_CHECK_PTR(dsum);
+    if (n <= 0 || c <= 0 || hw <= 0 || (long)n * c > 0x7fffffffL) return VCG_E_SHAPE;
+    if (hw % 4 != 0) return VCG_E_UNSUPPORTED;
+    if (ws == nullptr || ws_bytes < vcg_act_bwd_workspace_bytes(n, c, hw)) return VCG_E_WORKSPACE;
+    hipStream_t st = (hipStream_t)stream;
+    const unsigned gy = (unsigned)((long)n * c > 65535 ? 65535 : n * c);
+    int gx = ceil_div(hw, 256 * 4);
+    if (gx > 64) gx = 64;
+    float* part_sum = (float*)ws + (size_t)n * c * 64;
+    hipLaunchKernelGGL((act_bwd_kernel<true, true>), dim3(gx, gy), dim3(256), 0, st, nullptr, dz, n, c, hw, VCG_ACT_NONE, 0.f, nullptr, nullptr,
+                       nullptr, part_sum);
+    VCG_LAUNCH_CHECK();
+    hipLaunchKernelGGL(plane_partial_final_kernel, dim3(ceil_div(c, 256)), dim3(256), 0, st, (const float*)part_sum, n, c, gx, dsum);
+    VCG_LAUNCH_CHECK();
+    return VCG_OK;
+}
+
 int vcg_head_act_bwd(const float* z, const float* dy, float* dz, size_t count, int kind, vcg_stream_t stream) {
     VCG_CHECK_PTR(z); VCG_CHECK_PTR(dy); VCG_CHECK_PTR(dz);
     if (kind < VCG_HEAD_NONE || kind > VCG_HEAD_BILOG) return VCG_E_UNSUPPORTED;
diff --git a/video-cycle_gan-upscaling_amd/upscaler/_engine.py b/video-cycle_gan-upscaling_amd/upscaler/_engine.py
--- a/video-cycle_gan-upscaling_amd/upscaler/_engine.py
+++ b/video-cycle_gan-upscaling_amd/upscaler/_engine.py
@@ -296,7 +296,7 @@
                                                 y.data_ptr(), rec.data_ptr(), rt.stream), "vcg_conv2d_fwd_stats[%s]" % self.name)
         return y, (x, None, d), (rec, nrec, bias)
 
-    def backward(self, ctx, dy, need_dx=True, param_grads=True, which=0, dx_residual=None, tag=None):
+    def backward(self, ctx, dy, need_dx=True, param_grads=True, which=0, dx_residual=None, tag=None, input_lrelu_slope=None, input_lrelu_mask=None):
         rt = self.rt
         x, y, d = ctx
         n = d.n
@@ -305,9 +305,19 @@
             dy = act_bwd_bias(self, y, dy, d, param_grads, which)
         if param_grads:
             self._wgrad_fp32(d, x, dy, which, not db_done, tag)
-        dx = None
+        masked = input_lrelu_mask is not None
+        dx, applied = None, False
         if need_dx:
             dx = rt.empty(n, self.cin, d.h, d.w)
+            if masked and dx_residual is None:
+                with Timed(rt, tag and tag + "_dgrad"):
+                    rc = rt.lib.vcg_conv2d_dgrad_lrelu_mask(ctypes.byref(d), dy.data_ptr(), self.ps[self.name + "/kernel"].data_ptr(),
+                                                            self._wt.get().data_ptr(), dx.data_ptr(), input_lrelu_mask.data_ptr(),
+                                                            float(input_lrelu_slope), rt.stream)
+                if rc != L.E_UNSUPPORTED:
+                    L.check(rc, "vcg_conv2d_dgrad_lrelu_mask[%s]" % self.name)
+                    applied = True
+        if need_dx and not applied:
             dd, dyd = d, dy
             if self.stride > 2:
                 s = self.stride
@@ -318,7 +328,7 @@
                 L.check(rt.lib.vcg_conv2d_dgrad(ctypes.byref(dd), dyd.data_ptr(), self.ps[self.name + "/kernel"].data_ptr(),
                                                 self._wt.get().data_ptr(), dx.data_ptr(), _ptr(dx_residual), rt.stream),
                         "vcg_conv2d_dgrad[%s]" % self.name)
-        return dx
+        return (dx, applied) if masked else dx
 
     def _wgrad_fp32(self, d, x, dy, which, with_bias, tag):
         rt = self.rt
@@ -349,22 +359,35 @@
         crop = max(self.k - 2, 0) // 2
         return L.ConvDesc(n, self.cin, h, w, self.cout, 2 * h, 2 * w, self.k, self.k, 2, crop, crop)
 
-    def forward(self, x, tag=None):
+    def forward(self, x, tag=None, write_mask=False):
         rt = self.rt
         n, _, h, w = x.shape
         d = self.desc(n, h, w)
         y = rt.empty(n, self.cout, d.oh, d.ow)
         ep = L.Epilogue(_ptr(self.ps[self.name + "/bias"]), self.act, float(self.alpha), None, None)
+        if write_mask and self.act == L.ACT_LRELU:
+            mask = torch.empty(rt.lib.vcg_lrelu_mask_bytes(n, self.cout, d.oh, d.ow), dtype=torch.uint8, device=rt.device)
+            with Timed(rt, tag):
+                rc = rt.lib.vcg_conv_transpose2d_fwd_mask(ctypes.byref(d), x.data_ptr(), self._wt.get().data_ptr(), y.data_ptr(),
+                                                          ctypes.byref(ep), mask.data_ptr(), rt.stream)
+            if rc != L.E_UNSUPPORTED:
+                L.check(rc, "vcg_conv_transpose2d_fwd_mask[%s]" % self.name)
+                return y, (x, y, d, mask)
         with Timed(rt, tag):
             L.check(rt.lib.vcg_conv_transpose2d_fwd(ctypes.byref(d), x.data_ptr(), self._wt.get().data_ptr(), y.data_ptr(),
                                                     ctypes.byref(ep), rt.stream), "vcg_conv_transpose2d_fwd[%s]" % self.name)
         return y, (x, y if self.act != L.ACT_NONE else None, d)
 
-    def backward(self, ctx, dy, need_dx=True, param_grads=True, which=0, tag=None):
-        rt = self.rt
-        x, y, d = ctx
+    def backward(self, ctx, dy, need_dx=True, param_grads=True, which=0, tag=None, dy_is_dz=False):
+        rt = self.rt
+        x, y, d = ctx[:3]
         db_done = self.act != L.ACT_NONE
-        if db_done:
+        if dy_is_dz:
+            if param_grads:
+                ws, wsn = rt.workspace(rt.lib.vcg_act_bwd_workspace_bytes(d.n, self.cout, d.oh * d.ow))
+                L.check(rt.lib.vcg_act_bwd_dsum(dy.data_ptr(), d.n, self.cout, d.oh * d.ow, self.ps.grad(self.name + "/bias", which).data_ptr(),
+                                                ws, wsn, rt.stream), "vcg_act_bwd_dsum[%s]" % self.name)
+        elif db_done:
             dy = act_bwd_bias(self, y, dy, d, param_grads, which)
         if param_grads:
             need = rt.lib.vcg_conv_transpose2d_wgrad_workspace_bytes(ctypes.byref(d))
diff --git a/video-cycle_gan-upscaling_amd/upscaler/_lib.py b/video-cycle_gan-upscaling_amd/upscaler/_lib.py
--- a/video-cycle_gan-upscaling_amd/upscaler/_lib.py
+++ b/video-cycle_gan-upscaling_amd/upscaler/_lib.py
@@ -49,6 +49,9 @@
     "vcg_conv2d_wgrad_workspace_bytes": (c_size_t, [_D]),
     "vcg_conv2d_wgrad": (c_int, [_D, _P, _P, _P, _P, _P, c_size_t, _P]),
     "vcg_conv_transpose2d_fwd": (c_int, [_D, _P, _P, _P, _E, _P]),
+    "vcg_lrelu_mask_bytes": (c_size_t, [c_int, c_int, c_int, c_int]),
+    "vcg_conv_transpose2d_fwd_mask": (c_int, [_D, _P, _P, _P, _E, _P, _P]),
+    "vcg_conv2d_dgrad_lrelu_mask": (c_int, [_D, _P, _P, _P, _P, _P, c_float, _P]),
     "vcg_conv_transpose2d_dgrad": (c_int, [_D, _P, _P, _P, _P, _P]),
     "vcg_conv_transpose2d_wgrad_workspace_bytes": (c_size_t, [_D]),
     "vcg_conv_transpose2d_wgrad": (c_int, [_D, _P, _P, _P, _P, _P, c_size_t, _P]),
@@ -68,6 +71,7 @@
                                  _P, _P, _P, _P, _P, c_size_t, _P]),
     "vcg_act_bwd_workspace_bytes": (c_size_t, [c_int, c_int, c_int]),
     "vcg_act_bwd": (c_int, [_P, _P, c_int, c_int, c_int, c_int, c_float, _P, _P, _P, _P, _P, c_size_t, _P]),
+    "vcg_act_bwd_dsum": (c_int, [_P, c_int, c_int, c_int, _P, _P, c_size_t, _P]),
     "vcg_channel_sum_workspace_bytes": (c_size_t, [c_int, c_int, c_int]),
     "vcg_channel_sum": (c_int, [_P, c_int, c_int, c_int, _P, _P, c_size_t, _P]),
     "vcg_dense_fwd": (c_int, [_P, _P, _P, _P, c_int, c_int, c_int, _P]),
diff --git a/video-cycle_gan-upscaling_amd/upscaler/model.py b/video-cycle_gan-upscaling_amd/upscaler/model.py
--- a/video-cycle_gan-upscaling_amd/upscaler/model.py
+++ b/video-cycle_gan-upscaling_amd/upscaler/model.py
@@ -387,6 +387,7 @@
             self.ups.append(self._add(upc("upscaling/%d/block/conv_transp" % i, cin, 256, k, L.ACT_LRELU, 0.2)))
             cin = 256
         self.c_fin = self._add(E.FinalConv9x9Bf16("final/conv", cin, 3, 9) if self.tail_bf16 else E.Conv2D("final/conv", cin, 3, 9, act=L.ACT_TANH))
+        self.lrelu_mask = True
         self._finish()
         if bf and k == 3 and len(self.blocks) * 2 + 1 <= 48:
             E.PackGroup3x3([c for b in self.blocks for c in (b[0], b[2])] + [self.c_pre])
@@ -443,7 +444,8 @@
         if self.trunk_dtype == "bf16" and not self.tail_bf16:
             h = E.from_bf16_nhwc(self.rt, h)
         for u in self.ups:
-            h, a = u.forward(h, tag="convt"); tape.append(a)
+            kw = {"write_mask": True} if training and self.lrelu_mask and not self.tail_bf16 and u is self.ups[-1] else {}
+            h, a = u.forward(h, tag="convt", **kw); tape.append(a)
         h, a = self.c_fin.forward(h, tag="final_conv"); tape.append(a)
         return h, tape
 
@@ -458,9 +460,17 @@
                 d = self.ups[i].backward(tape.pop(), d, True, True, which, tag="convt", dz_channel_sums=sums, **kw)
                 sums = None
         else:
-            d = self.c_fin.backward(tape.pop(), dy, True, True, which, tag="final_conv")
+            c_ctx = tape.pop()
+            u_ctx = tape[-1] if self.ups else ()
+            is_dz = False
+            if len(u_ctx) > 3:
+                d, is_dz = self.c_fin.backward(c_ctx, dy, True, True, which, tag="final_conv", input_lrelu_slope=self.ups[-1].alpha,
+                                               input_lrelu_mask=u_ctx[3])
+            else:
+                d = self.c_fin.backward(c_ctx, dy, True, True, which, tag="final_conv")
             for u in reversed(self.ups):
-                d = u.backward(tape.pop(), d, True, True, which, tag="convt")
+                d = u.backward(tape.pop(), d, True, True, which, tag="convt", dy_is_dz=is_dz)
+                is_dz = False
         if self.init_bf16:
             dskip = d
         elif self.tail_bf16:
```

Result: no change. 138.0 frames/s (median of 6 runs) (+0.8%).
